# infergo-ml/gogp

Measured on AMD Instinct MI355X. Metric: GP.Observe+Gradient evals/sec (fp64) at N=16384 D=8, higher is better.
Workload: dtype f64

## Files before the change

### gogp_amd/_lib.py

```python
from __future__ import annotations

import ctypes
import os
import subprocess

from .kernel import CDesc

_HERE = os.path.dirname(os.path.abspath(__file__))
LIB_PATH = os.path.join(_HERE, "libgogp_hip.so")
HOOKS_PATH = os.path.join(_HERE, "libgogp_testhooks.so")

GOGP_OK, GOGP_EARG, GOGP_ENOTPD, GOGP_EHIP, GOGP_ESTATE, GOGP_ENOMEM, GOGP_ECOND = 0, 1, 2, 3, 4, 5, 6
GOGP_MAX_CANDIDATES = 16
GOGP_BATCH_MAX_N = 128
GOGP_COV_MAX_M = 4096
GOGP_MULTI_MAX_T = 128

_dp = ctypes.POINTER(ctypes.c_double)
_i64 = ctypes.c_int64
_h = ctypes.c_void_p
_descp = ctypes.POINTER(CDesc)
GOGP_UNIQUE_ID_BYTES = 128


class CXfer(ctypes.Structure):
    _fields_ = [("peer", ctypes.c_int32), ("is_send", ctypes.c_int32), ("buf", ctypes.c_void_p),
                ("bytes", ctypes.c_int64)]


EXCHANGE_FN = ctypes.CFUNCTYPE(ctypes.c_int, ctypes.c_void_p, ctypes.POINTER(CXfer), ctypes.c_int32)
ALLREDUCE_FN = ctypes.CFUNCTYPE(ctypes.c_int, ctypes.c_void_p, ctypes.POINTER(ctypes.c_double),
                                ctypes.c_int64)
class CGemmOpts(ctypes.Structure):
    _fields_ = [(n, ctypes.c_int32) for n in ("ktri", "krag0", "new_row0", "kbeg0", "small_below", "prio", "rule",
                                              "tpb_shift", "rblk0", "cblk0", "pr", "Pr", "pc", "Pc", "beta0", "k")]
    _fields_ += [("bstride", ctypes.c_int64)]
    DEFAULTS = dict(ktri=0, krag0=-1, new_row0=-1, kbeg0=0, small_below=384, prio=0, rule=0, tpb_shift=0, rblk0=0,
                    cblk0=0, pr=0, Pr=1, pc=0, Pc=1, beta0=-1, k=1, bstride=0)


class CKParams(ctypes.Structure):
    _T, _D, _E = 4, 64, 32
    _fields_ = [("ndim", ctypes.c_int32), ("nterms", ctypes.c_int32), ("kind", ctypes.c_int32 * _T),
                ("ard", ctypes.c_int32 * _T), ("c", ctypes.c_double * _T), ("w", ctypes.c_double * _T),
                ("inv_len", (ctypes.c_double * _D) * _T), ("noise_var", ctypes.c_double), ("dnoise", ctypes.c_double),
                ("nevents", ctypes.c_int32), ("ev_axis", ctypes.c_int32), ("ev_from", ctypes.c_double * _E),
                ("ev_to", ctypes.c_double * _E), ("ev_disc", ctypes.c_double * _E)]


GOGP_TEST_NACC = 16 + 64


class CGemmPlan(ctypes.Structure):
    _fields_ = [("tile", ctypes.c_int32), ("waves", ctypes.c_int32), ("grid_x", ctypes.c_int64),
                ("grid_z", ctypes.c_int64), ("flops", ctypes.c_double), ("tag", ctypes.c_int64)]


SYMBOLS = [
    ("gogp_desc_check", ctypes.c_int, [_descp]),
    ("gogp_desc_ntheta_noise", ctypes.c_int, [_descp]),
    ("gogp_create", ctypes.c_int, [_descp, ctypes.c_int, ctypes.POINTER(_h)]),
    ("gogp_destroy", None, [_h]),
    ("gogp_last_error", ctypes.c_char_p, [_h]),
    ("gogp_notpd_index", _i64, [_h]),
    ("gogp_graph_info", ctypes.c_int, [_h, ctypes.POINTER(ctypes.c_int64), ctypes.POINTER(ctypes.c_int)]),
    ("gogp_events_check", ctypes.c_int, [_dp, ctypes.c_int, ctypes.c_int, ctypes.c_int]),
    ("gogp_set_events", ctypes.c_int, [_h, _dp, ctypes.c_int, ctypes.c_int]),
    ("gogp_set_data", ctypes.c_int, [_h, _dp, _dp, _i64]),
    ("gogp_set_data_device", ctypes.c_int, [_h, ctypes.c_void_p, ctypes.c_void_p, _i64]),
    ("gogp_absorb", ctypes.c_int, [_h, _dp, _dp]),
    ("gogp_observe", ctypes.c_int, [_h, _dp, _i64, _dp]),
    ("gogp_observe_full", ctypes.c_int, [_h, _dp, _i64, _dp]),
    ("gogp_lml", ctypes.c_int, [_h, _dp]),
    ("gogp_gradient", ctypes.c_int, [_h, _dp, _i64]),
    ("gogp_loo", ctypes.c_int, [_h, _dp, _dp, _dp, _dp]),
    ("gogp_loo_gradient", ctypes.c_int, [_h, _dp, _i64]),
    ("gogp_multi_set_outputs", ctypes.c_int, [_h, _dp, _i64, ctypes.c_int32]),
    ("gogp_multi_lml", ctypes.c_int, [_h, _dp, _dp]),
    ("gogp_multi_gradient", ctypes.c_int, [_h, _dp, _i64]),
    ("gogp_multi_get_alpha", ctypes.c_int, [_h, _dp]),
    ("gogp_multi_produce", ctypes.c_int, [_h, _dp, _i64, _dp, _dp]),
    ("gogp_observe_gradient_batch", ctypes.c_int,
     [ctypes.POINTER(_h), ctypes.c_int, _dp, _i64, _dp, _dp, ctypes.POINTER(ctypes.c_int)]),
    ("gogp_observe_gradient_candidates", ctypes.c_int,
     [_h, ctypes.c_int, _dp, _i64, _dp, _dp, ctypes.POINTER(ctypes.c_int)]),
    ("gogp_batch_set_data", ctypes.c_int,
     [_h, _dp, _dp, _i64, ctypes.c_int32, ctypes.POINTER(_i64), ctypes.POINTER(_i64)]),
    ("gogp_batch_observe_gradient", ctypes.c_int,
     [_h, ctypes.c_int32, ctypes.POINTER(ctypes.c_int32), _dp, _i64, _dp, _dp, ctypes.POINTER(ctypes.c_int)]),
    ("gogp_batch_produce", ctypes.c_int,
     [_h, ctypes.c_int32, ctypes.POINTER(ctypes.c_int32), _dp, _i64, ctypes.POINTER(_i64), _dp, _dp, _dp, _dp,
      ctypes.POINTER(ctypes.c_int)]),
    ("gogp_batch_observe_full_gradient", ctypes.c_int,
     [_h, ctypes.c_int32, _dp, ctypes.POINTER(_i64), _dp, _dp, ctypes.POINTER(ctypes.c_int)]),
    ("gogp_batch_produce_full", ctypes.c_int,
     [_h, ctypes.c_int32, _dp, ctypes.POINTER(_i64), ctypes.POINTER(_i64), _dp, _dp, _dp, _dp,
      ctypes.POINTER(ctypes.c_int)]),
    ("gogp_produce", ctypes.c_int, [_h, _dp, _i64, _dp, _dp]),
    ("gogp_produce_gradient", ctypes.c_int, [_h, _dp, _i64, _dp, _dp, _dp, _dp]),
    ("gogp_produce_covariance", ctypes.c_int, [_h, _dp, _i64, _dp, _dp]),
    ("gogp_produce_samples", ctypes.c_int, [_h, _dp, _i64, _dp, _i64, ctypes.c_double, _dp, _dp]),
    ("gogp_n", _i64, [_h]),
    ("gogp_get_alpha", ctypes.c_int, [_h, _dp]),
    ("gogp_get_factor", ctypes.c_int, [_h, _dp]),
    ("gogp_get_factor_rows", ctypes.c_int, [_h, ctypes.POINTER(_i64), _i64, _dp]),
    ("gogp_get_factor_diag", ctypes.c_int, [_h, _dp]),
    ("gogp_set_factor", ctypes.c_int, [_h, _dp, _dp, _dp, _dp]),
    ("gogp_append", ctypes.c_int, [_h, _dp, _dp, ctypes.c_int64]),
    ("gogp_remove", ctypes.c_int, [_h, ctypes.POINTER(_i64), ctypes.c_int64]),
    ("gogp_dist_grid", ctypes.c_int, [ctypes.c_int, ctypes.POINTER(ctypes.c_int), ctypes.POINTER(ctypes.c_int)]),
    ("gogp_dist_unique_id", ctypes.c_int, [ctypes.c_void_p]),
    ("gogp_dist_init_rccl", ctypes.c_int,
     [_h, ctypes.c_int, ctypes.c_int, ctypes.c_int, ctypes.c_int, ctypes.c_char_p]),
    ("gogp_dist_init_callbacks", ctypes.c_int,
     [_h, ctypes.c_int, ctypes.c_int, ctypes.c_int, ctypes.c_int, ctypes.c_void_p, ctypes.c_void_p,
      ctypes.c_void_p]),
    ("gogp_dist_local_bytes", _i64, [_h]),
    ("gogp_dist_comm_ranks", ctypes.c_int, [_h, ctypes.POINTER(ctypes.c_int)]),
    ("gogp_dist_selftest", ctypes.c_int, [_h, ctypes.c_int, _i64]),
    ("gogp_profile_enable", ctypes.c_int, [_h, ctypes.c_int]),
    ("gogp_profile_read", ctypes.c_int, [_h, _dp, ctypes.POINTER(_i64), _dp, _dp]),
    ("gogp_profile_read_launches", ctypes.c_int,
     [_h, _i64, _dp, _dp, _dp, ctypes.POINTER(_i64), ctypes.POINTER(_i64)]),
    ("gogp_profile_read_aux", ctypes.c_int, [_h, ctypes.c_int, _dp, ctypes.POINTER(_i64)]),
    ("gogp_set_option", ctypes.c_int, [_h, ctypes.c_char_p, _i64]),
    ("gogp_version", ctypes.c_char_p, []),
]

HOOK_SYMBOLS = [
    ("gogp_mfma_f64_peak", ctypes.c_int, [ctypes.c_int, ctypes.c_int, _dp, _dp, _dp]),
    ("gogp_mfma_f32_peak", ctypes.c_int, [ctypes.c_int, ctypes.c_int, _dp, _dp, _dp]),
    ("gogp_bench_gemm", ctypes.c_int,
     [ctypes.c_int, ctypes.c_int, ctypes.c_int, ctypes.c_int, _i64, ctypes.c_int, _dp, _dp]),
    ("gogp_test_diag256", ctypes.c_int,
     [ctypes.c_int, _dp, _dp, _dp, ctypes.POINTER(ctypes.c_uint64), _dp]),
    ("gogp_test_dgemm_nt", ctypes.c_int,
     [ctypes.c_int, _i64, _i64, _i64, ctypes.c_double, _dp, _dp, ctypes.c_double, _dp]),
    ("gogp_test_valu_cost", ctypes.c_int, [ctypes.c_int, _dp]),
    ("gogp_test_panel128", ctypes.c_int,
     [ctypes.c_int, _dp, _dp, _i64, ctypes.c_int, ctypes.POINTER(ctypes.c_uint64), _dp]),
    ("gogp_test_panel128_slabs", ctypes.c_int, [ctypes.c_int, _dp, _dp, _i64, ctypes.c_int, ctypes.c_int, _dp]),
    ("gogp_test_gemm_nt", ctypes.c_int,
     [ctypes.c_int, ctypes.c_int, ctypes.c_int, ctypes.c_int, ctypes.c_int, _i64, ctypes.c_double, ctypes.c_double]
     + [ctypes.c_void_p, _i64, _i64, _i64] * 3 + [ctypes.POINTER(CGemmOpts)]),
    ("gogp_test_gemm_plan", ctypes.c_int,
     [ctypes.c_int, ctypes.c_int, ctypes.c_int, ctypes.c_int, _i64, ctypes.POINTER(CGemmOpts),
      ctypes.POINTER(CGemmPlan)]),
    ("gogp_test_diag_syrk", ctypes.c_int,
     [ctypes.c_int, ctypes.c_int, ctypes.c_void_p, _i64, _i64, _i64, _i64, _i64, _dp, _i64, ctypes.c_int]),
    ("gogp_test_diag256_product", ctypes.c_int,
     [ctypes.c_int, ctypes.c_int, _dp, _i64, _dp, _i64, _dp, _i64, _i64, ctypes.POINTER(ctypes.c_longlong)]),
    ("gogp_test_trsm_small_workspace", _i64, [_i64]),
    ("gogp_test_trsm_small", ctypes.c_int,
     [ctypes.c_int, ctypes.c_int, _i64, ctypes.c_void_p, _i64, _i64, ctypes.c_void_p, ctypes.c_void_p, _i64, _i64,
      ctypes.c_int, ctypes.c_int, _dp, _i64, ctypes.c_void_p, _i64, ctypes.POINTER(ctypes.c_int),
      ctypes.POINTER(ctypes.c_int), ctypes.POINTER(_i64), ctypes.POINTER(ctypes.c_uint)]),
    ("gogp_test_trsv_steps", ctypes.c_int,
     [ctypes.c_int, ctypes.c_int, ctypes.c_int, _i64, ctypes.c_void_p, _i64, _i64, ctypes.c_void_p, ctypes.c_int,
      ctypes.c_int, ctypes.c_int, _i64, _dp, _i64, _dp, _i64]),
    ("gogp_test_alpha_from_y", ctypes.c_int,
     [ctypes.c_int, ctypes.c_int, _i64, ctypes.c_void_p, _i64, _i64, _dp, _i64, _dp, _i64]),
    ("gogp_test_rownorm_dot", ctypes.c_int,
     [ctypes.c_int, ctypes.c_int, ctypes.c_void_p, _i64, _i64, _i64, _i64, _dp, _i64, _dp, _i64, _dp, _i64]),
    ("gogp_test_tinv", ctypes.c_int,
     [ctypes.c_int, ctypes.c_int, ctypes.c_int, ctypes.c_void_p, ctypes.c_void_p, _i64, _i64, ctypes.c_int,
      ctypes.c_void_p]),
    ("gogp_test_blockmm", ctypes.c_int,
     [ctypes.c_int, ctypes.c_int, ctypes.c_int, ctypes.c_void_p, _i64] + [ctypes.POINTER(_i64)] * 6
     + [ctypes.POINTER(ctypes.c_int), ctypes.c_double, ctypes.c_int, _i64]),
    ("gogp_test_grad_blocks", ctypes.c_int, [_i64, _i64, _i64, ctypes.c_int]),
    ("gogp_test_grad_reduce", ctypes.c_int,
     [ctypes.c_int, ctypes.c_int, ctypes.POINTER(CKParams)] + [ctypes.c_int] * 4
     + [_dp, _i64, _dp, _i64, ctypes.c_void_p, _i64, _i64, _i64, _i64, ctypes.c_int, ctypes.c_int, _i64, _dp, _i64, _dp]),
    ("gogp_test_grad_reduce_local", ctypes.c_int,
     [ctypes.c_int, ctypes.c_int, ctypes.POINTER(CKParams)] + [ctypes.c_int] * 4
     + [_dp, _i64, _dp, _i64, ctypes.c_void_p, _i64, _i64, _i64, _i64, _i64, _i64] + [ctypes.c_int] * 7
     + [_i64, _dp, _i64, _dp]),
    ("gogp_test_xgrad", ctypes.c_int,
     [ctypes.c_int, ctypes.POINTER(CKParams), ctypes.c_int, _dp, _i64, _dp, _i64, _dp, _i64, _i64, _i64, _i64, _dp,
      _i64]),
    ("gogp_test_append_gram", ctypes.c_int,
     [ctypes.c_int] + [ctypes.c_void_p, _i64, ctypes.c_int, ctypes.c_int, _i64] * 2
     + [ctypes.c_int, ctypes.c_int, _i64, _i64, _dp, _i64, _dp, _i64, _dp, _i64, _i64]),
    ("gogp_test_append_commit", ctypes.c_int,
     [ctypes.c_int, ctypes.POINTER(CKParams), ctypes.c_int, _dp, _i64, _dp, _i64, ctypes.c_int, _i64, _dp, _i64,
      ctypes.c_int, _dp, _i64, _i64, _dp, _i64, ctypes.POINTER(ctypes.c_longlong)]),
    ("gogp_test_remove_gather", ctypes.c_int,
     [ctypes.c_int, _dp, _i64, _i64, ctypes.POINTER(ctypes.c_int), _i64, _i64, _dp, _i64, _i64]),
    ("gogp_test_remove_w", ctypes.c_int,
     [ctypes.c_int, _dp, _i64, _i64, ctypes.POINTER(ctypes.c_int), _i64, ctypes.POINTER(ctypes.c_int), _i64, ctypes.c_int,
      ctypes.c_int, _i64, _i64, _i64, _dp, _i64]),
    ("gogp_test_remove_block", ctypes.c_int,
     [ctypes.c_int, _dp, _i64, _i64, ctypes.c_int, ctypes.c_int, _dp, _i64, _dp, _i64, ctypes.c_int, _i64, _i64, _i64]),
    ("gogp_test_bwd_panel", ctypes.c_int,
     [ctypes.c_int, _i64] + [_dp, _i64, _i64, _i64] * 3 + [_i64, _i64, ctypes.c_int, ctypes.c_int]),
    ("gogp_test_pcov_slabs", ctypes.c_int, [_i64, _i64, ctypes.c_int, ctypes.POINTER(ctypes.c_int)]),
    ("gogp_test_pcov", ctypes.c_int,
     [ctypes.c_int, ctypes.POINTER(CKParams), ctypes.c_int, _dp, _i64, _i64, _dp, _i64, _i64, _i64, ctypes.c_int, _dp, _i64,
      ctypes.c_double, _dp, _i64, _i64, _i64]),
    ("gogp_test_multi_weight", ctypes.c_int,
     [ctypes.c_int, _dp, _i64, _i64, ctypes.c_int, _dp, _i64, _i64, _i64, _i64, _dp, _i64]),
    ("gogp_test_dist_init_replay", ctypes.c_int, [ctypes.c_void_p] + [ctypes.c_int] * 4),
]


def build(force: bool = False) -> str:
    csrc = os.path.join(_HERE, "csrc")
    cmd = ["make", "-C", csrc, "-j8", "-s"]
    if force:
        cmd.append("-B")
    subprocess.check_call(cmd)
    if not os.path.exists(LIB_PATH):
        raise RuntimeError("build did not produce %s" % LIB_PATH)
    return LIB_PATH


_lib = None
_hooks = None


def hooks() -> ctypes.CDLL:
    global _hooks
    if _hooks is None:
        lib()
        if not os.path.exists(HOOKS_PATH):
            raise ImportError("%s is missing: run __graft_entry__.build()" % HOOKS_PATH)
        L = ctypes.CDLL(HOOKS_PATH)
        for name, restype, argtypes in HOOK_SYMBOLS:
            f = getattr(L, name)
            f.restype = restype
            f.argtypes = argtypes
        _hooks = L
    return _hooks


def lib() -> ctypes.CDLL:
    global _lib
    if _lib is None:
        if not os.path.exists(LIB_PATH):
            raise ImportError(
                "%s is missing: build it with `python -c 'import __graft_entry__ as g; g.build()'` "
                "(gogp_amd has no CPU fallback)" % LIB_PATH)
        try:
            import torch
        except ImportError:
            pass
        L = ctypes.CDLL(LIB_PATH, mode=ctypes.RTLD_GLOBAL)
        for name, restype, argtypes in SYMBOLS:
            f = getattr(L, name)
            f.restype = restype
            f.argtypes = argtypes
        _lib = L
    return _lib
```

### gogp_amd/csrc/api.hip

```cpp
#include <math.h>
#include <stdio.h>
#include <stdlib.h>
#include <string.h>

#include <algorithm>
#include <initializer_list>
#include <mutex>
#include <new>
#include <thread>
#include <type_traits>
#include <utility>

#include "handle.h"

using namespace gogp;

static thread_local std::string g_create_error;

extern "C" int gogp_desc_ntheta_noise(const gogp_desc *d) {
  return (d && (d->noise_kind == GOGP_NOISE_UNIFORM || d->noise_kind == GOGP_NOISE_CONSTANT_PARAM)) ? 1 : 0;
}

extern "C" int gogp_desc_check(const gogp_desc *d) {
  if (!d) return GOGP_EARG;
// ... 352 lines not shown
}

static void fill_params_theta(const gogp_handle *h, const double *ts, const double *tn, DevParams &p) {
  const gogp_desc &d = h->desc;
  memset(&p, 0, sizeof p);
  p.ndim = d.ndim;
  p.nterms = d.nterms;
  p.ns = h->ns;
  p.nn = h->nn;
  for (int t = 0; t < d.nterms; ++t) {
    const gogp_term &T = d.terms[t];
    p.kind[t] = T.kind;
    p.ard[t] = T.ard;
    p.c[t] = T.scale_idx >= 0 ? ts[T.scale_idx] : 1.0;
    p.w[t] = 0.0;
    if (T.kind == GOGP_K_PERIODIC)
      p.w[t] = M_PI / (T.period_mult * ts[T.period_idx]);
    for (int j = 0; j < d.ndim; ++j)
      p.inv_len[t][j] = 1.0 / ts[T.len_idx + (T.ard ? j : 0)];
  }
  if (d.noise_kind == GOGP_NOISE_CONSTANT || d.noise_kind == GOGP_NOISE_CONSTANT_PARAM) {
    p.noise_var = d.noise_std * d.noise_std;
    p.dnoise = 0.0;
  } else {
    const double sd = tn[0];
    p.noise_var = d.noise_scale * sd * sd;
    p.dnoise = 2.0 * p.noise_var;
  }
  p.nevents = h->nevents;
  p.ev_axis = h->ev_axis;
  for (int e = 0; e < h->nevents; ++e) {
    p.ev_from[e] = h->events[e][0];
    p.ev_to[e] = h->events[e][1];
    p.ev_disc[e] = h->events[e][2];
  }
}

static void fill_params(const gogp_handle *h, DevParams &p) {
  fill_params_theta(h, h->theta_s.data(), h->theta_n.data(), p);
}

int gogp_upload_params(gogp_handle *h) {
  if (h->batch_mode) return GOGP_OK;
  fill_params(h, *h->hostP);
  HIPCHK(h, hipMemcpyAsync(h->devP, h->hostP, sizeof(DevParams), hipMemcpyHostToDevice, h->s));
  return GOGP_OK;
}

static hipError_t cand_memset(gogp_handle *h, void *dst, size_t bytes, hipStream_t s) {
  hipError_t e = hipSuccess;
  for (int c = 0; c < h->batch_k && e == hipSuccess; ++c)
    e = gogp::rec_memset_async((char *)dst + (size_t)c * h->cand_stride, 0, bytes, s);
  return e;
}
static hipError_t cand_copy_in(gogp_handle *h, void *dst, const void *src, size_t bytes, hipStream_t s) {
  hipError_t e = hipSuccess;
  for (int c = 0; c < h->batch_k && e == hipSuccess; ++c)
    e = gogp::rec_memcpy_async((char *)dst + (size_t)c * h->cand_stride, src, bytes, hipMemcpyDeviceToDevice, s);
  return e;
}
static hipError_t cand_d2h(gogp_handle *h, double *hdst, const void *dsrc, size_t bytes, hipStream_t s) {
  hipError_t e = hipSuccess;
  for (int c = 0; c < h->batch_k && e == hipSuccess; ++c)
    e = gogp::rec_memcpy_async(hdst + (size_t)c * BATCH_ROW, (const char *)dsrc + (size_t)c * h->cand_stride, bytes,
                               hipMemcpyDeviceToHost, s);
  return e;
}

static int ensure_y(gogp_handle *h) {
  if (h->bufY && h->cap_y >= h->npad) return GOGP_OK;
  (void)hipFree(h->bufY);
  h->bufY = nullptr;
  h->cap_y = 0;
  const int64_t cap = std::max(h->npad, h->cap_npad);
  HIPCHK(h, hipMalloc(&h->bufY, (size_t)cap * (size_t)cap * h->esz()));
  h->cap_y = cap;
  return GOGP_OK;
}

static int ensure_d64(gogp_handle *h) {
  if (h->D64 && h->cap_d64 >= h->npad) return GOGP_OK;
  (void)hipFree(h->D64);
  h->D64 = nullptr;
  h->cap_d64 = 0;
  const int64_t cap = std::max(h->npad, h->cap_npad);
  HIPCHK(h, hipMalloc(&h->D64, (size_t)cap * PANEL * sizeof(double)));
  h->cap_d64 = cap;
  return GOGP_OK;
}

struct FactorResult {
  int rc = GOGP_OK;
  double lml = 0.0, cond_lb = 1.0, yta = 0.0;
  int64_t notpd = -1;
  std::string msg;
};
static FactorResult judge_scalars(const gogp_handle *h, const double *hs, bool fp32, bool refine, int64_t n = -1) {
  FactorResult r;
  long long info = 0;
  memcpy(&info, hs + HS_INFO, sizeof info);
  char buf[160];
  if (info != 0) {
    r.rc = GOGP_ENOTPD;
    r.notpd = (int64_t)info - 1;
    snprintf(buf, sizeof buf, "Factorize: matrix is not positive definite (pivot %lld)", (long long)r.notpd);
    r.msg = buf;
    return r;
  }
  const double logdet = fp32 ? hs[5] : hs[0];
  const double ztz = refine ? hs[6] : hs[1];
  r.yta = ztz;
  r.lml = -0.5 * (double)(n < 0 ? h->n : n) * log(2 * M_PI) - 0.5 * logdet - 0.5 * ztz;
  const double dmin = hs[3], dmax = hs[4];
  r.cond_lb = (dmin > 0.0) ? (dmax / dmin) * (dmax / dmin) : INFINITY;
  if (!(r.cond_lb <= h->cond_limit)) {
    snprintf(buf, sizeof buf, "Condition: matrix singular or near-singular with condition number >= %.4e",
             r.cond_lb);
    r.msg = buf;
    r.rc = GOGP_ECOND;
  }
  return r;
}

static int finish_factorize(gogp_handle *h, bool fp32, bool refine, bool kinv) {
  h->alpha_pending = true;
  if (h->batch_mode) {
    h->factored = h->have_alpha = true;
    if (kinv) h->have_kinv = true;
    return GOGP_OK;
  }
  HIPCHK(h, hipStreamSynchronize(h->s));
  HIPCHK(h, hipGetLastError());
  const FactorResult fr = judge_scalars(h, h->hscal, fp32, refine);
  if (fr.rc == GOGP_ENOTPD) {
    h->alpha_pending = h->kinv_pending = false;
    h->tinv_valid = h->tinv_pending = false;
    h->trtri_done = h->trtri_pending = false;
    h->notpd = fr.notpd;
    h->err = fr.msg;
    return GOGP_ENOTPD;
  }
  h->lml = fr.lml;
  h->logdet2 = h->hscal[0];
  h->yta = fr.yta;
  h->factored = h->have_alpha = true;
  h->z_valid = true;
  if (kinv) h->have_kinv = true;
  h->cond_lb = fr.cond_lb;
  if (fr.rc == GOGP_ECOND) h->err = fr.msg;
  return fr.rc;
}

static void diag_block(gogp_handle *h, hipStream_t sp, const double *A, int64_t ld, double *L, int64_t ldl,
                       double *Dp, int64_t c0) {
  launch_diag256(sp, A, ld, L, ldl, Dp, c0, h->n, h->info);
}
static void diag_block(gogp_handle *h, hipStream_t sp, const float *A, int64_t ld, float *L, int64_t ldl,
                       float *Dp, int64_t c0) {
  double *A64 = h->dscr, *L64 = h->dscr + PANEL * PANEL, *D64 = h->dscr + 2 * PANEL * PANEL;
  if (h->d64_active)
    A64 = h->D64 + (size_t)(c0 / PANEL) * PANEL * PANEL;
  else
    launch_convert_block(sp, A, ld, A64, PANEL, PANEL, PANEL);
  launch_diag256(sp, A64, PANEL, L64, PANEL, D64, c0, h->n, h->info);
  launch_convert_block(sp, L64, PANEL, L, ldl, PANEL, PANEL);
  launch_convert_block(sp, D64, PANEL, Dp, PANEL, PANEL, PANEL);
  launch_logdet_block(sp, L64, PANEL, c0, h->n, PANEL, h->scalars + 5);
}
static void diag_inv_only(gogp_handle *h, hipStream_t s, const double *L, int64_t ld, double *Dp) {
  (void)h;
  launch_diag256_inv_only(s, L, ld, Dp);
}
static void diag_inv_only(gogp_handle *h, hipStream_t s, const float *L, int64_t ld, float *Dp) {
  double *L64 = h->dscr + PANEL * PANEL, *D64 = h->dscr + 2 * PANEL * PANEL;
  launch_convert_block(s, L, ld, L64, PANEL, PANEL, PANEL);
  launch_diag256_inv_only(s, L64, PANEL, D64);
  launch_convert_block(s, D64, PANEL, Dp, PANEL, PANEL, PANEL);
}

static inline int chain_prio_of(const gogp_handle *h) {
  return h->chain_prio < 0 ? (h->npad <= 6144 ? 1 : 0) : h->chain_prio;
}
static inline GemmGrid chain_grid(const gogp_handle *h) {
  GemmGrid g;
  g.prio = chain_prio_of(h);
  return g;
}

static inline int superpanel_width(const gogp_handle *h, int npanel, int P0) {
  const int head = h->superpanel_head < 0 ? (h->prec == 32 ? 4 : 3) : h->superpanel_head;
  const int sw = (head > 0 && npanel - P0 > h->head_remaining) ? head : h->superpanel;
  return (npanel - P0 < sw) ? npanel - P0 : sw;
}
struct SuperPanel {
  int P0, nsub, prevP0, next_nsub;
  int64_t C0() const { return (int64_t)P0 * PANEL; }
  int64_t CE() const { return C0() + (int64_t)nsub * PANEL; }
};
static std::vector<SuperPanel> superpanels(const gogp_handle *h) {
  const int npanel = (int)(h->npad / PANEL);
  std::vector<SuperPanel> v;
  for (int P0 = 0; P0 < npanel; P0 += v.back().nsub) {
    const int nsub = superpanel_width(h, npanel, P0);
    if (!v.empty()) v.back().next_nsub = nsub;
    v.push_back({P0, nsub, v.empty() ? -1 : v.back().P0, 0});
  }
  return v;
}
struct InnerGroup {
  int grp;
  int64_t k0, ce;
};
static inline InnerGroup inner_group(int q, int64_t c2, int64_t CE) {
  const int done = q + 1, grp = done & -done;
  return {grp, c2 - (int64_t)grp * PANEL, std::min(c2 + (int64_t)grp * PANEL, CE)};
}

constexpr int TMT_BLOCKS = 8;
static inline int tinv_panels(const gogp_handle *h) { return h->produce_panels; }
static inline int64_t tinv_signature(const gogp_handle *h) {
  return (int64_t)h->produce_panels + (h->npad << 8) + ((int64_t)h->prec << 56);
}
static int ensure_tinv(gogp_handle *h) {
  const int64_t tld = (int64_t)tinv_panels(h) * PANEL;
  const size_t need = (size_t)std::max(h->npad, h->cap_npad) * (size_t)tld;
  if (!h->TX || h->cap_tinv < need) {
    (void)hipFree(h->TX);
    (void)hipFree(h->Tmt);
    h->TX = h->Tmt = nullptr;
    h->cap_tinv = 0;
    HIPCHK(h, hipMalloc(&h->TX, need * h->esz()));
    HIPCHK(h, hipMalloc(&h->Tmt, (size_t)TMT_BLOCKS * PANEL * PANEL * h->esz()));
    h->cap_tinv = need;
  }
  h->tinv_ld = tld;
  return GOGP_OK;
}

template <class T>
static void assemble_tinv(gogp_handle *h, hipStream_t sp, int P0, int nsub) {
  const int64_t ld = h->npad, tld = h->tinv_ld, C0 = (int64_t)P0 * PANEL;
  T *X = reinterpret_cast<T *>(h->TX) + C0 * tld;
  T *MT = reinterpret_cast<T *>(h->Tmt);
  const T *L = reinterpret_cast<const T *>(h->bufL);
  const T *Dinv = reinterpret_cast<const T *>(h->Dinv) + (size_t)P0 * PANEL * PANEL;
  launch_tinv_init(sp, Dinv, X, (T *)nullptr, nsub, tld);
  for (int d = 1; d < nsub; ++d) {
    const int cnt = nsub - d;
    for (int b0 = 0; b0 < cnt; b0 += 6) {
      const int nb = std::min(6, cnt - b0);
      const T *A1[6], *B1[6], *A2[6], *B2[6];
      T *C1[6], *C2[6];
      int64_t lda1[6], ldb1[6], ldc1[6], lda2[6], ldb2[6], ldc2[6];
      int K1[6], K2[6];
      for (int b = 0; b < nb; ++b) {
        const int i = d + b0 + b, j = i - d;
        A1[b] = L + (C0 + (int64_t)i * PANEL) * ld + C0 + (int64_t)j * PANEL;
        lda1[b] = ld;
        B1[b] = X + (int64_t)j * PANEL * tld + (int64_t)j * PANEL;
        ldb1[b] = tld;
        C1[b] = MT + (size_t)(b0 + b) * PANEL * PANEL;
        ldc1[b] = PANEL;
        K1[b] = d * PANEL;
        A2[b] = Dinv + (size_t)i * PANEL * PANEL;
        lda2[b] = PANEL;
        B2[b] = C1[b];
        ldb2[b] = PANEL;
        C2[b] = X + (int64_t)i * PANEL * tld + (int64_t)j * PANEL;
        ldc2[b] = tld;
        K2[b] = PANEL;
      }
      launch_blockmm(sp, nb, A1, lda1, B1, ldb1, C1, ldc1, K1, 1.0);
      launch_blockmm(sp, nb, A2, lda2, B2, ldb2, C2, ldc2, K2, -1.0);
    }
  }
}

template <class T>
struct InvBufs {
  T *A, *Y;
  const T *L, *Dinv;
};
template <class T>
static void trtri_superstep(gogp_handle *h, const InvBufs<T> &B, const SuperPanel &P, hipStream_t st, hipStream_t s2) {
  const int64_t npad = h->npad, ld = npad;
  T *R = B.A, *Y = B.Y;
  const T *L = B.L;
  GemmProfile *pf = &h->prof;
  const int P0 = P.P0;
  const int64_t C0 = P.C0(), CE = P.CE();
  for (int q = 0; q < P.nsub; ++q) {
    const int p = P0 + q;
    const int64_t c0 = (int64_t)p * PANEL, c2 = c0 + PANEL;
    const T *Dp = B.Dinv + (size_t)p * PANEL * PANEL;
    launch_ydiag(st, Dp, Y + c0 * ld + c0, ld);
    if (c2 < CE)
      launch_zero_block(st, Y + c2 * ld + c0, ld, CE - c2, PANEL);
    if (c0 > 0) {
      GemmGrid gtri = chain_grid(h);
      gtri.ktri = h->ktri;
      launch_gemm_nt(st, GEMM_RECT, (int)(c0 / TILE), 2, PANEL, 1.0, R + c0, ld, Dp, PANEL, 0.0,
                      Y + c0, ld, pf, &gtri);
    }
    if (c2 < CE) {
      const InnerGroup g = inner_group(q, c2, CE);
      GemmGrid gch = chain_grid(h);
      if (h->krag) gch.krag0 = (int)(g.k0 / TILE);
      launch_gemm_nt(st, GEMM_RECT, (int)(c2 / TILE), (int)((g.ce - c2) / TILE), (int64_t)g.grp * PANEL,
                      -1.0, Y + g.k0, ld, L + c2 * ld + g.k0, ld, 1.0, R + c2, ld, pf, &gch);
    }
  }
  order(h, EV_BASE + 4 * P0 + 2, st, s2);
  const int nt = (int)((npad - CE) / TILE);
  if (nt > 0) {
    const int64_t Kw = CE - C0;
    const int mr = (int)(CE / TILE);
    const int ntn = nt < 2 * P.next_nsub ? nt : 2 * P.next_nsub;
    if (P0 > 0 && st != s2)
      (void)gogp::rec_stream_wait(st, ev(h, EV_BASE + 4 * P.prevP0 + 3));
    GemmGrid gch = chain_grid(h), gbulk;
    if (h->krag) gch.krag0 = gbulk.krag0 = (int)(C0 / TILE);
    launch_gemm_nt(st, GEMM_RECT, mr, ntn, Kw, -1.0, Y + C0, ld, L + CE * ld + C0, ld, 1.0,
                    R + CE, ld, pf, &gch);
    if (nt > ntn) {
      const int64_t C3 = CE + (int64_t)ntn * TILE;
      launch_gemm_nt(s2, GEMM_RECT, mr, nt - ntn, Kw, -1.0, Y + C0, ld, L + C3 * ld + C0, ld, 1.0,
                      R + C3, ld, pf, &gbulk);
    }
    (void)gogp::rec_event_record(ev(h, EV_BASE + 4 * P0 + 3), s2);
  }
}

static inline bool mixed_gradient(const gogp_handle *h) {
  return h->grad_prec == 32 && h->prec == 64 && !h->batch_mode && !h->dist;
}
static int ensure_g32(gogp_handle *h) {
  const int64_t cap = std::max(h->npad, h->cap_npad);
  if (h->g32A && h->g32_cap >= cap) return GOGP_OK;
  (void)hipFree(h->g32A);
  (void)hipFree(h->g32L);
  (void)hipFree(h->g32Y);
  (void)hipFree(h->g32D);
  h->g32A = h->g32L = h->g32Y = h->g32D = nullptr;
  h->g32_cap = 0;
  const size_t nn = (size_t)cap * (size_t)cap * sizeof(float);
  HIPCHK(h, hipMalloc(&h->g32A, nn));
  HIPCHK(h, hipMalloc(&h->g32L, nn));
  HIPCHK(h, hipMalloc(&h->g32Y, nn));
  HIPCHK(h, hipMalloc(&h->g32D, (size_t)(cap / PANEL) * PANEL * PANEL * sizeof(float)));
  h->g32_cap = cap;
  return GOGP_OK;
}
static void mixed_superstep(gogp_handle *h, const SuperPanel &P, hipStream_t st, hipStream_t s2) {
  const int64_t npad = h->npad, ld = npad, C0 = P.C0(), W = P.CE() - C0;
  launch_convert_block(st, h->bufL + C0 * ld + C0, ld, h->g32L + C0 * ld + C0, ld, (int)(npad - C0), (int)W);
  launch_convert_block(st, h->Dinv + (size_t)P.P0 * PANEL * PANEL, PANEL, h->g32D + (size_t)P.P0 * PANEL * PANEL, PANEL,
                       (int)W, PANEL);
  const InvBufs<float> B{h->g32A, h->g32Y, h->g32L, h->g32D};
  trtri_superstep<float>(h, B, P, st, s2);
}

template <class T>
static void kinv_accumulate(gogp_handle *h, const T *Y, T *A, int64_t C0, int64_t CE) {
  (void)gogp::rec_stream_wait(h->sk, ev(h, EV_BASE + 4 * (size_t)(C0 / PANEL) + 2));
  GemmGrid gk;
  gk.new_row0 = (int)(C0 / TILE);
  if (h->krag) gk.krag0 = (int)(C0 / TILE);
  launch_gemm_nt(h->sk, GEMM_LOWER, (int)(CE / TILE), (int)(CE / TILE), CE - C0, 1.0, Y + C0, h->npad, Y + C0, h->npad,
                 1.0, A, h->npad, &h->prof, &gk);
}

template <class T>
static void zero_inverse_rhs(gogp_handle *h, bool mixed, hipStream_t s) {
  if (mixed)
    launch_zero_upper_blocks(s, h->g32A, h->npad, h->npad);
  else
    launch_zero_upper_blocks(s, reinterpret_cast<T *>(h->bufA), h->npad, h->npad);
}
template <class T>
static void inverse_superstep(gogp_handle *h, bool mixed, const SuperPanel &P, hipStream_t st, hipStream_t s2,
                              bool fuse_kinv) {
  if (mixed) {
    mixed_superstep(h, P, st, s2);
    if (fuse_kinv) kinv_accumulate<float>(h, h->g32Y, h->g32A, P.C0(), P.CE());
  } else {
    const InvBufs<T> B{reinterpret_cast<T *>(h->bufA), reinterpret_cast<T *>(h->bufY), reinterpret_cast<const T *>(h->bufL),
                       reinterpret_cast<const T *>(h->Dinv)};
    trtri_superstep<T>(h, B, P, st, s2);
    if (fuse_kinv) kinv_accumulate<T>(h, B.Y, B.A, P.C0(), P.CE());
  }
}

static inline int chain_split_of(const gogp_handle *h, bool eager) {
  if (h->dist || h->prec != 64) return 0;
  if (h->chain_split >= 0) return h->chain_split;
  return (h->npad <= 8192 || !eager) ? 2 : 0;
}
static void fused_panel(gogp_handle *h, hipStream_t sp, double *A, double *L, int64_t ld, int64_t c0, int64_t npad,
                        GemmProfile *pf) {
  const int64_t c1 = c0 + TILE, c2 = c0 + PANEL;
  const int mt1 = (int)((npad - c1) / TILE);
  const GemmGrid gch = chain_grid(h);
  launch_panel128_slabs(sp, A + c0 * ld + c0, ld, L + c0 * ld + c0, ld, 0, npad - c1, c0, h->n, h->info, h->chain_slabs);
  launch_gemm_nt(sp, GEMM_RECT, mt1, 1, TILE, -1.0, L + c1 * ld + c0, ld, L + c1 * ld + c0, ld, 1.0, A + c1 * ld + c1, ld,
                 pf, &gch);
  launch_panel128_slabs(sp, A + c0 * ld + c0, ld, L + c0 * ld + c0, ld, 1, npad - c2, c0, h->n, h->info, h->chain_slabs);
}

static void begin_evaluation(gogp_handle *h, std::initializer_list<hipStream_t> streams) {
  auto wait = [&](int e) {
    for (hipStream_t q : streams) (void)gogp::rec_stream_wait(q, ev(h, e));
  };
  if (h->trtri_pending) wait(EV_TRTRI);
  if (h->kinv_pending) wait(EV_KINV);
  if (h->kinv_c1 > 0 && !h->have_kinv) wait(EV_KINV);
  h->trtri_pending = h->kinv_pending = false;
  h->factored = h->have_alpha = h->have_kinv = h->grad_valid = false;
  h->multi_solved = false;
  h->alpha_pending = h->trtri_done = h->ydone_valid = h->d64_active = false;
  h->notpd = -1;
  h->kinv_c1 = 0;
  if (!h->batch_mode) h->tinv_valid = false;
}
static hipError_t enqueue_result_scalars(gogp_handle *h, hipStream_t s) {
  const hipError_t e = cand_d2h(h, h->hscal, h->scalars, 7 * sizeof(double), s);
  return e != hipSuccess ? e : cand_d2h(h, h->hscal + HS_INFO, h->info, sizeof(long long), s);
}

template <class T>
static void substitute_fwd(gogp_handle *h, hipStream_t q, const T *L, const T *Dinv, double *w, double *dst) {
  const int npanel = (int)(h->npad / PANEL);
  for (int b = 0; b < npanel; ++b) launch_trsv_fwd_step(q, L, h->npad, Dinv, b, npanel, w, dst);
}
template <class T>
static hipError_t substitute_bwd(gogp_handle *h, hipStream_t q, const T *L, const T *Dinv, const double *src, double *w,
                                 double *dst) {
  const int npanel = (int)(h->npad / PANEL);
  const hipError_t e = hipMemcpyAsync(w, src, (size_t)h->npad * sizeof(double), hipMemcpyDeviceToDevice, q);
  for (int b = npanel - 1; b >= 0 && e == hipSuccess; --b) launch_trsv_bwd_step(q, L, h->npad, Dinv, b, npanel, w, dst);
  return e;
}

template <class T>
struct Sweep {
  static constexpr bool fp32 = sizeof(T) == 4;
  gogp_handle *h;
  bool eager;
  T *A = reinterpret_cast<T *>(h->bufA), *L = reinterpret_cast<T *>(h->bufL), *Dinv = reinterpret_cast<T *>(h->Dinv);
  int64_t npad = h->npad, ld = npad;
  int npanel = (int)(npad / PANEL);
  GemmProfile *pf = &h->prof;
  hipStream_t s = h->s, st = h->st, s2 = h->s2;
  hipStream_t sp = h->lookahead ? h->sp : h->s;
  hipStream_t sz = h->lookahead ? h->sl : sp;
  bool mixed = !fp32 && mixed_gradient(h);
  bool fuse_kinv = eager && (h->kinv_fused < 0 ? (npad <= 10240 || mixed) : h->kinv_fused != 0);
  int split = fp32 ? 0 : chain_split_of(h, eager);

  void d64_init(hipStream_t q, int first, int nblk) const {
    if constexpr (fp32)
      launch_widen_diag_blocks(q, A + (int64_t)first * PANEL * (ld + 1), ld, h->D64 + (size_t)first * PANEL * PANEL, nblk);
  }
  void d64_update(hipStream_t q, int64_t k0, int64_t K, int first, int nblk) const {
    if constexpr (fp32) {
      if (h->d64_active)
        launch_diag_syrk_f64(q, L + (int64_t)first * PANEL * ld + k0, ld, K, h->D64 + (size_t)first * PANEL * PANEL, nblk);
    }
  }

  int build_gram() const {
    if (sp != s) order(h, EV_ENTRY, s, sp);
    HIPCHK(h, cand_memset(h, h->info, sizeof(long long), sp));
    const int w0 = superpanel_width(h, npanel, 0);
    {
      AuxTimer tm(h, GOGP_PROF_GRAM, s);
      launch_gram_lower_split(sp, s, h->devP, h->D, h->dX, h->n, npad, A, ld, (int64_t)w0 * PANEL, h->ev());
    }
    h->d64_active = fp32 && h->diag_fp64 != 0;
    if (h->d64_active) {
      const int rc = ensure_d64(h);
      if (rc != GOGP_OK) return rc;
      d64_init(sp, 0, w0);
      if (npanel > w0) d64_init(s, w0, npanel - w0);
    }
    (void)gogp::rec_event_record(ev(h, EV_GRAM), s);
    if (eager) {
      (void)gogp::rec_stream_wait(s2, ev(h, EV_GRAM));
      (void)gogp::rec_stream_wait(st, ev(h, EV_GRAM));
      zero_inverse_rhs<T>(h, mixed, s2);
      order(h, EV_INIT, s2, st);
    }
    return GOGP_OK;
  }

  void chain_superpanel(const SuperPanel &P) const {
    const int64_t CE = P.CE();
    for (int q = 0; q < P.nsub; ++q) {
      const int p = P.P0 + q;
      const int64_t c0 = (int64_t)p * PANEL, c2 = c0 + PANEL;
      if constexpr (!fp32) {
        if (split) fused_panel(h, sp, A, L, ld, c0, npad, pf);
      }
      if (!split) {
        T *Dp = Dinv + (size_t)p * PANEL * PANEL;
        diag_block(h, sp, A + c0 * ld + c0, ld, L + c0 * ld + c0, ld, Dp, c0);
        const int mt2 = (int)((npad - c2) / TILE);
        if (mt2 > 0) {
          GemmGrid gtri = chain_grid(h);
          gtri.ktri = h->ktri;
          launch_gemm_nt(sp, GEMM_RECT, mt2, 2, PANEL, 1.0, A + c2 * ld + c0, ld, Dp, PANEL, 0.0,
                          L + c2 * ld + c0, ld, pf, &gtri);
        }
      }
      if (c2 < CE) {
        d64_update(sp, c0, PANEL, p + 1, (int)((CE - c2) / PANEL));
        const InnerGroup g = inner_group(q, c2, CE);
        const GemmGrid gch = chain_grid(h);
        launch_gemm_nt(sp, GEMM_TRAP, (int)((npad - c2) / TILE), (int)((g.ce - c2) / TILE),
                        (int64_t)g.grp * PANEL, -1.0, L + c2 * ld + g.k0, ld, L + c2 * ld + g.k0, ld, 1.0,
                        A + c2 * ld + c2, ld, pf, &gch);
      }
    }
  }

  void panels_final(const SuperPanel &P) const {
    order(h, EV_BASE + 4 * P.P0, sp, s);
    if (sz != sp) (void)gogp::rec_stream_wait(sz, ev(h, EV_BASE + 4 * P.P0));
    if constexpr (!fp32) {
      if (split) {
        launch_dinv256_blocks(sz, L + (int64_t)P.P0 * PANEL * (ld + 1), ld, Dinv + (size_t)P.P0 * PANEL * PANEL, P.nsub);
        if (eager) {
          (void)gogp::rec_event_record(ev(h, EV_BASE + 5 * (size_t)npanel + 32 + (size_t)P.P0), sz);
          (void)gogp::rec_stream_wait(st, ev(h, EV_BASE + 5 * (size_t)npanel + 32 + (size_t)P.P0));
        }
      }
    }
    for (int q = 0; q < P.nsub; ++q) launch_trsv_fwd_step(sz, L, ld, Dinv, P.P0 + q, npanel, h->w, h->z);
  }

  void trailing_update(const SuperPanel &P) const {
    const int64_t C0 = P.C0(), CE = P.CE();
    const int mtE = (int)((npad - CE) / TILE);
    if (mtE <= 0) return;
    const int64_t Kw = CE - C0;
    const int ntn = mtE < 2 * P.next_nsub ? mtE : 2 * P.next_nsub;
    (void)gogp::rec_stream_wait(sp, ev(h, P.P0 > 0 ? EV_BASE + 4 * P.prevP0 + 1 : EV_GRAM));
    const GemmGrid gch = chain_grid(h);
    launch_gemm_nt(sp, GEMM_TRAP, mtE, ntn, Kw, -1.0, L + CE * ld + C0, ld, L + CE * ld + C0, ld,
                    1.0, A + CE * ld + CE, ld, pf, &gch);
    d64_update(sp, C0, Kw, (int)(CE / PANEL), ntn / 2);
    if (mtE > ntn) {
      const int64_t C3 = CE + (int64_t)ntn * TILE;
      launch_gemm_nt(s, GEMM_LOWER, mtE - ntn, mtE - ntn, Kw, -1.0, L + C3 * ld + C0, ld,
                      L + C3 * ld + C0, ld, 1.0, A + C3 * ld + C3, ld, pf);
      d64_update(s, C0, Kw, (int)(C3 / PANEL), (mtE - ntn) / 2);
    }
    (void)gogp::rec_event_record(ev(h, EV_BASE + 4 * P.P0 + 1), s);
  }

  void inverse_behind(const SuperPanel &P) const {
    const int64_t CE = P.CE();
    (void)gogp::rec_stream_wait(st, ev(h, EV_BASE + 4 * P.P0));
    inverse_superstep<T>(h, mixed, P, st, s2, fuse_kinv);
    if (!fp32 && !fuse_kinv && !mixed && !h->batch_mode && h->kinv_split > 0 && h->kinv_c1 == 0 && CE < npad &&
        CE * 100 >= npad * (int64_t)h->kinv_split) {
      (void)gogp::rec_stream_wait(h->sk, ev(h, EV_BASE + 4 * P.P0 + 2));
      const T *Y0 = reinterpret_cast<const T *>(h->bufY);
      launch_gemm_nt(h->sk, GEMM_LAUUM, (int)(CE / TILE), (int)(CE / TILE), CE, 1.0, Y0, ld, Y0, ld, 0.0, A, ld, pf);
      (void)gogp::rec_event_record(ev(h, EV_KINV), h->sk);
      h->kinv_c1 = CE;
    }
  }

  int finish_alpha() const {
    if (fp32) {
      if (sz != sp) (void)gogp::rec_stream_wait(sp, ev(h, EV_FWD));
      HIPCHK(h, substitute_bwd(h, sp, L, Dinv, h->z, h->w, h->alpha));
      for (int it = 0; it < h->refine_steps; ++it) {
        launch_residual(sp, h->devP, h->D, h->dX, h->n, npad, h->alpha, h->dy, h->rpart, REFINE_SLABS, h->rw,
                        h->radial1, h->ev());
        substitute_fwd(h, sp, L, Dinv, h->rw, h->rz);
        HIPCHK(h, substitute_bwd(h, sp, L, Dinv, h->rz, h->rw, h->rd));
        launch_axpy(sp, h->alpha, h->rd, npad);
      }
      launch_dot(sp, h->dy, h->alpha, h->n, h->scalars + 6);
      order(h, EV_ALPHA, sp, s);
    }
    HIPCHK(h, enqueue_result_scalars(h, s));
    if (fp32) {
      if (eager) (void)gogp::rec_event_record(ev(h, EV_TRTRI), st);
    } else if (eager && !mixed) {
      (void)gogp::rec_stream_wait(st, ev(h, EV_FWD));
      launch_alpha_from_y(st, reinterpret_cast<const T *>(h->bufY), ld, h->z, npad, h->alpha);
      (void)gogp::rec_event_record(ev(h, EV_ALPHA), st);
      (void)gogp::rec_event_record(ev(h, EV_TRTRI), st);
    } else {
      if (sz != sp) (void)gogp::rec_stream_wait(sp, ev(h, EV_FWD));
      HIPCHK(h, substitute_bwd(h, sp, L, Dinv, h->z, h->w, h->alpha));
      (void)gogp::rec_event_record(ev(h, EV_ALPHA), sp);
    }
    return GOGP_OK;
  }
};

template <class T>
static int factorize_t(gogp_handle *h, bool eager) {
  const Sweep<T> c{h, eager && h->lookahead != 0};
  begin_evaluation(h, {c.s, c.sp});
  int rc = gogp_upload_params(h);
  if (rc == GOGP_OK && (c.mixed || c.eager)) rc = c.mixed ? ensure_g32(h) : ensure_y(h);
  if (rc == GOGP_OK) rc = c.build_gram();
  if (rc != GOGP_OK) return rc;
  if (c.fp32) HIPCHK(h, hipMemsetAsync(h->scalars + 5, 0, sizeof(double), c.sp));
  HIPCHK(h, cand_copy_in(h, h->w, h->dy, (size_t)c.npad * sizeof(double), c.sp));
  if (c.sz != c.sp) order(h, EV_W, c.sp, c.sz);
  for (const SuperPanel &P : superpanels(h)) {
    c.chain_superpanel(P);
    c.panels_final(P);
    c.trailing_update(P);
    if (c.eager) c.inverse_behind(P);
  }
  if (c.fuse_kinv) {
    (void)gogp::rec_event_record(ev(h, EV_KINV), h->sk);
    h->kinv_pending = true;
  }
  if (c.eager) {
    (void)gogp::rec_event_record(ev(h, EV_TRTRI), c.st);
    (void)gogp::rec_event_record(ev(h, EV_YDONE), c.st);
    h->ydone_valid = h->trtri_done = h->trtri_pending = true;
  }
  order(h, EV_FWD, c.sz, c.s);
  launch_lml_scalars(c.s, c.L, c.ld, h->z, nullptr, nullptr, h->n, h->scalars);
  rc = c.finish_alpha();
  if (rc != GOGP_OK) return rc;
  const int rcf = finish_factorize(h, c.fp32, c.fp32, false);
  if (rcf == GOGP_ENOTPD)
    for (hipStream_t q : {c.sp, c.st, c.s2, h->sl, h->sk}) (void)hipStreamSynchronize(q);
  return rcf;
}

static inline bool tiny_ok(const gogp_handle *h) {
  return h->tiny && !h->dist && h->prec == 64 && h->npad == PANEL && h->n <= TILE && !mixed_gradient(h);
}
static int tiny_factorize(gogp_handle *h, bool eager) {
  hipStream_t s = h->s;
  begin_evaluation(h, {s});
  int rc = gogp_upload_params(h);
  if (rc != GOGP_OK) return rc;
  if (h->lookahead && !h->batch_mode) {
    order(h, EV_ENTRY, h->sp, s);
    order(h, EV_W, h->sl, s);
  }
  HIPCHK(h, cand_memset(h, h->info, sizeof(long long), s));
  launch_tiny_eval(s, h->devP, h->dX, h->dy, h->n, h->bufA, h->bufL, h->Dinv, h->z, h->alpha, h->info, eager, h->ev());
  launch_lml_scalars(s, h->bufL, h->npad, h->z, nullptr, nullptr, h->n, h->scalars);
  (void)gogp::rec_event_record(ev(h, EV_ALPHA), s);
  HIPCHK(h, enqueue_result_scalars(h, s));
  return finish_factorize(h, false, false, eager);
// ... 1946 lines not shown
  return GOGP_OK;
}

extern "C" int gogp_profile_read(gogp_handle *h, double *gemm_ms, int64_t *gemm_launches,
                                 double *gemm_flops, double *gemm_busy_ms) {
  if (!h) return GOGP_EARG;
  HIPCHK(h, hipSetDevice(h->device));
  for (hipStream_t q : work_streams(h)) HIPCHK(h, hipStreamSynchronize(q));
  double ms = 0.0, busy = 0.0;
  std::vector<std::pair<double, double>> iv;
  iv.reserve(h->prof.used / 2);
  for (size_t i = 0; i + 1 < h->prof.used; i += 2) {
    float t = 0.f, t0 = 0.f;
    if (hipEventElapsedTime(&t, h->prof.pool[i], h->prof.pool[i + 1]) != hipSuccess) continue;
    ms += t;
    if (hipEventElapsedTime(&t0, h->prof.pool[0], h->prof.pool[i]) != hipSuccess) continue;
    iv.emplace_back((double)t0, (double)t0 + (double)t);
  }
  std::sort(iv.begin(), iv.end());
  double cur_b = 0, cur_e = -1;
  for (auto &p : iv) {
    if (cur_e < cur_b || p.first > cur_e) {
      if (cur_e >= cur_b) busy += cur_e - cur_b;
      cur_b = p.first;
      cur_e = p.second;
    } else if (p.second > cur_e) {
      cur_e = p.second;
    }
  }
  if (cur_e >= cur_b && !iv.empty()) busy += cur_e - cur_b;
  if (gemm_ms) *gemm_ms = ms;
  if (gemm_launches) *gemm_launches = h->prof.launches;
  if (gemm_flops) *gemm_flops = h->prof.flops;
  if (gemm_busy_ms) *gemm_busy_ms = busy;
  h->prof.used = 0;
  h->prof.flops = 0;
  h->prof.launches = 0;
  h->prof.lflops.clear();
  h->prof.ltag.clear();
  return GOGP_OK;
}

extern "C" int gogp_set_option(gogp_handle *h, const char *name, int64_t value) {
  if (!h || !name) return GOGP_EARG;
  drop_cand_graph(h);
  if (strcmp(name, "produce_tinv") == 0) {
    h->produce_tinv = value != 0;
    return GOGP_OK;
  }
  if (strcmp(name, "produce_panels") == 0) {
    if (value < 1 || value > 8) return fail(h, GOGP_EARG, "produce_panels must be 1..8");
    h->produce_panels = (int)value;
    return GOGP_OK;
  }
  if (strcmp(name, "produce_small_below") == 0) {
    if (value < 0) return fail(h, GOGP_EARG, "produce_small_below must be >= 0");
    h->produce_small_below = (int)value;
    return GOGP_OK;
  }
  if (strcmp(name, "produce_small_max") == 0) {
    if (value < 0 || value > 64) return fail(h, GOGP_EARG, "produce_small_max must be 0..64");
    h->produce_small_max = (int)value;
    return GOGP_OK;
  }
  if (strcmp(name, "produce_groups") == 0) {
    if (value < 1 || value > PRODUCE_GROUPS) return fail(h, GOGP_EARG, "produce_groups must be 1..4");
    h->produce_groups = (int)value;
    return GOGP_OK;
  }
  if (strcmp(name, "gradient_precision") == 0) {
    if (value != 32 && value != 64) return fail(h, GOGP_EARG, "gradient_precision must be 32 or 64");
    if (value == 32 && (h->desc.nterms != 1 || h->desc.terms[0].scale_idx < 0))
      return fail(h, GOGP_EARG, "gradient_precision = 32 is offered for one-term kernels with an output scale only");
    HIPCHK(h, hipSetDevice(h->device));
    for (hipStream_t q : work_streams(h)) HIPCHK(h, hipStreamSynchronize(q));
    h->grad_prec = (int)value;
    h->have_kinv = h->grad_valid = false;
    h->trtri_done = h->trtri_pending = h->kinv_pending = false;
    return GOGP_OK;
  }
  if (strcmp(name, "trace_fp64") == 0) {
    h->trace_fp64 = value != 0;
    return GOGP_OK;
  }
  if (strcmp(name, "krag") == 0) {
    h->krag = value != 0;
    return GOGP_OK;
  }
  if (strcmp(name, "lookahead") == 0) {
    h->lookahead = value != 0;
    return GOGP_OK;
  }
  if (strcmp(name, "eager") == 0) {
    h->eager = value != 0;
    return GOGP_OK;
  }
  if (strcmp(name, "precision") == 0) {
    if (value != 32 && value != 64) return fail(h, GOGP_EARG, "precision must be 32 or 64");
    if (h->dist && (int)value != h->prec)
      return fail(h, GOGP_EARG, "precision: set it before gogp_dist_init_* (the shard's buffers are typed)");
    if ((int)value != h->prec) {
      HIPCHK(h, hipSetDevice(h->device));
      for (hipStream_t q : work_streams(h)) HIPCHK(h, hipStreamSynchronize(q));
      free_n_buffers(h);
      free_m_buffers(h);
      free_cand_buffers(h);
      h->prec = (int)value;
      h->have_data = h->factored = h->have_alpha = h->have_kinv = h->observed = h->grad_valid = false;
      h->multi_T = 0;
      h->multi_solved = false;
      h->trtri_done = h->trtri_pending = h->alpha_pending = h->kinv_pending = false;
    }
    return GOGP_OK;
  }
  if (strcmp(name, "kinv_split") == 0) {
    if (value < 0 || value > 95) return fail(h, GOGP_EARG, "kinv_split must be 0..95");
    h->kinv_split = (int)value;
    return GOGP_OK;
  }
  if (strcmp(name, "kinv_fused") == 0) {
    h->kinv_fused = value < 0 ? -1 : (value != 0);
    return GOGP_OK;
  }
  if (strcmp(name, "superpanel_head") == 0) {
    if (value < -1 || value > 8) return fail(h, GOGP_EARG, "superpanel_head must be -1..8");
    h->superpanel_head = (int)value;
    return GOGP_OK;
  }
  if (strcmp(name, "head_remaining") == 0) {
    if (value < 0) return fail(h, GOGP_EARG, "head_remaining must be >= 0");
    h->head_remaining = (int)value;
    return GOGP_OK;
  }
  if (strcmp(name, "ard_mfma_min_dims") == 0) {
    if (value < 1 || value > 65) return fail(h, GOGP_EARG, "ard_mfma_min_dims must be 1..65");
    h->ard_mfma_min = (int)value;
    return GOGP_OK;
  }
  if (strcmp(name, "chain_prio") == 0) {
    if (value < -1 || value > 2) return fail(h, GOGP_EARG, "chain_prio must be -1..2");
    h->chain_prio = (int)value;
    return GOGP_OK;
  }
  if (strcmp(name, "tiny") == 0) {
    if (value < 0 || value > 1) return fail(h, GOGP_EARG, "tiny must be 0 or 1");
    h->tiny = (int)value;
    return GOGP_OK;
  }
  if (strcmp(name, "chain_slabs") == 0) {
    if (value < 0 || value > 8) return fail(h, GOGP_EARG, "chain_slabs must be 0..8");
    h->chain_slabs = (int)value;
    return GOGP_OK;
  }
  if (strcmp(name, "chain_split") == 0) {
    if (value < -1 || value > 2 || value == 1) return fail(h, GOGP_EARG, "chain_split must be -1, 0 or 2");
    h->chain_split = (int)value;
    return GOGP_OK;
  }
  if (strcmp(name, "ktri") == 0) {
    h->ktri = value != 0;
    return GOGP_OK;
  }
  if (strcmp(name, "graph") == 0) {
    if (value < 0 || value > 3) return fail(h, GOGP_EARG, "graph must be 0..3");
    h->use_graph = (int)value;
    h->graph_failed = false;
    drop_cand_graph(h);
    return GOGP_OK;
  }
  if (strcmp(name, "diag_fp64") == 0) {
    if (value < 0 || value > 1) return fail(h, GOGP_EARG, "diag_fp64 must be 0 or 1");
    h->diag_fp64 = (int)value;
    return GOGP_OK;
  }
  if (strcmp(name, "refine_steps") == 0) {
    if (value < 0 || value > 8) return fail(h, GOGP_EARG, "refine_steps must be 0..8");
    h->refine_steps = (int)value;
    return GOGP_OK;
  }
  if (strcmp(name, "cond_limit_log10") == 0) {
    if (value < 1 || value > 300) return fail(h, GOGP_EARG, "cond_limit_log10 must be 1..300");
    h->cond_limit = pow(10.0, (double)value);
    return GOGP_OK;
  }
  if (strcmp(name, "superpanel") == 0) {
    if (value < 1 || value > 8) return fail(h, GOGP_EARG, "superpanel must be 1..8");
    h->superpanel = (int)value;
    return GOGP_OK;
  }
  return fail(h, GOGP_EARG, "unknown option");
}
```

### gogp_amd/csrc/common.h

```cpp
#pragma once
#include <hip/hip_runtime.h>
#include <stdint.h>

#include <string>
#include <vector>

#include "../../include/gogp_hip.h"
#include "graphrec.h"

namespace gogp {

constexpr int TILE = 128;
constexpr int PANEL = 256;
constexpr int GEMM_BK = 16;

struct DevParams {
  int ndim, nterms, ns, nn;
  int kind[GOGP_MAX_TERMS];
  int ard[GOGP_MAX_TERMS];
  double c[GOGP_MAX_TERMS];
  double w[GOGP_MAX_TERMS];
  double inv_len[GOGP_MAX_TERMS][GOGP_MAX_NDIM];
  double noise_var;
  double dnoise;
  int nevents, ev_axis;
  double ev_from[GOGP_MAX_EVENTS], ev_to[GOGP_MAX_EVENTS], ev_disc[GOGP_MAX_EVENTS];
};

constexpr int ACC_TRACE = 3 * GOGP_MAX_TERMS;
constexpr int ACC_ARD0 = 16;
constexpr int NACC = ACC_ARD0 + GOGP_MAX_NDIM;

struct Batch {
  int k = 1;
  long stride = 0;
};
inline thread_local Batch tl_batch;
template <class P>
__device__ __forceinline__ P *cand(P *p, long bstride) {
  return (P *)((const char *)p + (long)blockIdx.z * bstride);
}

struct GemmProfile {
  bool on = false;
  std::vector<hipEvent_t> pool;
  size_t used = 0;
  double flops = 0;
  int64_t launches = 0;
  std::vector<double> lflops;
  std::vector<int64_t> ltag;
};

struct GemmGrid {
  int rule = 0, tpb_shift = 0, rblk0 = 0, cblk0 = 0, pr = 0, Pr = 1, pc = 0, Pc = 1, beta0 = -1;
  int new_row0 = -1;
  int ktri = 0;
  int prio = 0;
  int krag0 = -1;
  int small_below = 384;
  int kbeg0 = 0;
};

struct BlockMap {
  int nb_shift = 9, pr = 0, Pr = 1, pc = 0, Pc = 1;
  __host__ __device__ long grow(long lrow) const {
    const long nbm = (1L << nb_shift) - 1;
    return ((((lrow >> nb_shift) * Pr + pr)) << nb_shift) + (lrow & nbm);
  }
  __host__ __device__ long gcol(long lcol) const {
    const long nbm = (1L << nb_shift) - 1;
    return ((((lcol >> nb_shift) * Pc + pc)) << nb_shift) + (lcol & nbm);
  }
};

#ifdef GOGP_WGSTAMP
struct StampRec {
  long long base, nwg, tag, stream;
};
constexpr int STAMP_SLOTS = 8;
extern unsigned long long *g_stamp_buf;
extern long long g_stamp_cap, g_stamp_used, g_stamp_nrec;
extern StampRec g_stamp_rec[1 << 16];
unsigned long long *stamp_reserve(long long nwg, long long tag, hipStream_t s);
#endif

enum GemmMode { GEMM_RECT = 0, GEMM_LOWER = 1, GEMM_LAUUM = 2,
                GEMM_TRAP = 3 };

void launch_dgemm_nt(hipStream_t s, GemmMode mode, int mt, int nt, int64_t K,
                     double alpha, const double *A, int64_t lda, const double *B,
                     int64_t ldb, double beta, double *C, int64_t ldc,
                     GemmProfile *prof, const GemmGrid *grid = nullptr);

void launch_gemm_nt(hipStream_t s, GemmMode mode, int mt, int nt, int64_t K, double alpha, const double *A,
                    int64_t lda, const double *B, int64_t ldb, double beta, double *C, int64_t ldc,
                    GemmProfile *prof, const GemmGrid *grid = nullptr);
void launch_gemm_nt(hipStream_t s, GemmMode mode, int mt, int nt, int64_t K, double alpha, const float *A,
                    int64_t lda, const float *B, int64_t ldb, double beta, float *C, int64_t ldc,
                    GemmProfile *prof, const GemmGrid *grid = nullptr);
void launch_gram_lower_split(hipStream_t s_first, hipStream_t s_rest, const DevParams *p, int ndim,
                             const double *X, int64_t n, int64_t npad, float *K, int64_t ld,
                             int64_t wcols, bool ev = false);
void launch_cross(hipStream_t s, const DevParams *p, int ndim, const double *X, int64_t n,
                  int64_t npad, const double *Z, int64_t m, int64_t mpad, float *KsT, int64_t ld, bool ev = false);
void launch_trsv_fwd_step(hipStream_t s, const float *L, int64_t ld, const float *Dinv, int b, int nblk,
                          double *y, double *z);
void launch_trsv_bwd_step(hipStream_t s, const float *L, int64_t ld, const float *Dinv, int b, int nblk,
                          double *zwork, double *alpha);
void launch_lml_scalars(hipStream_t s, const float *L, int64_t ld, const double *z, const double *y,
                        const double *alpha, int64_t n, double *scalars);
void launch_alpha_from_y(hipStream_t s, const float *Y, int64_t ld, const double *z, int64_t npad,
                         double *alpha);
void launch_rownorm_dot(hipStream_t s, const float *V, int64_t ld, const double *vec, int64_t ncols,
                        int64_t m, double *dot, double *sq);
void launch_zero_upper_blocks(hipStream_t s, float *R, int64_t ld, int64_t npad);
void launch_zero_block(hipStream_t s, float *B, int64_t ld, int64_t rows, int64_t cols);
void launch_ydiag(hipStream_t s, const float *Dinv, float *Ydiag, int64_t ld);
void launch_extract_lower(hipStream_t s, const float *L, int64_t ld, int64_t n, double *out);
void launch_pack_lower(hipStream_t s, const double *in, int64_t n, int64_t npad, float *L, int64_t ld);
void launch_convert_block(hipStream_t s, const float *src, int64_t lds_, double *dst, int64_t ldd, int rows,
                          int cols);
void launch_convert_block(hipStream_t s, const double *src, int64_t lds_, float *dst, int64_t ldd, int rows,
                          int cols);
void launch_grad_reduce(hipStream_t s, const DevParams *p, int ndim, int ard_dims, const double *X,
                        const double *alpha, const float *Kinv, int64_t ld, int64_t n, int64_t npad,
                        double *partials, double *out, bool radial1 = false, int mfma_min_dims = 1, bool ev = false,
                        int max_blocks = 0);

void launch_gram_lower(hipStream_t s, const DevParams *p, int ndim, const double *X,
                       int64_t n, int64_t npad, double *K, int64_t ld, bool ev = false);
void launch_gram_local(hipStream_t s, const DevParams *p, int ndim, const double *X, int64_t n,
                       int64_t mrows, int64_t ncols, BlockMap map, double *K, int64_t ld, bool ev = false);
void launch_gram_local(hipStream_t s, const DevParams *p, int ndim, const double *X, int64_t n,
                       int64_t mrows, int64_t ncols, BlockMap map, float *K, int64_t ld, bool ev = false);
void launch_gram_lower_split(hipStream_t s_first, hipStream_t s_rest, const DevParams *p, int ndim,
                             const double *X, int64_t n, int64_t npad, double *K, int64_t ld,
                             int64_t wcols, bool ev = false);
void launch_cross(hipStream_t s, const DevParams *p, int ndim, const double *X, int64_t n,
                  int64_t npad, const double *Z, int64_t m, int64_t mpad, double *KsT,
                  int64_t ld, bool ev = false);
void launch_residual(hipStream_t s, const DevParams *p, int ndim, const double *X, int64_t n, int64_t npad,
                     const double *v, const double *y, double *part, int nslab, double *r, bool radial1 = false,
                     bool ev = false);
void launch_kmatvec_share(hipStream_t s, const DevParams *p, int ndim, const double *X, int64_t n, int64_t npad,
                          const double *v, int part_idx, int nparts, double *part, int nslab, double *out,
                          bool radial1 = false, bool ev = false);
void launch_prior(hipStream_t s, const DevParams *p, const double *Z, int64_t m,
                  double *prior);

void launch_trsv_fwd_step(hipStream_t s, const double *L, int64_t ld, const double *Dinv,
                          int b, int nblk, double *y, double *z);
void launch_trsv_bwd_step(hipStream_t s, const double *L, int64_t ld, const double *Dinv,
                          int b, int nblk, double *zwork, double *alpha);

void launch_lml_scalars(hipStream_t s, const double *L, int64_t ld, const double *z,
                        const double *y, const double *alpha, int64_t n, double *scalars);
void launch_diag256(hipStream_t s, const double *A, int64_t ld, double *Lout, int64_t ldl,
                    double *Dinv, int64_t row0, int64_t nvalid, long long *info);
void launch_diag256_ld512(hipStream_t s, const double *A, int64_t ld, double *Lout, int64_t ldl,
                          double *Dinv, int64_t row0, int64_t nvalid, long long *info);
void launch_diag256_inv_only(hipStream_t s, const double *L, int64_t ld, double *Dinv);
void launch_diag_syrk_f64(hipStream_t s, const float *Lrows, int64_t ld, int64_t K, double *D64, int nblocks);
void launch_widen_diag_blocks(hipStream_t s, const float *A, int64_t ld, double *D64, int nblocks);
void launch_diag_syrk_f64_tiles(hipStream_t s, const float *Lrows, int64_t ld, int64_t K, double *D64, int nblocks,
                                int64_t row_stride, int bs);
void launch_panel128(hipStream_t s, const double *A, int64_t ld, double *Lout, int64_t ldl, int half, int64_t rows_below,
                     int64_t row0, int64_t nvalid, long long *info);
void launch_panel128_slabs(hipStream_t s, const double *A, int64_t ld, double *Lout, int64_t ldl, int half,
                           int64_t rows_below, int64_t row0, int64_t nvalid, long long *info, int slabs);
void launch_tiny_eval(hipStream_t s, const DevParams *P, const double *X, const double *y, int64_t n, double *A, double *L,
                      double *Dinv, double *z, double *alpha, long long *info, bool want_kinv, bool ev = false);
struct BatchItem {
  DevParams P;
  long off, n;
  long zoff, m;
  long roff;
};
constexpr int BATCH_ROW = NACC + 16;
void launch_batch_eval(hipStream_t s, const BatchItem *items, int k, const double *X, const double *y, const double *Z,
                       double *rows, double *mu, double *sigma, int ard_dims, bool produce, bool ev);
void launch_batch_eval_full(hipStream_t s, const BatchItem *items, int k, const double *x, const double *Z, double *rows,
                            double *mu, double *sigma, int ard_dims, bool produce, bool ev);
void launch_dinv256_blocks(hipStream_t s, const double *L, int64_t ld, double *Dinv, int nblk);
void launch_diag256_inv_only_ld512(hipStream_t s, const double *L, int64_t ld, double *Dinv);
void launch_convert_block(hipStream_t s, const double *src, int64_t lds_, double *dst, int64_t ldd, int rows,
                          int cols);
void launch_pack_lower(hipStream_t s, const double *in, int64_t n, int64_t npad, double *L,
                       int64_t ld);
void launch_sigma(hipStream_t s, const double *prior, const double *q, int64_t m,
                  double *sigma);
void launch_bwd_panel(hipStream_t s, int64_t rows16, const double *A, int64_t lda, const double *B, int64_t ldb,
                      double *C, int64_t ldc, int64_t ncols, int K, bool tri, bool sub);
int pgrad_slabs(int64_t npad, int64_t m, int *tiles_per_slab);
void launch_pgrad(hipStream_t s, const DevParams *p, int ndim, const double *X, int64_t n, int64_t npad,
                  const double *Z, int64_t m, const double *alpha, const double *Wt, int64_t ld, const double *sigma,
                  double *part, double *dmu, double *dsigma, bool ev);
int pcov_slabs(int64_t npad, int64_t m, int ncu, int *cols_per_slab);
void launch_pcov(hipStream_t s, const DevParams *p, const double *Z, int64_t m, const double *Vt, int64_t ld,
                 int64_t npad, int ncu, double *part, double diag_add, double *out, int64_t mo, int64_t ldo, bool ev);
void launch_pcov_add_mu(hipStream_t s, const double *G, int64_t ldg, const double *mu, int64_t ns, int64_t m, double *out);
int grad_reduce_blocks(int64_t npad);

void launch_grad_reduce(hipStream_t s, const DevParams *p, int ndim, int ard_dims,
                        const double *X, const double *alpha, const double *Kinv, int64_t ld, int64_t n,
                        int64_t npad, double *partials, double *out, bool radial1 = false, int mfma_min_dims = 1,
                        bool ev = false, int max_blocks = 0);
int grad_reduce_blocks_local(int64_t mrows, int64_t ncols);
void launch_grad_reduce_local(hipStream_t s, const DevParams *p, int ndim, int ard_dims,
                              const double *X, const double *alpha, const double *Kinv, int64_t ld,
                              int64_t n, int64_t mrows, int64_t ncols, BlockMap map, double *partials,
                              double *out, bool radial1 = false, int mfma_min_dims = 1, bool ev = false,
                              int max_blocks = 0);
void launch_grad_reduce_local(hipStream_t s, const DevParams *p, int ndim, int ard_dims,
                              const double *X, const double *alpha, const float *Kinv, int64_t ld,
                              int64_t n, int64_t mrows, int64_t ncols, BlockMap map, double *partials,
                              double *out, bool radial1 = false, int mfma_min_dims = 1, bool ev = false,
                              int max_blocks = 0);

void launch_grad_ard_mfma(hipStream_t s, const DevParams *p, int ndim, const double *X, const double *alpha,
                          const double *Kinv, int64_t ld, int64_t n, int nt, int ntc, int ntiles, int blocks,
                          BlockMap map, double *partials);
void launch_grad_ard_mfma(hipStream_t s, const DevParams *p, int ndim, const double *X, const double *alpha,
                          const float *Kinv, int64_t ld, int64_t n, int nt, int ntc, int ntiles, int blocks,
                          BlockMap map, double *partials);

void launch_xgrad(hipStream_t s, const DevParams *p, int ndim, const double *X,
                  const double *alpha, double *Kinv, int64_t ld, int64_t n, int64_t npad,
                  double *gx, bool ev = false);

void launch_rownorm_dot(hipStream_t s, const double *V, int64_t ld, const double *vec,
                        int64_t ncols, int64_t m, double *dot, double *sq);

void launch_zero_upper_blocks(hipStream_t s, double *R, int64_t ld, int64_t npad);
void launch_alpha_from_y(hipStream_t s, const double *Y, int64_t ld, const double *z,
                         int64_t npad, double *alpha);
void launch_zero_block(hipStream_t s, double *B, int64_t ld, int64_t rows, int64_t cols);
void launch_ydiag(hipStream_t s, const double *Dinv, double *Ydiag, int64_t ld);
void launch_tinv_init(hipStream_t s, const double *Dinv, double *X, double *XT, int nsub, int64_t tld);
void launch_tinv_init(hipStream_t s, const float *Dinv, float *X, float *XT, int nsub, int64_t tld);
void launch_blockmm(hipStream_t s, int nprod, const double *const *A, const int64_t *lda, const double *const *B,
                    const int64_t *ldb, double *const *C, const int64_t *ldc, const int *K, double alpha);
void launch_blockmm(hipStream_t s, int nprod, const float *const *A, const int64_t *lda, const float *const *B,
                    const int64_t *ldb, float *const *C, const int64_t *ldc, const int *K, double alpha);
void launch_trace_from_y(hipStream_t s, const float *Y, int64_t ld, int64_t n, int64_t npad, const double *alpha,
                         double *part, double *out);
size_t trsm_small_workspace_bytes(int64_t npad);
void launch_trsm_small(hipStream_t s, const double *L, int64_t ld, const double *Dinv, const double *KsT, int64_t ldk,
                       int64_t npad, int j0, int cnt, void *ws, double *dq, unsigned **tmo_dev);
void launch_trsm_small(hipStream_t s, const float *L, int64_t ld, const float *Dinv, const float *KsT, int64_t ldk,
                       int64_t npad, int j0, int cnt, void *ws, double *dq, unsigned **tmo_dev);
enum { TS_SOL_PAIRED = 0, TS_SOL_COMPACT = 1, TS_SOL_GRANULE = 2, TS_SOL_ROWS = 3 };
struct TsSolution {
  const void *p = nullptr;
  int kind = TS_SOL_PAIRED, width = 32;
};
TsSolution trsm_small_solution(int64_t npad, int j0, int cnt, void *ws, bool f32 = false);
constexpr int APPEND_PART = 64 * 64 + 64;
void launch_append_gram(hipStream_t s, TsSolution v0, TsSolution v1, int m0, int m, int64_t npc, int64_t n,
                        const double *z, double *part, double *Lnew, int64_t ld);
void launch_append_commit(hipStream_t s, const DevParams *p, const double *X2, const double *y2, int m, int64_t n,
                          const double *part, int nslab, double *Lnew, int64_t ld, double *z2out, long long *info,
                          bool ev);
void launch_append_identity_rows(hipStream_t s, double *L, int64_t ld, int64_t r0, int64_t r1, int64_t ncols);
void launch_append_restride(hipStream_t s, const double *src, int64_t ld0, int64_t npad0, double *dst, int64_t ld1,
                            int64_t npad1);
constexpr int REMOVE_W = 32, REMOVE_W_SMALL = 4;
void launch_remove_gather(hipStream_t s, const double *src, int64_t ld0, const int *map, int64_t n1, double *dst,
                          int64_t npad1);
void launch_remove_rows(hipStream_t s, const double *src, const int *map, int64_t n1, int width, double *dst);
void launch_remove_w(hipStream_t s, const double *src, int64_t ld0, const int *map, const int *rem, int mc, int mw, int64_t r0,
                     int64_t n1, int64_t npad1, double *W);
void launch_remove_snap(hipStream_t s, const double *L, int64_t ld, int b0, int nb, double *snap);
void launch_remove_block(hipStream_t s, double *L, int64_t ld, const double *snap, double *W, int mw, int64_t kb, int64_t n1);
void launch_loo_stats(hipStream_t s, const double *Kinv, int64_t ld, const double *alpha, const double *y, int64_t n,
                      int64_t npad, double *mu, double *sigma, double *logp, double *v, double *sc, double *part);
void launch_loo_scale_symv(hipStream_t s, const double *Kinv, int64_t ld, int64_t n, int64_t npad, const double *sc,
                           const double *v, double *B, int64_t ldb, double *upart, double *u);
void launch_loo_rank2(hipStream_t s, double *G, int64_t ld, int64_t n, int64_t npad, const double *u, const double *alpha);
void launch_multi_weight(hipStream_t s, const double *At, int64_t ld, int T, const double *Kinv, int64_t ldk, int64_t n,
                         int64_t npad, double *G);
void launch_multi_dots(hipStream_t s, const double *Yt, const double *At, int64_t ld, int64_t n, int T, double *dots);
void launch_fill(hipStream_t s, double *p, int64_t count, double v);
void launch_axpy(hipStream_t s, double *a, const double *b, int64_t count);
void launch_dot(hipStream_t s, const double *a, const double *b, int64_t n, double *out);
void launch_transpose_sq(hipStream_t s, const double *src, int64_t lds_, double *dst, int64_t ldd,
                         int n);
void launch_transpose_sq(hipStream_t s, const float *src, int64_t lds_, float *dst, int64_t ldd, int n);
void launch_pack_blocks(hipStream_t s, double *dst, const double *src, int nblk, int64_t blk,
                        int first, int stride);
int64_t chunk_tdot_scratch(int64_t max_rows, int nb);
void launch_chunk_tdot(hipStream_t s, const double *chunk, int64_t rows, int nb, const double *v,
                       double *part, double *out);
void launch_chunk_tdot(hipStream_t s, const float *chunk, int64_t rows, int nb, const double *v,
                       double *part, double *out);
void launch_chunk_alpha(hipStream_t s, const double *Ych, int mloc, int nloc, int nb, BlockMap map,
                        const double *z, double *out);
void launch_chunk_alpha(hipStream_t s, const float *Ych, int mloc, int nloc, int nb, BlockMap map,
                        const double *z, double *out);
void launch_chunk_sumsq(hipStream_t s, const double *Ych, int mloc, int nloc, int nb, BlockMap map, int64_t n, double *part,
                        double *out);
void launch_chunk_sumsq(hipStream_t s, const float *Ych, int mloc, int nloc, int nb, BlockMap map, int64_t n, double *part,
                        double *out);
void launch_logdet_block(hipStream_t s, const double *L, int64_t ld, int64_t row0, int64_t n, int nb,
                         double *acc);
void launch_sumsq_info(hipStream_t s, const double *z, int64_t n, const long long *info, double *out);
void launch_info_to_double(hipStream_t s, const long long *info, double *out);
void launch_extract_lower(hipStream_t s, const double *L, int64_t ld, int64_t n,
                          double *out);

}
```

### gogp_amd/csrc/diag256.hip

```cpp
#ifndef GOGP_EV
#include "common.h"
#include "kern_eval.h"
#include "pivot16.h"

#ifndef GOGP_NS
#define GOGP_NS gogp
#endif
namespace GOGP_NS {
using namespace gogp;


typedef double f64x4 __attribute__((ext_vector_type(4)));
typedef double f64x2 __attribute__((ext_vector_type(2)));

namespace {

constexpr int SLD = 130;
constexpr int XLD = 18;
constexpr int GSIZE = 2304;
constexpr int NT = 512;
constexpr int NW = NT / 64;

__device__ __forceinline__ double readlane_d(double x, int l) {
  int lo = __double2loint(x), hi = __double2hiint(x);
  lo = __builtin_amdgcn_readlane(lo, l);
  hi = __builtin_amdgcn_readlane(hi, l);
  return __hiloint2double(hi, lo);
}

__device__ __forceinline__ f64x4 mfma(double a, double b, f64x4 c) {
  return __builtin_amdgcn_mfma_f64_16x16x4f64(a, b, c, 0, 0, 0);
}

__device__ __forceinline__ void panel16(double *S, int kb, int lane, int row0, bool report,
                                        long grow0, long nvalid, long long *info,
                                        double (&keep)[16], double &keep_rinv) {
  const int r = lane & 15;
  const int prow = row0 + lane;
  const double *srcd = S + (kb * 16 + r) * SLD + kb * 16;
  double *srcp = S + (prow < 128 ? prow : 127) * SLD + kb * 16;
  double ap[16];
#pragma unroll
  for (int c = 0; c < 16; c += 2) {
    const f64x2 v = *reinterpret_cast<const f64x2 *>(srcd + c);
    const f64x2 u = *reinterpret_cast<const f64x2 *>(srcp + c);
    keep[c] = v.x;
    keep[c + 1] = v.y;
    ap[c] = u.x;
    ap[c + 1] = u.y;
  }
  int bad = 16;
  double mine = 0.0;
  PivotColumn<0, true>::run(keep, ap, bcast16<0>(keep[0]), 0.0, 0.0, bad, mine, r);
#pragma unroll
  for (int c = 0; c < 16; ++c) asm volatile("" : "+v"(ap[c]));
  asm volatile("" : "+v"(mine));
  if (row0 < 128) {
#pragma unroll
    for (int c = 0; c < 16; c += 2) *reinterpret_cast<f64x2 *>(srcp + c) = (f64x2){ap[c], ap[c + 1]};
  }
  keep_rinv = mine;
  if (report && bad < 16 && lane == 0 && grow0 + bad < nvalid && *info == 0)
    *info = (long long)(grow0 + bad + 1);
}

__device__ __forceinline__ void panel16_store_diag(double *S, int kb, double *rinv, int lane,
                                                   const double (&keep)[16], double keep_rinv) {
  if (lane < 16) {
    double *dst = S + (kb * 16 + lane) * SLD + kb * 16;
#pragma unroll
    for (int c = 0; c < 16; ++c) dst[c] = (c <= lane) ? keep[c] : 0.0;
    rinv[lane] = keep_rinv;
  }
}

template <bool HAVE_RINV>
__device__ __forceinline__ void inv16(const double *S, int kb, double *Xb, const double *rinv,
                                      int lane) {
  const int r = lane & 15;
  const double *Lb = S + (kb * 16) * SLD + kb * 16;
  double x[16];
#pragma unroll
  for (int rr = 0; rr < 16; ++rr) {
    double s = (rr == r) ? 1.0 : 0.0;
#pragma unroll
    for (int q = 0; q < rr; ++q) s -= Lb[rr * SLD + q] * x[q];
    double ri;
    if (HAVE_RINV) {
      ri = rinv[rr];
    } else {
      const double d = Lb[rr * SLD + rr];
      ri = __builtin_amdgcn_rcp(d);
      ri = fma(ri, fma(-d, ri, 1.0), ri);
      ri = fma(ri, fma(-d, ri, 1.0), ri);
    }
    x[rr] = (rr >= r) ? s * ri : 0.0;
  }
  if (lane < 16) {
#pragma unroll
    for (int rr = 0; rr < 16; ++rr) Xb[rr * XLD + r] = x[rr];
  }
}

__device__ __forceinline__ void tile_update16(double *S, int i, int c, int kb, int fr, int fk) {
  f64x4 acc = {0.0, 0.0, 0.0, 0.0};
#pragma unroll
  for (int k4 = 0; k4 < 4; ++k4) {
    const double av = S[(i * 16 + fr) * SLD + kb * 16 + k4 * 4 + fk];
    const double bv = S[(c * 16 + fr) * SLD + kb * 16 + k4 * 4 + fk];
    acc = mfma(av, bv, acc);
  }
#pragma unroll
  for (int v = 0; v < 4; ++v) S[(i * 16 + fk + 4 * v) * SLD + c * 16 + fr] -= acc[v];
}

#ifdef GOGP_POTRF_NOINLINE
__device__ __noinline__ void potrf128_lds(
#else
__device__ __forceinline__ void potrf128_lds(
#endif
    double *S, double *XD, double *rinv, int tid, long grow0,
                             long nvalid, long long *info, unsigned long long *st = nullptr) {
  const int lane = tid & 63, w = tid >> 6;
  const int fr = lane & 15, fk = lane >> 4;
  double keep[16], keep_rinv = 0.0;
  if (w < 2) panel16(S, 0, lane, 16 + 64 * w, w == 0, grow0, nvalid, info, keep, keep_rinv);
  if (st && tid == 0) st[1] = __builtin_amdgcn_s_memtime();
  __syncthreads();
  for (int kb = 0; kb < 7; ++kb) {
    if (w == 0) panel16_store_diag(S, kb, rinv + kb * 16, lane, keep, keep_rinv);
    if (kb + 1 + w < 8) tile_update16(S, kb + 1 + w, kb + 1, kb, fr, fk);
    __syncthreads();
    if (w < 2) {
      if ((kb + 2) * 16 + 64 * w < 128 || w == 0)
        panel16(S, kb + 1, lane, (kb + 2) * 16 + 64 * w, w == 0, grow0 + (kb + 1) * 16, nvalid,
                info, keep, keep_rinv);
      if (st && tid == 0 && kb < 2) st[kb * 3 + 2] = __builtin_amdgcn_s_memtime();
    } else {
      const int m = 6 - kb;
      const int nt3 = m * (m + 1) / 2;
      for (int t = w - 2; t < nt3; t += 6) {
        int ii = 0;
        while ((ii + 1) * (ii + 2) / 2 <= t) ++ii;
        const int cc = t - ii * (ii + 1) / 2;
        tile_update16(S, kb + 2 + ii, kb + 2 + cc, kb, fr, fk);
      }
    }
    __syncthreads();
  }
  if (w == 0) panel16_store_diag(S, 7, rinv + 7 * 16, lane, keep, keep_rinv);
  __syncthreads();
  inv16<true>(S, w, XD + w * 16 * XLD, rinv + w * 16, lane);
  __syncthreads();
}

template <int BS>
__device__ __forceinline__ void inv_phase(const double *S, f64x4 (&acc)[2], int w, int fr, int fk,
                                          int aoff, int boff) {
  constexpr int TB = BS / 16, NTPP = TB * TB, NTL = 4 * TB, KS = BS / 4;
  double av[2][KS], bv[2][KS];
#pragma unroll
  for (int u = 0; u < 2; ++u) {
    const int tile = w + u * NW;
    acc[u] = (f64x4){0.0, 0.0, 0.0, 0.0};
    if (tile < NTL) {
      const int p = tile / NTPP, tl = tile - p * NTPP;
      const int ti = tl / TB, tj = tl - ti * TB, o = p * 2 * BS;
#pragma unroll
      for (int ks = 0; ks < KS; ++ks) {
        av[u][ks] = S[(o + BS + ti * 16 + fr) * SLD + o + aoff + ks * 4 + fk];
        bv[u][ks] = S[(o + boff + ks * 4 + fk) * SLD + o + tj * 16 + fr];
      }
    }
  }
#pragma unroll
  for (int ks = 0; ks < KS; ++ks)
#pragma unroll
    for (int u = 0; u < 2; ++u)
      if (w + u * NW < NTL) acc[u] = mfma(av[u][ks], bv[u][ks], acc[u]);
}

template <int BS>
__device__ __forceinline__ void inv_store(double *S, const f64x4 (&acc)[2], int w, int fr, int fk,
                                          double sign) {
  constexpr int TB = BS / 16, NTPP = TB * TB, NTL = 4 * TB;
#pragma unroll
  for (int u = 0; u < 2; ++u) {
    const int tile = w + u * NW;
    if (tile < NTL) {
      const int p = tile / NTPP, tl = tile - p * NTPP;
      const int ti = tl / TB, tj = tl - ti * TB, o = p * 2 * BS;
#pragma unroll
      for (int v = 0; v < 4; ++v)
        S[(o + BS + ti * 16 + fk + 4 * v) * SLD + o + tj * 16 + fr] = sign * acc[u][v];
    }
  }
}

template <int BS>
__device__ __forceinline__ void inv_level(double *S, int w, int fr, int fk) {
  f64x4 acc[2];
  inv_phase<BS>(S, acc, w, fr, fk, 0, 0);
  __syncthreads();
  inv_store<BS>(S, acc, w, fr, fk, 1.0);
  __syncthreads();
  inv_phase<BS>(S, acc, w, fr, fk, BS, BS);
  __syncthreads();
  inv_store<BS>(S, acc, w, fr, fk, -1.0);
  __syncthreads();
}

__device__ void invert128_lds(double *S, const double *XD, int tid) {
  const int lane = tid & 63, w = tid >> 6;
  const int fr = lane & 15, fk = lane >> 4;
  for (int idx = tid; idx < 8 * 256; idx += NT) {
    const int kb = idx >> 8, e = idx & 255, rr = e >> 4, c = e & 15;
    S[(kb * 16 + rr) * SLD + kb * 16 + c] = XD[kb * 16 * XLD + rr * XLD + c];
  }
  __syncthreads();
  inv_level<16>(S, w, fr, fk);
  inv_level<32>(S, w, fr, fk);
  inv_level<64>(S, w, fr, fk);
}

#define GOGP_RT(m) ((m) ? 7 - wr : wr)
#define GOGP_CT(n) (2 * (n) + wc)
enum { TRI_A = 0, TRI_B = 1, TRI_SYM = 2 };
constexpr int BCH = 8;
constexpr int BBUF = 1152;
static_assert(2 * BBUF <= GSIZE, "chunk buffers must fit G");
template <bool B_NT, int TRI>
__device__ void wg_gemm128(f64x4 (&c)[2][4], const double *S, double *G, const double *Bg, long ldb,
                           int tid) {
  const int lane = tid & 63, w = tid >> 6;
  const int fr = lane & 15, fk = lane >> 4;
  const int wr = w >> 1, wc = w & 1;
#pragma unroll
  for (int m = 0; m < 2; ++m)
#pragma unroll
    for (int n = 0; n < 4; ++n) c[m][n] = (f64x4){0.0, 0.0, 0.0, 0.0};
  const double *gp;
  long gstep;
  int so;
  if (B_NT) {
    const int jj = tid >> 2, kq = (tid & 3) * 2;
    gp = Bg + (long)jj * ldb + kq;
    gstep = BCH;
    so = jj * 9 + kq;
  } else {
    const int kk = tid >> 6, j2 = (tid & 63) * 2;
    gp = Bg + (long)kk * ldb + j2;
    gstep = BCH * ldb;
    so = kk * 144 + j2;
  }
  const double *ap0 = S + (GOGP_RT(0) * 16 + fr) * SLD + fk;
  const double *ap1 = S + (GOGP_RT(1) * 16 + fr) * SLD + fk;
  const int bo = B_NT ? (wc * 16 + fr) * 9 + fk : fk * 144 + wc * 16 + fr;
  constexpr int BN = B_NT ? 32 * 9 : 32;
  constexpr int BS = B_NT ? 4 : 4 * 144;
  const int e0 = (TRI == TRI_A) ? 2 * (GOGP_RT(0) + 1) : 128 / BCH;
  const int e1 = (TRI == TRI_A) ? 2 * (GOGP_RT(1) + 1) : 128 / BCH;
  const int n0 = (TRI == TRI_SYM) ? (wr >= wc ? (wr - wc) / 2 + 1 : 0) : 4;
  const int n1 = (TRI == TRI_SYM) ? (7 - wr - wc) / 2 + 1 : 4;
  if (TRI == TRI_SYM) {
    const double *bp = S + (wc * 16 + fr) * SLD + fk;
#pragma unroll 2
    for (int k4 = 0; k4 < 32; ++k4) {
      const double a0 = ap0[k4 * 4];
      const double a1 = ap1[k4 * 4];
      double b[4];
#pragma unroll
      for (int n = 0; n < 4; ++n) b[n] = bp[n * 32 * SLD + k4 * 4];
#pragma unroll
      for (int n = 0; n < 4; ++n) {
        if (n < n0) c[0][n] = mfma(a0, b[n], c[0][n]);
        if (n < n1) c[1][n] = mfma(a1, b[n], c[1][n]);
      }
    }
    __syncthreads();
    return;
  }
  constexpr int NCH = 128 / BCH, PD = 4;
  static_assert(NCH % PD == 0, "the chunk loop is unrolled by the prefetch depth");
  double2 pre[PD];
  pre[0] = *reinterpret_cast<const double2 *>(gp);
#pragma unroll
  for (int u = 1; u < PD; ++u) pre[u] = *reinterpret_cast<const double2 *>(gp + (long)u * gstep);
  G[so] = pre[0].x;
  G[so + 1] = pre[0].y;
  __syncthreads();
#pragma unroll 1
  for (int kc0 = 0; kc0 < NCH; kc0 += PD) {
#pragma unroll
    for (int u = 0; u < PD; ++u) {
      const int kc = kc0 + u;
      const bool more = kc + 1 < NCH;
      if (kc + PD < NCH) pre[u] = *reinterpret_cast<const double2 *>(gp + (long)(kc + PD) * gstep);
      const double *bs = G + (kc & 1) * BBUF + bo;
      int nb = 0;
      if (TRI == TRI_B) {
        const int h = kc / 2 - wc;
        nb = h < 0 ? 0 : min(4, h / 2 + 1);
      }
      const bool act0 = kc < e0, act1 = kc < e1;
      if (act0 || act1) {
#pragma unroll
        for (int k4 = 0; k4 < BCH / 4; ++k4) {
          const double a0 = ap0[kc * BCH + k4 * 4];
          const double a1 = ap1[kc * BCH + k4 * 4];
          double b[4];
#pragma unroll
          for (int n = 0; n < 4; ++n) b[n] = bs[n * BN + k4 * BS];
#pragma unroll
          for (int n = 0; n < 4; ++n) {
            const bool on = (TRI == TRI_B) ? n < nb : true;
            if (on && act0 && n < n0) c[0][n] = mfma(a0, b[n], c[0][n]);
            if (on && act1 && n < n1) c[1][n] = mfma(a1, b[n], c[1][n]);
          }
        }
      }
      if (more) {
        double *d = G + ((kc + 1) & 1) * BBUF + so;
        d[0] = pre[(u + 1) % PD].x;
        d[1] = pre[(u + 1) % PD].y;
      }
      __syncthreads();
    }
  }
}

}

#define GOGP_STAMP(k)                                                   \
  do {                                                                  \
    if (STAMP && tid == 0) stamps[k] = __builtin_amdgcn_s_memtime();    \
  } while (0)

template <bool DO_POTRF, bool STAMP, int LDD>
__device__ __forceinline__ void diag256_body(double *S, double *G, double *rinv_s,
                                             const double *__restrict__ A, long ld,
                                             double *__restrict__ Lout, long ldl,
                                             double *__restrict__ Dinv, long row0, long nvalid,
                                             long long *info, unsigned long long *stamps) {
  const int tid = threadIdx.x;
  const int lane = tid & 63, w = tid >> 6;
  const int fr = lane & 15, fk = lane >> 4;
  const int wr = w >> 1, wc = w & 1;
  f64x4 c[2][4];
  const double *L10g = DO_POTRF ? (Lout + 128 * ldl) : (A + 128 * ld);
  const long ld10 = DO_POTRF ? ldl : ld;

#pragma unroll 1
  for (int half = 0; half < 2; ++half) {
    const long off = half * 128;
    GOGP_STAMP(half * 8 + 0);
    if (half == 0 || !DO_POTRF) {
#pragma unroll 2
      for (int idx = tid; idx < 128 * 64; idx += NT) {
        const int i = idx >> 6, cc = (idx & 63) * 2;
        const f64x2 v = *reinterpret_cast<const f64x2 *>(A + (off + i) * ld + off + cc);
        *reinterpret_cast<f64x2 *>(S + i * SLD + cc) =
            (f64x2){(cc <= i) ? v.x : 0.0, (cc + 1 <= i) ? v.y : 0.0};
      }
      __syncthreads();
    } else {
      wg_gemm128<true, TRI_SYM>(c, S, G, L10g, ld10, tid);
      GOGP_STAMP(26);
      double a11[2][4][4];
#pragma unroll
      for (int m = 0; m < 2; ++m)
#pragma unroll
        for (int n = 0; n < 4; ++n)
#pragma unroll
          for (int v = 0; v < 4; ++v)
            a11[m][n][v] = A[(128 + GOGP_RT(m) * 16 + fk + 4 * v) * ld + 128 + GOGP_CT(n) * 16 + fr];
      asm volatile("" ::: "memory");
#pragma unroll
      for (int m = 0; m < 2; ++m)
#pragma unroll
        for (int n = 0; n < 4; ++n)
#pragma unroll
          for (int v = 0; v < 4; ++v) {
            const int i = GOGP_RT(m) * 16 + fk + 4 * v, cc = GOGP_CT(n) * 16 + fr;
            S[i * SLD + cc] = (cc <= i) ? a11[m][n][v] - c[m][n][v] : 0.0;
          }
      __syncthreads();
    }
    GOGP_STAMP(half * 8 + 1);
    if (DO_POTRF) {
      potrf128_lds(S, G, rinv_s, tid, row0 + off, nvalid, info,
                   (STAMP && half == 0) ? stamps + 19 : nullptr);
      GOGP_STAMP(half * 8 + 2);
#pragma unroll 2
      for (int idx = tid; idx < 128 * 64; idx += NT) {
        const int i = idx >> 6, cc = (idx & 63) * 2;
        *reinterpret_cast<f64x2 *>(Lout + (off + i) * ldl + off + cc) =
            *reinterpret_cast<const f64x2 *>(S + i * SLD + cc);
        if (half == 0)
          *reinterpret_cast<f64x2 *>(Lout + i * ldl + 128 + cc) = (f64x2){0.0, 0.0};
      }
    } else {
      inv16<false>(S, w, G + w * 16 * XLD, rinv_s + w * 16, lane);
    }
    __syncthreads();
    GOGP_STAMP(half * 8 + 3);
    invert128_lds(S, G, tid);
    GOGP_STAMP(half * 8 + 4);
#pragma unroll 2
    for (int idx = tid; idx < 128 * 64; idx += NT) {
      const int i = idx >> 6, cc = (idx & 63) * 2;
      *reinterpret_cast<f64x2 *>(Dinv + (off + i) * LDD + off + cc) =
          *reinterpret_cast<const f64x2 *>(S + i * SLD + cc);
      if (half == 0) *reinterpret_cast<f64x2 *>(Dinv + i * LDD + 128 + cc) = (f64x2){0.0, 0.0};
    }
    __syncthreads();
    GOGP_STAMP(half * 8 + 5);
    if (half == 0) {
      if (DO_POTRF) {
        wg_gemm128<true, TRI_A>(c, S, G, A + 128 * ld, ld, tid);
        GOGP_STAMP(27);
#pragma unroll
        for (int m = 0; m < 2; ++m)
#pragma unroll
          for (int n = 0; n < 4; ++n)
#pragma unroll
            for (int v = 0; v < 4; ++v) {
              const int i = GOGP_RT(m) * 16 + fk + 4 * v, j = GOGP_CT(n) * 16 + fr;
              S[j * SLD + i] = c[m][n][v];
            }
        __syncthreads();
#pragma unroll 2
        for (int idx = tid; idx < 128 * 64; idx += NT) {
          const int i = idx >> 6, cc = (idx & 63) * 2;
          *reinterpret_cast<f64x2 *>(Lout + (128 + i) * ldl + cc) =
              *reinterpret_cast<const f64x2 *>(S + i * SLD + cc);
        }
      }
    }
  }
  GOGP_STAMP(16);
  wg_gemm128<false, TRI_A>(c, S, G, L10g, ld10, tid);
  GOGP_STAMP(17);
#pragma unroll
  for (int m = 0; m < 2; ++m)
#pragma unroll
    for (int n = 0; n < 4; ++n)
#pragma unroll
      for (int v = 0; v < 4; ++v)
        S[(GOGP_RT(m) * 16 + fk + 4 * v) * SLD + GOGP_CT(n) * 16 + fr] = c[m][n][v];
  __syncthreads();
  wg_gemm128<false, TRI_B>(c, S, G, Dinv, LDD, tid);
#pragma unroll
  for (int m = 0; m < 2; ++m)
#pragma unroll
    for (int n = 0; n < 4; ++n)
#pragma unroll
      for (int v = 0; v < 4; ++v)
        Dinv[(128 + GOGP_RT(m) * 16 + fk + 4 * v) * LDD + GOGP_CT(n) * 16 + fr] = -c[m][n][v];
  GOGP_STAMP(18);
}

template <bool DO_POTRF, bool STAMP, int LDD>
__global__ __launch_bounds__(NT) void diag256_kernel(const double *__restrict__ A, long ld,
                                                       double *__restrict__ Lout, long ldl,
                                                       double *__restrict__ Dinv, long row0,
                                                       long nvalid, long long *info,
                                                       unsigned long long *stamps, long bstride) {
  A = gogp::cand(A, bstride);
  if (Lout) Lout = gogp::cand(Lout, bstride);
  Dinv = gogp::cand(Dinv, bstride);
  if (info) info = gogp::cand(info, bstride);
  __shared__ __attribute__((aligned(16))) double S[128 * SLD];
  __shared__ __attribute__((aligned(16))) double G[GSIZE];
  __shared__ double rinv_s[8 * 16];
#ifdef GOGP_WGSTAMP
  unsigned long long *wgst = STAMP ? nullptr : stamps;
  if (wgst && threadIdx.x == 0) {
    wgst[blockIdx.z * 8 + 0] = __builtin_amdgcn_s_memrealtime();
    wgst[blockIdx.z * 8 + 4] = __builtin_amdgcn_s_getreg((4 << 0) | (0 << 6) | (31 << 11));
    wgst[blockIdx.z * 8 + 5] = __builtin_amdgcn_s_getreg((20 << 0) | (0 << 6) | (31 << 11));
  }
#endif
  diag256_body<DO_POTRF, STAMP, LDD>(S, G, rinv_s, A, ld, Lout, ldl, Dinv, row0, nvalid, info, stamps);
#ifdef GOGP_WGSTAMP
  if (wgst) {
    __builtin_amdgcn_s_waitcnt(0x0F70);
    __syncthreads();
    if (threadIdx.x == 0) wgst[blockIdx.z * 8 + 3] = __builtin_amdgcn_s_memrealtime();
  }
#endif
}

__global__ __launch_bounds__(NT) void dinv256_blocks_kernel(const double *__restrict__ L, long ld, double *__restrict__ Dinv,
                                                             long bstride) {
  L = gogp::cand(L, bstride);
  Dinv = gogp::cand(Dinv, bstride);
  __shared__ __attribute__((aligned(16))) double S[128 * SLD];
  __shared__ __attribute__((aligned(16))) double G[GSIZE];
  __shared__ double rinv_s[8 * 16];
  const long b = blockIdx.x;
  diag256_body<false, false, 256>(S, G, rinv_s, L + b * 256 * (ld + 1), ld, nullptr, 0L, Dinv + b * 65536L, 0L, 0L, nullptr,
                                  nullptr);
}

#define GOGP_EV 0
#define GOGP_EVN(name) name
#endif

__global__ __launch_bounds__(NT) void GOGP_EVN(tiny_eval_kernel)(const DevParams *__restrict__ Pp, const double *__restrict__ X,
                                                        const double *__restrict__ y, long n, double *__restrict__ A,
                                                        double *__restrict__ Lout, double *__restrict__ Dinv,
                                                        double *__restrict__ z, double *__restrict__ alpha,
                                                        long long *info, int want_kinv, long bstride) {
  const DevParams &P = *gogp::cand(Pp, bstride);
  A = gogp::cand(A, bstride);
  Lout = gogp::cand(Lout, bstride);
  Dinv = gogp::cand(Dinv, bstride);
  z = gogp::cand(z, bstride);
  alpha = gogp::cand(alpha, bstride);
  info = gogp::cand(info, bstride);
  const int tid = threadIdx.x;
  if (blockIdx.x != 0) {
    const int q = blockIdx.x, r0 = (q >= 2) ? 128 : 0, c0 = (q & 1) ? 128 : 0;
    for (int idx = tid; idx < 128 * 64; idx += NT) {
      const int i = idx >> 6, cc = (idx & 63) * 2;
      const f64x2 v = {(q == 3 && cc == i) ? 1.0 : 0.0, (q == 3 && cc + 1 == i) ? 1.0 : 0.0};
      *reinterpret_cast<f64x2 *>(Lout + (long)(r0 + i) * 256 + c0 + cc) = v;
      *reinterpret_cast<f64x2 *>(Dinv + (long)(r0 + i) * 256 + c0 + cc) = v;
      if (want_kinv) *reinterpret_cast<f64x2 *>(A + (long)(r0 + i) * 256 + c0 + cc) = v;
    }
    if (q == 3)
      for (int i = tid; i < 128; i += NT) z[128 + i] = alpha[128 + i] = 0.0;
    return;
  }
  __shared__ __attribute__((aligned(16))) double S[128 * SLD];
  __shared__ __attribute__((aligned(16))) double G[GSIZE];
  __shared__ double rinv_s[8 * 16];
  __shared__ double ys[128], zs[128];
  __shared__ unsigned long long em[GOGP_EV ? 128 : 1];
  const int D = P.ndim;
  if (GOGP_EV) {
    if (tid < 128) em[tid] = event_mask(P, tid < n ? X[(long)tid * D + P.ev_axis] : 0.0);
    __syncthreads();
  }
  for (int idx = tid; idx < 128 * 128; idx += NT) {
    const int i = idx >> 7, j = idx & 127;
    double k = 0.0;
    if (j <= i) {
      if (i < n) {
        const double *xi = X + (long)i * D, *xj = X + (long)j * D;
        k = simil_value(P, [&](int d) { return xi[d]; }, [&](int d) { return xj[d]; });
        if (GOGP_EV) k *= event_discount(P, em[i], em[j]);
        if (i == j) k += P.noise_var;
      } else {
        k = (i == j) ? 1.0 : 0.0;
      }
    }
    S[i * SLD + j] = k;
  }
  if (tid < 128) ys[tid] = tid < n ? y[tid] : 0.0;
  __syncthreads();
  potrf128_lds(S, G, rinv_s, tid, 0, n, info);
  for (int idx = tid; idx < 128 * 64; idx += NT) {
    const int i = idx >> 6, cc = (idx & 63) * 2;
    *reinterpret_cast<f64x2 *>(Lout + (long)i * 256 + cc) = *reinterpret_cast<const f64x2 *>(S + i * SLD + cc);
  }
  __syncthreads();
  invert128_lds(S, G, tid);
  for (int idx = tid; idx < 128 * 64; idx += NT) {
    const int i = idx >> 6, cc = (idx & 63) * 2;
    *reinterpret_cast<f64x2 *>(Dinv + (long)i * 256 + cc) = *reinterpret_cast<const f64x2 *>(S + i * SLD + cc);
  }
  {
    const int i = tid >> 2, p = tid & 3;
    double a = 0.0;
    for (int k = p; k <= i; k += 4) a += S[i * SLD + k] * ys[k];
    a += __shfl_xor(a, 1);
    a += __shfl_xor(a, 2);
    if (p == 0) {
      zs[i] = a;
      z[i] = a;
    }
  }
  __syncthreads();
  {
    const int j = tid >> 2, p = tid & 3;
    double a = 0.0;
    for (int k = j + p; k < 128; k += 4) a += S[k * SLD + j] * zs[k];
    a += __shfl_xor(a, 1);
    a += __shfl_xor(a, 2);
    if (p == 0) alpha[j] = a;
  }
  if (!want_kinv) return;
  __syncthreads();
  for (int idx = tid; idx < 128 * 128; idx += NT) {
    const int i = idx >> 7, j = idx & 127;
    if (j < i) {
      const double v = S[i * SLD + j];
      S[j * SLD + i] = v;
      S[i * SLD + j] = 0.0;
    }
  }
  __syncthreads();
  f64x4 c[2][4];
  wg_gemm128<true, TRI_SYM>(c, S, G, nullptr, 0, tid);
  const int lane = tid & 63, w = tid >> 6;
  const int fr = lane & 15, fk = lane >> 4;
  const int wr = w >> 1, wc = w & 1;
#pragma unroll
  for (int m = 0; m < 2; ++m)
#pragma unroll
    for (int nn = 0; nn < 4; ++nn)
      if (GOGP_CT(nn) <= GOGP_RT(m)) {
#pragma unroll
        for (int v = 0; v < 4; ++v) {
          const long i = GOGP_RT(m) * 16 + fk + 4 * v, j = GOGP_CT(nn) * 16 + fr;
          A[i * 256 + j] = c[m][nn][v];
          A[j * 256 + i] = c[m][nn][v];
        }
      }
}

template <int ARD_D, bool PRODUCE, bool FULL = false>
__global__ __launch_bounds__(NT) void GOGP_EVN(batch_eval_kernel)(const BatchItem *__restrict__ items,
                                                          const double *__restrict__ X, const double *__restrict__ y,
                                                          const double *__restrict__ Z, double *__restrict__ rows,
                                                          double *__restrict__ mu, double *__restrict__ sigma,
                                                          int ard_dims) {
  const BatchItem &it = items[blockIdx.x];
  const DevParams &P = it.P;
  const int D = P.ndim;
  const long n = it.n;
  if (FULL) {
    X += it.off;
    y = X + n * D;
  } else {
    X += it.off * D;
    y += it.off;
  }
  double *row = FULL ? rows + it.roff : rows + (long)blockIdx.x * BATCH_ROW;
  __shared__ __attribute__((aligned(16))) double S[128 * SLD];
  __shared__ __attribute__((aligned(16))) double G[GSIZE];
  __shared__ double rinv_s[8 * 16];
  __shared__ double ys[128], zs[128];
  __shared__ double sc[2][3];
  __shared__ long long info_s;
  __shared__ unsigned long long em[GOGP_EV ? 128 : 1];
  const int tid = threadIdx.x;
  const int lane = tid & 63, w = tid >> 6;
  if (tid == 0) info_s = 0;
  if (GOGP_EV) {
    if (tid < 128) em[tid] = event_mask(P, tid < n ? X[(long)tid * D + P.ev_axis] : 0.0);
    __syncthreads();
  }
  for (int idx = tid; idx < 128 * 128; idx += NT) {
    const int i = idx >> 7, j = idx & 127;
// ... 343 lines not shown
```

### gogp_amd/csrc/handle.h

```cpp
#pragma once
#include <algorithm>
#include <array>
#include <string>
#include <vector>

#include "common.h"

namespace gogp {
struct Dist2D;
}
using gogp::DevParams;
using gogp::GemmProfile;

constexpr int REFINE_SLABS = 8;

constexpr int HS_INFO = 8;
constexpr int HS_TRACE = 9;
constexpr int HS_TMO = 10;
constexpr int HS_PIVOT = 12;
constexpr int HS_GRAD = 16;
static_assert(HS_INFO < HS_TMO && HS_TMO < HS_PIVOT && HS_PIVOT < HS_GRAD, "the staging words lie below the gradient's sums");
static_assert(HS_GRAD + gogp::NACC == gogp::BATCH_ROW, "the pinned row is a batch row");

struct EvalBufs {
  DevParams *devP = nullptr;
  long long *info = nullptr;
  double *scalars = nullptr;
  double *gout = nullptr;
  double *bufA = nullptr, *bufL = nullptr, *bufY = nullptr, *Dinv = nullptr;
  double *z = nullptr, *w = nullptr, *alpha = nullptr;
  double *gpart = nullptr;
};

struct NBufs {
  double *dX = nullptr, *dy = nullptr, *bufA = nullptr, *bufL = nullptr, *Dinv = nullptr;
  double *z = nullptr, *w = nullptr, *alpha = nullptr, *gpart = nullptr;
};

struct gogp_handle;
struct Workspace {
  void *p = nullptr;
  size_t bytes = 0;
  inline int reserve(gogp_handle *h, size_t need);
  void release() {
    (void)hipFree(p);
    p = nullptr;
    bytes = 0;
  }
  template <class T>
  T *as() const { return static_cast<T *>(p); }
};

struct EvalState {
  bool factored = false, have_alpha = false, have_kinv = false;
  bool observed = false, with_obs = false;
  bool grad_valid = false;
  bool trtri_done = false;
  double lml = 0.0;
  double logdet2 = 0.0;
  double cond_lb = 1.0;
  int64_t notpd = -1;
};

struct CandGraphKey {
  int k = 0;
  int64_t n = 0, cap_npad = 0;
  size_t stride = 0;
  const void *arena = nullptr, *dX = nullptr, *dy = nullptr, *hostP = nullptr, *hscal = nullptr;
  bool operator==(const CandGraphKey &o) const {
    return k == o.k && n == o.n && cap_npad == o.cap_npad && stride == o.stride && arena == o.arena && dX == o.dX &&
           dy == o.dy && hostP == o.hostP && hscal == o.hscal;
  }
};

struct gogp_handle : EvalBufs, EvalState {
  gogp_desc desc;
  int device = 0;
  int ns = 0, nn = 0, P = 0, D = 0;
  int ard_dims = 0;
  bool radial1 = false;
  int nevents = 0, ev_axis = 0;
  double events[GOGP_MAX_EVENTS][3] = {};
  bool ev() const { return nevents > 0; }
  int64_t n = 0, npad = 0;
  int nblk = 0;
  double *dX = nullptr, *dy = nullptr;
  double *dscr = nullptr;
  double *D64 = nullptr;
  int64_t cap_d64 = 0;
  int diag_fp64 = 1;
  bool d64_active = false;
  int prec = 64;
  size_t esz() const { return prec == 32 ? sizeof(float) : sizeof(double); }
  int refine_steps = 1;
  double *rw = nullptr, *rz = nullptr, *rd = nullptr, *rpart = nullptr;
  DevParams *hostP = nullptr;
  double *hscal = nullptr;
  int64_t cap_npad = 0;
  int64_t cap_y = 0;
  double *dZ = nullptr, *KsT = nullptr, *Vt = nullptr, *pvec = nullptr;
  int64_t cap_m = 0, cap_mp_npad = 0;
  Workspace pg_ws;
  Workspace pc_ws;
  int ncu = 0;
  hipStream_t s = nullptr;
  hipStream_t sp = nullptr;
  char *cand_arena = nullptr;
  size_t cand_stride = 0;
  int cand_cap_k = 0;
  int64_t cand_cap_npad = 0;
  DevParams *cand_hostP = nullptr;
  double *cand_hscal = nullptr;
  int cand_host_k = 0;
  int batch_k = 1;
  bool batch_mode = false;
  int use_graph = 1;
  bool graph_failed = false;
  int graph_nodes = 0;
  std::string graph_note;
  hipGraphExec_t cand_graph = nullptr;
  hipStream_t sg = nullptr;
  CandGraphKey cand_graph_key, cand_seen_key;
  double *bt_X = nullptr, *bt_y = nullptr;
  int64_t bt_rows = 0, bt_cap_rows = 0;
  std::vector<int64_t> bt_off, bt_n;
  bool bt_have = false;
  char *bt_din = nullptr, *bt_hin = nullptr;
  size_t bt_in_cap = 0;
  double *bt_dout = nullptr, *bt_hout = nullptr;
  size_t bt_out_cap = 0;
  gogp::Dist2D *dist = nullptr;
  hipStream_t sl = nullptr;
  hipStream_t s2 = nullptr;
  hipStream_t st = nullptr;
  hipStream_t sk = nullptr;
  void *stream_set = nullptr;
  std::vector<hipEvent_t> evs;
  int lookahead = 1;
  int superpanel = 2;
  int eager = 1;
  int superpanel_head = -1;
  int head_remaining = 16;
  int chain_prio = -1;
  int tiny = 1;
  int chain_slabs = 0;
  int chain_split = -1;
  int ktri = 1;
  double *TX = nullptr, *Tmt = nullptr;
  int64_t tinv_ld = 0;
  size_t cap_tinv = 0;
  int grad_prec = 64;
  float *g32A = nullptr, *g32L = nullptr, *g32Y = nullptr, *g32D = nullptr;
  int64_t g32_cap = 0;
  int produce_panels = 4;
  int produce_small_below = 1024;
  int produce_tinv = 1;
  bool tinv_valid = false, tinv_pending = false;
  int64_t tinv_sig = 0;
  int produce_small_max = 64;
  Workspace small_ws;
  int produce_groups = 2;
  int krag = 1;
  int ard_mfma_min = 1;
  int kinv_split = 60;
  int64_t kinv_c1 = 0;
  int kinv_fused = -1;
  bool kinv_pending = false;
  bool trtri_pending = false;
  bool ydone_valid = false;
  bool alpha_pending = false;
  std::vector<double> theta_s, theta_n;
  bool have_data = false;
  bool have_theta = false;
  bool z_valid = false;
  Workspace app_ws;
  Workspace rm_ws;
  Workspace loo_vec;
  Workspace loo_mat;
  int multi_T = 0;
  bool multi_solved = false;
  Workspace multi_vec;
  Workspace multi_mean;
  Workspace multi_mat;
  double yta = 0.0;
  int trace_fp64 = 1;
  double cond_limit = 1e16;
  std::vector<double> grad_cache;
  std::string err;
  GemmProfile prof;
  std::vector<hipEvent_t> aux_ev[GOGP_PROF_NCLASS];
  size_t aux_used[GOGP_PROF_NCLASS] = {0, 0, 0, 0};
};

struct AuxTimer {
  gogp_handle *h;
  int cls;
  hipStream_t s;
  hipEvent_t e1 = nullptr;
  AuxTimer(gogp_handle *h_, int cls_, hipStream_t s_) : h(h_), cls(cls_), s(s_) {
    if (!h->prof.on || cls < 0 || cls >= GOGP_PROF_NCLASS) return;
    auto &pool = h->aux_ev[cls];
    size_t &used = h->aux_used[cls];
    while (pool.size() < used + 2) {
      hipEvent_t e = nullptr;
      (void)hipEventCreate(&e);
      pool.push_back(e);
    }
    (void)hipEventRecord(pool[used], s);
    e1 = pool[used + 1];
    used += 2;
  }
  ~AuxTimer() {
    if (e1) (void)hipEventRecord(e1, s);
  }
};

#define HIPCHK(h, call)                                                                \
  do {                                                                                 \
    hipError_t e_ = (call);                                                            \
    if (e_ != hipSuccess) {                                                            \
      char buf_[512];                                                                  \
      snprintf(buf_, sizeof buf_, "%s failed: %s (%s:%d)", #call, hipGetErrorString(e_), \
               __FILE__, __LINE__);                                                    \
      (h)->err = buf_;                                                                 \
      (void)hipGetLastError();  \
      return (e_ == hipErrorOutOfMemory) ? GOGP_ENOMEM : GOGP_EHIP;                     \
    }                                                                                  \
  } while (0)

inline int Workspace::reserve(gogp_handle *h, size_t need) {
  if (p && bytes >= need) return GOGP_OK;
  release();
  HIPCHK(h, hipMalloc(&p, need));
  bytes = need;
  return GOGP_OK;
}

static inline unsigned *hs_tmo(const gogp_handle *h) { return reinterpret_cast<unsigned *>(h->hscal + HS_TMO); }

static inline void nbufs_free(const NBufs &b) {
  for (double *q : {b.dX, b.dy, b.bufA, b.bufL, b.Dinv, b.z, b.w, b.alpha, b.gpart}) (void)hipFree(q);
}
static inline hipError_t nbufs_alloc(const gogp_handle *h, int64_t cap, NBufs *b) {
  const size_t nn = (size_t)cap * (size_t)cap * h->esz(), vec = (size_t)cap * sizeof(double);
  hipError_t e = hipMalloc(&b->dX, ((size_t)cap * h->D + GOGP_MAX_NDIM) * sizeof(double));
  if (e == hipSuccess) e = hipMalloc(&b->dy, vec);
  if (e == hipSuccess) e = hipMalloc(&b->bufA, nn);
  if (e == hipSuccess) e = hipMalloc(&b->bufL, nn);
  if (e == hipSuccess) e = hipMalloc(&b->Dinv, (size_t)(cap / gogp::PANEL) * gogp::PANEL * gogp::PANEL * h->esz());
  if (e == hipSuccess) e = hipMalloc(&b->z, vec);
  if (e == hipSuccess) e = hipMalloc(&b->w, vec);
  if (e == hipSuccess) e = hipMalloc(&b->alpha, vec);
  if (e == hipSuccess) e = hipMalloc(&b->gpart, (size_t)gogp::grad_reduce_blocks(cap) * gogp::NACC * sizeof(double));
  if (e != hipSuccess) {
    nbufs_free(*b);
    *b = NBufs();
  }
  return e;
}
static inline NBufs nbufs_of(const gogp_handle *h) {
  NBufs b;
  b.dX = h->dX, b.dy = h->dy, b.bufA = h->bufA, b.bufL = h->bufL, b.Dinv = h->Dinv;
  b.z = h->z, b.w = h->w, b.alpha = h->alpha, b.gpart = h->gpart;
  return b;
}
static inline void nbufs_put(gogp_handle *h, const NBufs &b) {
  h->dX = b.dX, h->dy = b.dy, h->bufA = b.bufA, h->bufL = b.bufL, h->Dinv = b.Dinv;
  h->z = b.z, h->w = b.w, h->alpha = b.alpha, h->gpart = b.gpart;
}

static inline std::array<hipStream_t, 6> work_streams(const gogp_handle *h) {
  return {h->s, h->sp, h->s2, h->st, h->sl, h->sk};
}

static inline int fail(gogp_handle *h, int code, const char *msg) {
  if (h) h->err = msg;
  return code;
}

enum { EV_GRAM = 0, EV_FWD = 1, EV_ALPHA = 2, EV_INIT = 3, EV_TRTRI = 4, EV_W = 5, EV_ENTRY = 6, EV_KINV = 7,
       EV_YDONE = 8,
       EV_TINV = 9,
       EV_BASE = 10 };
static inline hipEvent_t ev(gogp_handle *h, size_t i) {
  while (h->evs.size() <= i) {
    hipEvent_t e = nullptr;
    (void)hipEventCreateWithFlags(&e, hipEventDisableTiming);
    h->evs.push_back(e);
  }
  return h->evs[i];
}
static inline void order(gogp_handle *h, size_t i, hipStream_t from, hipStream_t to) {
  hipEvent_t e = ev(h, i);
  (void)gogp::rec_event_record(e, from);
  (void)gogp::rec_stream_wait(to, e);
}


// ... 11 lines not shown
```

### gogp_amd/csrc/testhooks.hip

```cpp
#include <cstdlib>
#include <cstring>
#include <stdio.h>

#include "common.h"
#include "gemm_plan.h"
#include "../../include/gogp_testhooks.h"

struct gogp_handle;
namespace gogp {
int dist_init_replay(gogp_handle *h, int rank, int nranks, int prow, int pcol);
}
extern "C" int gogp_test_dist_init_replay(void *h, int rank, int nranks, int prow, int pcol) {
  return gogp::dist_init_replay(static_cast<gogp_handle *>(h), rank, nranks, prow, pcol);
}

namespace gogp_th {
void launch_diag256(hipStream_t s, const double *A, int64_t ld, double *Lout, int64_t ldl,
                    double *Dinv, int64_t row0, int64_t nvalid, long long *info);
void launch_diag256_stamped(hipStream_t s, const double *A, double *Lout, double *Dinv,
                            long long *info, unsigned long long *stamps);
void launch_panel128_stamped(hipStream_t s, const double *A, double *Lout, int64_t rows_below, long long *info,
                             unsigned long long *stamps);
}

// ... 174 lines not shown
  if (e == hipSuccess) e = hipMemcpy(dC, C, (size_t)M * N * sizeof(double), hipMemcpyHostToDevice);
  if (e == hipSuccess) {
    launch_dgemm_nt(0, GEMM_RECT, (int)(M / TILE), (int)(N / TILE), K, alpha, dA, K, dB, K, beta,
                    dC, N, nullptr);
    e = hipDeviceSynchronize();
  }
  if (e == hipSuccess) e = hipMemcpy(C, dC, (size_t)M * N * sizeof(double), hipMemcpyDeviceToHost);
  (void)hipFree(dA);
  (void)hipFree(dB);
  (void)hipFree(dC);
  return e == hipSuccess ? GOGP_OK : GOGP_EHIP;
}

namespace {
bool covers(int64_t len, int64_t off, int64_t ld, int64_t rows, int64_t cols, int64_t k, int64_t stride) {
  if (len <= 0 || off < 0 || ld < cols || rows <= 0 || cols <= 0 || k <= 0 || stride < 0) return false;
  const int64_t hi = off + (k - 1) * stride + (rows - 1) * ld + cols;
  return hi <= len;
}
bool device_ok(int device) {
  int ndev = 0;
  if (hipGetDeviceCount(&ndev) != hipSuccess || ndev <= 0) return false;
  return device < 0 || hipSetDevice(device) == hipSuccess;
}
bool gemm_launch_args_ok(int precision, int mode, int mt, int nt, int64_t K, const gogp_test_gemm_opts &o) {
  if (precision != 64 && precision != 32) return false;
  if (mode < GEMM_RECT || mode > GEMM_TRAP || mt <= 0 || nt <= 0 || K <= 0) return false;
  const int64_t kstep = precision == 64 ? GEMM_BK : SGEMM_BK, al = 16 / (precision / 8);
  if (K % kstep || K > (1 << 30)) return false;
  if ((mode == GEMM_LOWER || mode == GEMM_LAUUM) && mt != nt) return false;
  if (o.k < 1 || o.k > 64 || o.bstride < 0 || o.bstride % al || (o.k > 1 && o.bstride == 0)) return false;
  if (precision == 32 && (o.k > 1 || o.kbeg0 != 0)) return false;
  if (o.kbeg0 < 0 || o.kbeg0 % kstep || o.kbeg0 > K || (o.kbeg0 && mode != GEMM_LAUUM)) return false;
  if (o.new_row0 < -1 || (o.new_row0 >= 0 && mode != GEMM_LOWER)) return false;
  if (o.ktri && mode != GEMM_RECT) return false;
  if (o.krag0 < -1 || (o.krag0 >= 0 && (o.ktri || (mode != GEMM_RECT && mode != GEMM_LOWER)))) return false;
  if (o.krag0 >= 0 && o.krag0 < mt && K < (int64_t)(mt - o.krag0) * TILE) return false;
  if (o.rule < 0 || o.rule > 2 || (o.rule && mode != GEMM_RECT)) return false;
  if (o.rule && (o.tpb_shift < 0 || o.tpb_shift > 8 || o.rblk0 < 0 || o.cblk0 < 0 || o.Pr < 1 || o.Pc < 1 ||
                 o.pr < 0 || o.pr >= o.Pr || o.pc < 0 || o.pc >= o.Pc))
    return false;
  return true;
}
const gogp_test_gemm_opts GEMM_OPTS_DEFAULT = {0, -1, -1, 0, 384, 0, 0, 0, 0, 0, 0, 1, 0, 1, -1, 1, 0};
GemmGrid gemm_grid_of(const gogp_test_gemm_opts &o) {
  GemmGrid g;
  g.ktri = o.ktri;
  g.krag0 = o.krag0;
  g.new_row0 = o.new_row0;
  g.kbeg0 = o.kbeg0;
  g.small_below = o.small_below;
  g.prio = o.prio;
  g.rule = o.rule;
  g.tpb_shift = o.tpb_shift;
  g.rblk0 = o.rblk0;
  g.cblk0 = o.cblk0;
  g.pr = o.pr;
  g.Pr = o.Pr;
  g.pc = o.pc;
  g.Pc = o.Pc;
  g.beta0 = o.beta0;
  return g;
}
}

extern "C" int gogp_test_gemm_plan(int precision, int mode, int mt, int nt, int64_t K, const gogp_test_gemm_opts *opt,
                                   gogp_test_gemm_plan_out *out) {
  const gogp_test_gemm_opts o = opt ? *opt : GEMM_OPTS_DEFAULT;
  if (!out || !gemm_launch_args_ok(precision, mode, mt, nt, K, o)) return GOGP_EARG;
  const GemmGrid g = gemm_grid_of(o);
  const GemmPlan p = gemm_plan((GemmMode)mode, mt, nt, K, &g, o.k, precision == 64 ? GEMM_F64 : GEMM_F32);
  out->tile = p.tile;
  out->waves = p.waves;
  out->grid_x = p.gridx;
  out->grid_z = p.gridz;
  out->flops = p.flops;
  out->tag = p.tag;
  return GOGP_OK;
}

extern "C" int gogp_test_gemm_nt(int device, int precision, int mode, int mt, int nt, int64_t K, double alpha,
                                 double beta, const void *A, int64_t a_len, int64_t a_off, int64_t lda, const void *B,
                                 int64_t b_len, int64_t b_off, int64_t ldb, void *C, int64_t c_len, int64_t c_off,
                                 int64_t ldc, const gogp_test_gemm_opts *opt) {
  const gogp_test_gemm_opts o = opt ? *opt : GEMM_OPTS_DEFAULT;
  if (!A || !B || !C || !gemm_launch_args_ok(precision, mode, mt, nt, K, o)) return GOGP_EARG;
  const int64_t es = precision / 8, al = 16 / es;
  if (alpha == 0.0 || (precision == 32 && (float)alpha == 0.0f)) return GOGP_EARG;
  if (lda % al || ldb % al || ldc % al || a_off % al || b_off % al || c_off % al) return GOGP_EARG;
  const int64_t M = (int64_t)mt * TILE, N = (int64_t)nt * TILE;
  if (!covers(a_len, a_off, lda, M, K, o.k, o.bstride) || !covers(b_len, b_off, ldb, N, K, o.k, o.bstride) ||
      !covers(c_len, c_off, ldc, M, N, o.k, o.bstride))
    return GOGP_EARG;
  if (!device_ok(device)) return GOGP_EHIP;

  char *dA = nullptr, *dB = nullptr, *dC = nullptr;
  hipError_t e = hipMalloc(&dA, (size_t)(a_len * es));
  if (e == hipSuccess) e = hipMalloc(&dB, (size_t)(b_len * es));
  if (e == hipSuccess) e = hipMalloc(&dC, (size_t)(c_len * es));
  if (e == hipSuccess) e = hipMemcpy(dA, A, (size_t)(a_len * es), hipMemcpyHostToDevice);
  if (e == hipSuccess) e = hipMemcpy(dB, B, (size_t)(b_len * es), hipMemcpyHostToDevice);
  if (e == hipSuccess) e = hipMemcpy(dC, C, (size_t)(c_len * es), hipMemcpyHostToDevice);
  if (e == hipSuccess) {
    const GemmGrid g = gemm_grid_of(o);
    tl_batch.k = o.k;
    tl_batch.stride = (long)(o.bstride * es);
    if (precision == 64)
      launch_gemm_nt(0, (GemmMode)mode, mt, nt, K, alpha, (const double *)dA + a_off, lda, (const double *)dB + b_off, ldb,
                     beta, (double *)dC + c_off, ldc, nullptr, &g);
    else
      launch_gemm_nt(0, (GemmMode)mode, mt, nt, K, alpha, (const float *)dA + a_off, lda, (const float *)dB + b_off, ldb,
                     beta, (float *)dC + c_off, ldc, nullptr, &g);
    tl_batch.k = 1;
    tl_batch.stride = 0;
    e = hipGetLastError();
    if (e == hipSuccess) e = hipDeviceSynchronize();
  }
  if (e == hipSuccess) e = hipMemcpy(C, dC, (size_t)(c_len * es), hipMemcpyDeviceToHost);
  (void)hipFree(dA);
  (void)hipFree(dB);
  (void)hipFree(dC);
  return e == hipSuccess ? GOGP_OK : GOGP_EHIP;
}

extern "C" int gogp_test_diag_syrk(int device, int bs, const float *L, int64_t l_len, int64_t l_off, int64_t ld,
                                   int64_t K, int64_t row_stride, double *D64, int64_t d_len, int nblocks) {
  if (!L || !D64 || (bs != PANEL && bs != 2 * PANEL) || nblocks < 1 || nblocks > 4096) return GOGP_EARG;
  if (K < 16 || K % 16 || ld % 4 || l_off % 4 || row_stride % 4) return GOGP_EARG;
  if (bs == PANEL && row_stride != PANEL * ld) return GOGP_EARG;
  if (!covers(l_len, l_off, ld, bs, K, nblocks, row_stride) || d_len < (int64_t)nblocks * bs * bs) return GOGP_EARG;
  if (!device_ok(device)) return GOGP_EHIP;
  float *dL = nullptr;
  double *dD = nullptr;
  hipError_t e = hipMalloc(&dL, (size_t)l_len * sizeof(float));
  if (e == hipSuccess) e = hipMalloc(&dD, (size_t)d_len * sizeof(double));
  if (e == hipSuccess) e = hipMemcpy(dL, L, (size_t)l_len * sizeof(float), hipMemcpyHostToDevice);
  if (e == hipSuccess) e = hipMemcpy(dD, D64, (size_t)d_len * sizeof(double), hipMemcpyHostToDevice);
  if (e == hipSuccess) {
    if (bs == PANEL)
      launch_diag_syrk_f64(0, dL + l_off, ld, K, dD, nblocks);
    else
      launch_diag_syrk_f64_tiles(0, dL + l_off, ld, K, dD, nblocks, row_stride, bs);
    e = hipGetLastError();
    if (e == hipSuccess) e = hipDeviceSynchronize();
  }
  if (e == hipSuccess) e = hipMemcpy(D64, dD, (size_t)d_len * sizeof(double), hipMemcpyDeviceToHost);
  (void)hipFree(dL);
  (void)hipFree(dD);
  return e == hipSuccess ? GOGP_OK : GOGP_EHIP;
}

extern "C" int gogp_test_diag256_product(int device, int variant, const double *A, int64_t ld, double *L, int64_t ldl,
                                         double *Dinv, int64_t row0, int64_t nvalid, long long *info) {
  if (!A || !L || !Dinv || !info || variant < 0 || variant > 3) return GOGP_EARG;
  if (ld < PANEL || ldl < PANEL || ld % 2 || ldl % 2 || row0 < 0 || nvalid < 0) return GOGP_EARG;
  const int64_t ldd = (variant & 1) ? 2 * PANEL : PANEL;
  if (!device_ok(device)) return GOGP_EHIP;
  double *dA = nullptr, *dL = nullptr, *dD = nullptr;
  long long *dinfo = nullptr;
  const size_t na = (size_t)PANEL * ld * 8, nl = (size_t)PANEL * ldl * 8, nd = (size_t)PANEL * ldd * 8;
  hipError_t e = hipMalloc(&dA, na);
  if (e == hipSuccess) e = hipMalloc(&dL, nl);
  if (e == hipSuccess) e = hipMalloc(&dD, nd);
  if (e == hipSuccess) e = hipMalloc(&dinfo, 8);
  if (e == hipSuccess) e = hipMemcpy(dA, A, na, hipMemcpyHostToDevice);
  if (e == hipSuccess) e = hipMemcpy(dL, L, nl, hipMemcpyHostToDevice);
  if (e == hipSuccess) e = hipMemcpy(dD, Dinv, nd, hipMemcpyHostToDevice);
  if (e == hipSuccess) e = hipMemcpy(dinfo, info, 8, hipMemcpyHostToDevice);
  if (e == hipSuccess) {
    switch (variant) {
      case 0: launch_diag256(0, dA, ld, dL, ldl, dD, row0, nvalid, dinfo); break;
      case 1: launch_diag256_ld512(0, dA, ld, dL, ldl, dD, row0, nvalid, dinfo); break;
      case 2: launch_diag256_inv_only(0, dA, ld, dD); break;
      default: launch_diag256_inv_only_ld512(0, dA, ld, dD); break;
    }
    e = hipGetLastError();
    if (e == hipSuccess) e = hipDeviceSynchronize();
  }
  if (e == hipSuccess) e = hipMemcpy(L, dL, nl, hipMemcpyDeviceToHost);
  if (e == hipSuccess) e = hipMemcpy(Dinv, dD, nd, hipMemcpyDeviceToHost);
  if (e == hipSuccess) e = hipMemcpy(info, dinfo, 8, hipMemcpyDeviceToHost);
  (void)hipFree(dA); (void)hipFree(dL); (void)hipFree(dD); (void)hipFree(dinfo);
  return e == hipSuccess ? GOGP_OK : GOGP_EHIP;
}

extern "C" int gogp_test_diag256(int device, const double *A, double *Lout, double *Dinv,
                                 unsigned long long *stamps, double *elapsed_us) {
  if (!A || !Lout || !Dinv || !stamps) return GOGP_EARG;
  int ndev = 0;
  if (hipGetDeviceCount(&ndev) != hipSuccess || ndev <= 0) return GOGP_EHIP;
  if (device >= 0 && hipSetDevice(device) != hipSuccess) return GOGP_EHIP;
  double *dA = nullptr, *dL = nullptr, *dD = nullptr;
  long long *dinfo = nullptr;
  unsigned long long *dst = nullptr;
  const size_t nb = 256 * 256 * sizeof(double);
  hipError_t e = hipMalloc(&dA, nb);
  if (e == hipSuccess) e = hipMalloc(&dL, nb);
  if (e == hipSuccess) e = hipMalloc(&dD, nb);
  if (e == hipSuccess) e = hipMalloc(&dinfo, 8);
  if (e == hipSuccess) e = hipMalloc(&dst, 32 * 8);
  if (e == hipSuccess) e = hipMemcpy(dA, A, nb, hipMemcpyHostToDevice);
  if (e == hipSuccess) e = hipMemset(dinfo, 0, 8);
  if (e == hipSuccess) e = hipMemset(dst, 0, 32 * 8);
  hipEvent_t e0, e1;
  (void)hipEventCreate(&e0);
  (void)hipEventCreate(&e1);
  float ms = 0.f;
  if (e == hipSuccess) {
    gogp_th::launch_diag256_stamped(0, dA, dL, dD, dinfo, dst);
    (void)hipDeviceSynchronize();
    (void)hipEventRecord(e0, 0);
    gogp::launch_diag256(0, dA, 256, dL, 256, dD, 0, 256, dinfo);
    (void)hipEventRecord(e1, 0);
    (void)hipEventSynchronize(e1);
    (void)hipEventElapsedTime(&ms, e0, e1);
    gogp_th::launch_diag256_stamped(0, dA, dL, dD, dinfo, dst);
    e = hipDeviceSynchronize();
  }
  if (e == hipSuccess) e = hipMemcpy(Lout, dL, nb, hipMemcpyDeviceToHost);
  if (e == hipSuccess) e = hipMemcpy(Dinv, dD, nb, hipMemcpyDeviceToHost);
  if (e == hipSuccess) e = hipMemcpy(stamps, dst, 32 * 8, hipMemcpyDeviceToHost);
  if (elapsed_us) *elapsed_us = ms * 1e3;
  (void)hipFree(dA); (void)hipFree(dL); (void)hipFree(dD); (void)hipFree(dinfo); (void)hipFree(dst);
  (void)hipEventDestroy(e0); (void)hipEventDestroy(e1);
  return e == hipSuccess ? GOGP_OK : GOGP_EHIP;
}

__global__ __launch_bounds__(64) void valu_cost_kernel(double *out, double seed) {
  double x = seed + 1e-9 * threadIdx.x, y = 1.0000001, z = 0.9999999;
  double a0 = x, a1 = x + 1, a2 = x + 2, a3 = x + 3, a4 = x + 4, a5 = x + 5, a6 = x + 6, a7 = x + 7;
  unsigned long long t[9];
#define GOGP_T(k) t[k] = __builtin_amdgcn_s_memtime(); asm volatile("s_waitcnt lgkmcnt(0)" ::: "memory")
#define REP8(X) X X X X X X X X
#define REP64(X) REP8(REP8(X))
  GOGP_T(0);
  asm volatile(REP64("v_fma_f64 %0, %0, %1, %2\n\t") : "+v"(a0) : "v"(y), "v"(z));
  GOGP_T(1);
  asm volatile(REP8("v_fma_f64 %0, %0, %8, %9\n\tv_fma_f64 %1, %1, %8, %9\n\tv_fma_f64 %2, %2, %8, %9\n\tv_fma_f64 %3, %3, %8, %9\n\t"
                    "v_fma_f64 %4, %4, %8, %9\n\tv_fma_f64 %5, %5, %8, %9\n\tv_fma_f64 %6, %6, %8, %9\n\tv_fma_f64 %7, %7, %8, %9\n\t")
               : "+v"(a0), "+v"(a1), "+v"(a2), "+v"(a3), "+v"(a4), "+v"(a5), "+v"(a6), "+v"(a7) : "v"(y), "v"(z));
  GOGP_T(2);
  asm volatile(REP64("s_nop 1\n\tv_mov_b64_dpp %0, %0 row_newbcast:3 row_mask:0xf bank_mask:0xf bound_ctrl:1\n\t") : "+v"(a0));
  GOGP_T(3);
  asm volatile(REP8("v_mov_b64_dpp %0, %8 row_newbcast:1 row_mask:0xf bank_mask:0xf bound_ctrl:1\n\t"
                    "v_mov_b64_dpp %1, %8 row_newbcast:2 row_mask:0xf bank_mask:0xf bound_ctrl:1\n\t"
                    "v_mov_b64_dpp %2, %8 row_newbcast:3 row_mask:0xf bank_mask:0xf bound_ctrl:1\n\t"
                    "v_mov_b64_dpp %3, %8 row_newbcast:4 row_mask:0xf bank_mask:0xf bound_ctrl:1\n\t"
                    "v_mov_b64_dpp %4, %8 row_newbcast:5 row_mask:0xf bank_mask:0xf bound_ctrl:1\n\t"
                    "v_mov_b64_dpp %5, %8 row_newbcast:6 row_mask:0xf bank_mask:0xf bound_ctrl:1\n\t"
                    "v_mov_b64_dpp %6, %8 row_newbcast:7 row_mask:0xf bank_mask:0xf bound_ctrl:1\n\t"
                    "v_mov_b64_dpp %7, %8 row_newbcast:8 row_mask:0xf bank_mask:0xf bound_ctrl:1\n\t")
               : "+v"(a0), "+v"(a1), "+v"(a2), "+v"(a3), "+v"(a4), "+v"(a5), "+v"(a6), "+v"(a7) : "v"(y));
  GOGP_T(4);
  asm volatile(REP64("v_rsq_f64 %0, %0\n\t") : "+v"(a0));
  GOGP_T(5);
  asm volatile(REP8("v_rsq_f64 %0, %8\n\tv_rsq_f64 %1, %8\n\tv_rsq_f64 %2, %8\n\tv_rsq_f64 %3, %8\n\t"
                    "v_rsq_f64 %4, %8\n\tv_rsq_f64 %5, %8\n\tv_rsq_f64 %6, %8\n\tv_rsq_f64 %7, %8\n\t")
               : "+v"(a0), "+v"(a1), "+v"(a2), "+v"(a3), "+v"(a4), "+v"(a5), "+v"(a6), "+v"(a7) : "v"(y));
  GOGP_T(6);
  asm volatile(REP64("v_mul_f64 %0, %0, %1\n\t") : "+v"(a1) : "v"(y));
  GOGP_T(7);
  asm volatile(REP64("s_nop 1\n\tv_mov_b64_dpp %1, %0 row_newbcast:3 row_mask:0xf bank_mask:0xf bound_ctrl:1\n\tv_fma_f64 %0, %1, %2, %0\n\t")
               : "+v"(a2), "+v"(a3) : "v"(y));
  GOGP_T(8);
#undef GOGP_T
#undef REP8
#undef REP64
  if (threadIdx.x == 0)
    for (int k = 0; k < 8; ++k) out[k] = (double)(t[k + 1] - t[k]) / 64.0;
  out[8 + threadIdx.x] = a0 + a1 + a2 + a3 + a4 + a5 + a6 + a7;
}
extern "C" int gogp_test_valu_cost(int device, double *out8) {
  if (!out8) return GOGP_EARG;
  int ndev = 0;
  if (hipGetDeviceCount(&ndev) != hipSuccess || ndev <= 0) return GOGP_EHIP;
  if (device >= 0 && hipSetDevice(device) != hipSuccess) return GOGP_EHIP;
  double *d = nullptr;
  if (hipMalloc(&d, (8 + 64) * sizeof(double)) != hipSuccess) return GOGP_ENOMEM;
  for (int rep = 0; rep < 3; ++rep) hipLaunchKernelGGL(valu_cost_kernel, dim3(1), dim3(64), 0, 0, d, 1.5);
  hipError_t e = hipDeviceSynchronize();
  if (e == hipSuccess) e = hipMemcpy(out8, d, 8 * sizeof(double), hipMemcpyDeviceToHost);
  (void)hipFree(d);
  return e == hipSuccess ? GOGP_OK : GOGP_EHIP;
}

extern "C" int gogp_test_panel128(int device, const double *A, double *Lout, int64_t rows_below, int reps,
                                  unsigned long long *stamps, double *elapsed_us) {
  if (!A || !Lout || !stamps || rows_below < 0 || rows_below % 64 || reps <= 0) return GOGP_EARG;
  int ndev = 0;
  if (hipGetDeviceCount(&ndev) != hipSuccess || ndev <= 0) return GOGP_EHIP;
  if (device >= 0 && hipSetDevice(device) != hipSuccess) return GOGP_EHIP;
  double *dA = nullptr, *dL = nullptr;
  long long *dinfo = nullptr;
  unsigned long long *dst = nullptr;
  const size_t rows = 128 + (size_t)rows_below, nb = rows * 128 * sizeof(double), nb2 = rows * 256 * sizeof(double);
  hipError_t e = hipMalloc(&dA, nb + nb2);
  if (e == hipSuccess) e = hipMalloc(&dL, nb + nb2);
  if (e == hipSuccess) e = hipMalloc(&dinfo, 8);
  if (e == hipSuccess) e = hipMalloc(&dst, 72 * 8);
  if (e == hipSuccess) e = hipMemcpy(dA, A, nb, hipMemcpyHostToDevice);
  if (e == hipSuccess) e = hipMemcpy2D(dA + rows * 128, 256 * sizeof(double), A, 128 * sizeof(double), 128 * sizeof(double), rows,
                                       hipMemcpyHostToDevice);
  if (e == hipSuccess) e = hipMemset(dinfo, 0, 8);
  if (e == hipSuccess) e = hipMemset(dst, 0, 72 * 8);
  hipEvent_t e0, e1;
  (void)hipEventCreate(&e0);
  (void)hipEventCreate(&e1);
  float ms = 0.f;
  if (e == hipSuccess) {
    double *A2 = dA + rows * 128, *L2 = dL + rows * 128;
    gogp::launch_panel128(0, A2, 256, L2, 256, 0, rows_below, 0, (int64_t)rows, dinfo);
    (void)hipDeviceSynchronize();
    (void)hipEventRecord(e0, 0);
    for (int r = 0; r < reps; ++r) gogp::launch_panel128(0, A2, 256, L2, 256, 0, rows_below, 0, (int64_t)rows, dinfo);
    (void)hipEventRecord(e1, 0);
    (void)hipEventSynchronize(e1);
    (void)hipEventElapsedTime(&ms, e0, e1);
    gogp_th::launch_panel128_stamped(0, dA, dL, rows_below, dinfo, dst);
    (void)hipDeviceSynchronize();
    gogp_th::launch_panel128_stamped(0, dA, dL, rows_below, dinfo, dst);
    e = hipDeviceSynchronize();
  }
  if (e == hipSuccess) e = hipMemcpy(Lout, dL, nb, hipMemcpyDeviceToHost);
  if (e == hipSuccess) e = hipMemcpy(stamps, dst, 72 * 8, hipMemcpyDeviceToHost);
  if (elapsed_us) *elapsed_us = ms * 1e3 / reps;
  (void)hipFree(dA); (void)hipFree(dL); (void)hipFree(dinfo); (void)hipFree(dst);
  (void)hipEventDestroy(e0); (void)hipEventDestroy(e1);
  return e == hipSuccess ? GOGP_OK : GOGP_EHIP;
}

extern "C" int gogp_test_panel128_slabs(int device, const double *A, double *Lout, int64_t rows_below, int slabs, int reps,
                                        double *elapsed_us) {
  if (!A || !Lout || rows_below < 0 || rows_below % 64 || slabs < 0 || slabs > 8 || reps <= 0) return GOGP_EARG;
  int ndev = 0;
  if (hipGetDeviceCount(&ndev) != hipSuccess || ndev <= 0) return GOGP_EHIP;
// ... 786 lines not shown
```

### gogp_amd/gp.py

```python
from __future__ import annotations

import ctypes
import operator
from typing import List, Optional, Sequence

import numpy as np

from . import _lib
from .kernel import NoiseKernel, SimilKernel, build_desc


class GogpError(RuntimeError):
    def __init__(self, code: int, msg: str):
        super().__init__("gogp_hip error %d: %s" % (code, msg))
        self.code = code


class FactorizeError(GogpError):

    def __init__(self, msg: str, pivot: int):
        super().__init__(_lib.GOGP_ENOTPD, msg)
        self.pivot = pivot


# ... 556 lines not shown
        self.Priors = Priors
        self._x = None

    def Observe(self, x) -> float:
        self._x = _arr(x).reshape(-1).copy()
        if self._x.size != self.gp._ns + self.gp._nn:
            raise ValueError("len(x): the LOO objective takes the hyperparameters only")
        self.gp.Observe(self._x)
        v = self.gp.LOOScore()
        return v + self.Priors.Observe(self._x) if self.Priors is not None else v

    def Gradient(self) -> np.ndarray:
        g = self.gp.LOOGradient()
        if self.Priors is not None:
            self.Priors.Observe(self._x)
            pg = np.asarray(self.Priors.Gradient(), dtype=float)
            g[:len(pg)] += pg
        return g


class MultiModel:

    def __init__(self, gp: GP, Priors=None):
        self.gp = gp
        self.Priors = Priors
        self._x = None

    def Observe(self, x) -> float:
        self._x = _arr(x).reshape(-1).copy()
        if self._x.size != self.gp._ns + self.gp._nn:
            raise ValueError("len(x): the multi-output objective takes the hyperparameters only")
        self.gp.Observe(self._x)
        v = self.gp.MultiLML()[0]
        return v + self.Priors.Observe(self._x) if self.Priors is not None else v

    def Gradient(self) -> np.ndarray:
        g = self.gp.MultiGradient()
        if self.Priors is not None:
            self.Priors.Observe(self._x)
            pg = np.asarray(self.Priors.Gradient(), dtype=float)
            g[:len(pg)] += pg
        return g


def mfma_f64_peak(iters: int = 20000, device: int = -1, details: bool = False):
    v, c, m = ctypes.c_double(0.0), ctypes.c_double(0.0), ctypes.c_double(0.0)
    rc = _lib.hooks().gogp_mfma_f64_peak(device, iters, ctypes.byref(v), ctypes.byref(c),
                                       ctypes.byref(m))
    if rc != _lib.GOGP_OK:
        raise GogpError(rc, "mfma_f64_peak")
    return (v.value, c.value, m.value) if details else v.value


def mfma_f32_peak(iters: int = 20000, device: int = -1, details: bool = False):
    v, c, m = ctypes.c_double(0.0), ctypes.c_double(0.0), ctypes.c_double(0.0)
    rc = _lib.hooks().gogp_mfma_f32_peak(device, iters, ctypes.byref(v), ctypes.byref(c), ctypes.byref(m))
    if rc != _lib.GOGP_OK:
        raise GogpError(rc, "mfma_f32_peak")
    return (v.value, c.value, m.value) if details else v.value


def dgemm_nt_check(A: np.ndarray, B: np.ndarray, C: np.ndarray, alpha=1.0, beta=0.0,
                  device: int = -1) -> np.ndarray:
    A, B = _arr(A), _arr(B)
    out = _arr(C).copy()
    M, K = A.shape
    N = B.shape[0]
    rc = _lib.hooks().gogp_test_dgemm_nt(device, M, N, K, alpha, _dp(A), _dp(B), beta, _dp(out))
    if rc != _lib.GOGP_OK:
        raise GogpError(rc, "test_dgemm_nt")
    return out


def diag256_check(A: np.ndarray, device: int = -1):
    A = _arr(A)
    assert A.shape == (256, 256)
    L, X = np.zeros((256, 256)), np.zeros((256, 256))
    st = (ctypes.c_uint64 * 32)()
    us = ctypes.c_double(0.0)
    rc = _lib.hooks().gogp_test_diag256(device, _dp(A), _dp(L), _dp(X), st, ctypes.byref(us))
    if rc != _lib.GOGP_OK:
        raise GogpError(rc, "test_diag256")
    return L, X, np.array(list(st), dtype=np.uint64), us.value


def bench_gemm(mode: int, mt: int, nt: int, K: int, reps: int = 5, device: int = -1):
    ms, tf = ctypes.c_double(0.0), ctypes.c_double(0.0)
    rc = _lib.hooks().gogp_bench_gemm(device, mode, mt, nt, K, reps, ctypes.byref(ms), ctypes.byref(tf))
    if rc != _lib.GOGP_OK:
        raise GogpError(rc, "bench_gemm")
    return ms.value, tf.value


GEMM_MODES = {"RECT": 0, "LOWER": 1, "LAUUM": 2, "TRAP": 3}


def _covers(n, off, ld, rows, cols, k, stride, what):
    if off < 0 or ld < cols or stride < 0 or off + (k - 1) * stride + (rows - 1) * ld + cols > n:
        raise ValueError("%s: %d elements do not cover off %d, ld %d, %d x %d, %d slots %d apart"
                         % (what, n, off, ld, rows, cols, k, stride))


def gemm_nt_check(mode, mt: int, nt: int, K: int, A: np.ndarray, B: np.ndarray, C: np.ndarray, alpha=1.0, beta=0.0,
                  lda=None, ldb=None, ldc=None, a_off=0, b_off=0, c_off=0, device: int = -1, **opts) -> np.ndarray:
    mode = GEMM_MODES.get(mode, mode)
    arrs = []
    for a in (A, B, C):
        if not isinstance(a, np.ndarray) or a.dtype not in (np.float64, np.float32) or not a.flags.c_contiguous:
            raise TypeError("operands: C-contiguous float64 / float32 arrays")
        arrs.append(a)
    if len({a.dtype for a in arrs}) != 1:
        raise TypeError("A, B and C must share one dtype")
    prec = 64 if A.dtype == np.float64 else 32
    lda = A.shape[-1] if lda is None else lda
    ldb = B.shape[-1] if ldb is None else ldb
    ldc = C.shape[-1] if ldc is None else ldc
    o = dict(_lib.CGemmOpts.DEFAULTS)
    unknown = set(opts) - set(o)
    if unknown:
        raise TypeError("unknown options %s" % sorted(unknown))
    o.update(opts)
    k, bstride = o["k"], o["bstride"]
    rows_b = mt if mode in (1, 2) else nt
    _covers(A.size, a_off, lda, mt * 128, K, k, bstride, "A")
    _covers(B.size, b_off, ldb, rows_b * 128, K, k, bstride, "B")
    _covers(C.size, c_off, ldc, mt * 128, nt * 128, k, bstride, "C")
    out = C.copy()
    copt = _lib.CGemmOpts(**o)
    rc = _lib.hooks().gogp_test_gemm_nt(device, prec, mode, mt, nt, K, alpha, beta,
                                        A.ctypes.data, A.size, a_off, lda, B.ctypes.data, B.size, b_off, ldb,
                                        out.ctypes.data, out.size, c_off, ldc, ctypes.byref(copt))
    if rc != _lib.GOGP_OK:
        raise GogpError(rc, "test_gemm_nt")
    return out


def diag_syrk_check(L: np.ndarray, D64: np.ndarray, K: int, nblocks: int, bs: int = 256, ld=None, l_off: int = 0,
                    row_stride=None, device: int = -1) -> np.ndarray:
    if L.dtype != np.float32 or D64.dtype != np.float64 or not (L.flags.c_contiguous and D64.flags.c_contiguous):
        raise TypeError("L: float32, D64: float64, both C-contiguous")
    ld = L.shape[-1] if ld is None else ld
    row_stride = bs * ld if row_stride is None else row_stride
    _covers(L.size, l_off, ld, bs, K, nblocks, row_stride, "L")
    if D64.size < nblocks * bs * bs:
        raise ValueError("D64 holds fewer than %d blocks" % nblocks)
    out = D64.copy()
    rc = _lib.hooks().gogp_test_diag_syrk(device, bs, L.ctypes.data, L.size, l_off, ld, K, row_stride, _dp(out),
                                          out.size, nblocks)
    if rc != _lib.GOGP_OK:
        raise GogpError(rc, "test_diag_syrk")
    return out


def diag256_product(A: np.ndarray, variant: int = 0, row0: int = 0, nvalid: int = 256, L=None, Dinv=None,
                    device: int = -1):
    A = _arr(A)
    if A.ndim != 2 or A.shape[0] != 256 or A.shape[1] < 256:
        raise ValueError("A: 256 rows of at least 256")
    L = np.zeros((256, 256)) if L is None else _arr(L).copy()
    ldd = 512 if variant in (1, 3) else 256
    Dinv = np.zeros((256, ldd)) if Dinv is None else _arr(Dinv).copy()
    if L.ndim != 2 or L.shape[0] != 256 or L.shape[1] < 256 or Dinv.shape != (256, ldd):
        raise ValueError("L: 256 rows of at least 256, Dinv: 256 x %d" % ldd)
    info = ctypes.c_longlong(0)
    rc = _lib.hooks().gogp_test_diag256_product(device, variant, _dp(A), A.shape[1], _dp(L), L.shape[1], _dp(Dinv),
                                                row0, nvalid, ctypes.byref(info))
    if rc != _lib.GOGP_OK:
        raise GogpError(rc, "test_diag256_product")
    return L, Dinv, info.value


def _mat(a, what):
    if not isinstance(a, np.ndarray) or a.dtype not in (np.float64, np.float32) or not a.flags.c_contiguous:
        raise TypeError("%s: a C-contiguous float64 / float32 array" % what)
    return a


def _prec(*arrs):
    if len({a.dtype for a in arrs}) != 1:
        raise TypeError("the matrices must share one dtype")
    return 64 if arrs[0].dtype == np.float64 else 32


def _vec(a, what):
    if not isinstance(a, np.ndarray) or a.dtype != np.float64 or not a.flags.c_contiguous:
        raise TypeError("%s: a C-contiguous float64 array" % what)
    return a


def trsm_small_workspace(npad: int) -> int:
    n = _lib.hooks().gogp_test_trsm_small_workspace(npad)
    if n < 0:
        raise GogpError(_lib.GOGP_EARG, "test_trsm_small_workspace")
    return int(n)


def trsm_small_check(npad: int, L: np.ndarray, ld: int, Dinv: np.ndarray, KsT: np.ndarray, ldk: int, j0: int, cnt: int,
                     dq: np.ndarray, ws=None, device: int = -1):
    L, Dinv, KsT = _mat(L, "L"), _mat(Dinv, "Dinv"), _mat(KsT, "KsT")
    prec = _prec(L, Dinv, KsT)
    if Dinv.size != npad * 256:
        raise ValueError("Dinv: npad / 256 blocks of 256 x 256")
    dq = _vec(dq, "dq").copy()
    nbytes = trsm_small_workspace(npad)
    ws = np.zeros(nbytes, np.uint8) if ws is None else np.ascontiguousarray(ws, dtype=np.uint8).copy()
    kind, width, tmo, off = ctypes.c_int(-1), ctypes.c_int(-1), ctypes.c_uint(0), ctypes.c_int64(-1)
    rc = _lib.hooks().gogp_test_trsm_small(device, prec, npad, L.ctypes.data, L.size, ld, Dinv.ctypes.data,
                                           KsT.ctypes.data, KsT.size, ldk, j0, cnt, _dp(dq), dq.size, ws.ctypes.data,
                                           ws.size, ctypes.byref(kind), ctypes.byref(width), ctypes.byref(off),
                                           ctypes.byref(tmo))
    if rc != _lib.GOGP_OK:
        raise GogpError(rc, "test_trsm_small")
    return dq, ws, kind.value, width.value, off.value, tmo.value


def trsv_steps_check(direction: str, npad: int, L: np.ndarray, ld: int, Dinv: np.ndarray, b0: int, b1: int,
                     w: np.ndarray, out: np.ndarray, k: int = 1, bstride: int = 0, device: int = -1):
    L, Dinv = _mat(L, "L"), _mat(Dinv, "Dinv")
    prec = _prec(L, Dinv)
    if Dinv.size != (k - 1) * bstride + npad * 256:
        raise ValueError("Dinv: (k - 1) * bstride + npad * 256 elements")
    w, out = _vec(w, "w").copy(), _vec(out, "out").copy()
    rc = _lib.hooks().gogp_test_trsv_steps(device, prec, {"fwd": 0, "bwd": 1}[direction], npad, L.ctypes.data, L.size,
                                           ld, Dinv.ctypes.data, b0, b1, k, bstride, _dp(w), w.size, _dp(out), out.size)
    if rc != _lib.GOGP_OK:
        raise GogpError(rc, "test_trsv_steps")
    return w, out


def alpha_from_y_check(npad: int, Y: np.ndarray, ld: int, z: np.ndarray, alpha: np.ndarray, device: int = -1):
    Y, z, alpha = _mat(Y, "Y"), _vec(z, "z"), _vec(alpha, "alpha").copy()
    rc = _lib.hooks().gogp_test_alpha_from_y(device, _prec(Y), npad, Y.ctypes.data, Y.size, ld, _dp(z), z.size,
                                             _dp(alpha), alpha.size)
    if rc != _lib.GOGP_OK:
        raise GogpError(rc, "test_alpha_from_y")
    return alpha


def rownorm_dot_check(V: np.ndarray, ld: int, ncols: int, m: int, vec=None, dot=None, sq=None, device: int = -1):
    V = _mat(V, "V")
    vec = None if vec is None else _vec(vec, "vec")
    dot = None if dot is None else _vec(dot, "dot").copy()
    sq = None if sq is None else _vec(sq, "sq").copy()
    size = lambda a: 0 if a is None else a.size
    rc = _lib.hooks().gogp_test_rownorm_dot(device, _prec(V), V.ctypes.data, V.size, ld, ncols, m, _dp(vec), size(vec),
                                            _dp(dot), size(dot), _dp(sq), size(sq))
    if rc != _lib.GOGP_OK:
        raise GogpError(rc, "test_rownorm_dot")
    return dot, sq


def tinv_check(nsub: int, Dinv: np.ndarray, X: np.ndarray, tld: int, XT=None, device: int = -1):
    Dinv, X = _mat(Dinv, "Dinv"), _mat(X, "X").copy()
    arrs = [Dinv, X]
    if XT is not None:
        XT = _mat(XT, "XT").copy()
        arrs.append(XT)
        if XT.size != X.size:
            raise ValueError("XT: as many elements as X")
    if Dinv.size != nsub * 65536:
        raise ValueError("Dinv: nsub blocks of 256 x 256")
    rc = _lib.hooks().gogp_test_tinv(device, _prec(*arrs), nsub, Dinv.ctypes.data, X.ctypes.data, X.size, tld,
                                     int(XT is not None), None if XT is None else XT.ctypes.data)
    if rc != _lib.GOGP_OK:
        raise GogpError(rc, "test_tinv")
    return X, XT


def blockmm_check(arena: np.ndarray, prods, alpha: float = 1.0, k: int = 1, bstride: int = 0, device: int = -1):
    arena = _mat(arena, "arena").copy()
    n = len(prods)
    cols = [(ctypes.c_int64 * max(n, 1))(*[int(p[i]) for p in prods]) for i in range(6)]
    K = (ctypes.c_int * max(n, 1))(*[int(p[6]) for p in prods])
    rc = _lib.hooks().gogp_test_blockmm(device, _prec(arena), n, arena.ctypes.data, arena.size, *cols, K, alpha, k,
                                        bstride)
    if rc != _lib.GOGP_OK:
        raise GogpError(rc, "test_blockmm")
    return arena


NACC = _lib.GOGP_TEST_NACC
ACC_TRACE, ACC_ARD0 = 12, 16


def kparams(ndim: int, terms, noise_var: float = 0.0, dnoise: float = 0.0, events=(), ev_axis: int = 0):
    if not 1 <= ndim <= 64 or not 1 <= len(terms) <= 4 or len(events) > 32:
        raise ValueError("kparams: 1..64 dimensions, 1..4 terms, at most 32 events")
    p = _lib.CKParams()
    p.ndim, p.nterms, p.noise_var, p.dnoise, p.nevents, p.ev_axis = ndim, len(terms), noise_var, dnoise, len(events), ev_axis
    for t, T in enumerate(terms):
        p.kind[t], p.ard[t], p.c[t], p.w[t] = int(T["kind"]), int(bool(T.get("ard"))), T.get("c", 1.0), T.get("w", 0.0)
        il = np.broadcast_to(np.asarray(T.get("inv_len", 1.0), float), (ndim,))
        for d in range(ndim):
            p.inv_len[t][d] = il[d]
    for e, (frm, to, disc) in enumerate(events):
        p.ev_from[e], p.ev_to[e], p.ev_disc[e] = frm, to, disc
    return p


def grad_blocks(npad: int, max_blocks: int = 0, mrows: int = 0, ncols: int = 0) -> int:
    b = _lib.hooks().gogp_test_grad_blocks(npad, mrows, ncols, max_blocks)
    if b < 0:
        raise GogpError(_lib.GOGP_EARG, "test_grad_blocks")
    return int(b)


# ... 164 lines not shown
```

### include/gogp_testhooks.h

```cpp
#ifndef GOGP_TESTHOOKS_H
#define GOGP_TESTHOOKS_H

#include <stdint.h>

#include "gogp_hip.h"

#ifdef __cplusplus
extern "C" {
#endif

int gogp_mfma_f64_peak(int device, int iters, double *tflops, double *cyc_per_mfma,
                       double *clock_mhz);
int gogp_mfma_f32_peak(int device, int iters, double *tflops, double *cyc_per_mfma,
                       double *clock_mhz);

int gogp_test_dgemm_nt(int device, int64_t M, int64_t N, int64_t K, double alpha,
                       const double *A, const double *B, double beta, double *C);

typedef struct gogp_test_gemm_opts {
  int32_t ktri, krag0, new_row0, kbeg0, small_below, prio;
  int32_t rule, tpb_shift, rblk0, cblk0, pr, Pr, pc, Pc, beta0;
  int32_t k;
  int64_t bstride;
} gogp_test_gemm_opts;

int gogp_test_gemm_nt(int device, int precision, int mode, int mt, int nt, int64_t K, double alpha, double beta,
                      const void *A, int64_t a_len, int64_t a_off, int64_t lda, const void *B, int64_t b_len,
                      int64_t b_off, int64_t ldb, void *C, int64_t c_len, int64_t c_off, int64_t ldc,
                      const gogp_test_gemm_opts *opt);

typedef struct gogp_test_gemm_plan_out {
  int32_t tile, waves;
  int64_t grid_x, grid_z;
  double flops;
  int64_t tag;
} gogp_test_gemm_plan_out;
int gogp_test_gemm_plan(int precision, int mode, int mt, int nt, int64_t K, const gogp_test_gemm_opts *opt,
                        gogp_test_gemm_plan_out *out);

int gogp_test_diag_syrk(int device, int bs, const float *L, int64_t l_len, int64_t l_off, int64_t ld, int64_t K,
                        int64_t row_stride, double *D64, int64_t d_len, int nblocks);

int gogp_test_diag256_product(int device, int variant, const double *A, int64_t ld, double *L, int64_t ldl,
                              double *Dinv, int64_t row0, int64_t nvalid, long long *info);


int64_t gogp_test_trsm_small_workspace(int64_t npad);

int gogp_test_trsm_small(int device, int precision, int64_t npad, const void *L, int64_t l_len, int64_t ld,
                         const void *Dinv, const void *KsT, int64_t k_len, int64_t ldk, int j0, int cnt, double *dq,
                         int64_t dq_len, void *sol, int64_t sol_len, int *kind, int *width, int64_t *sol_off,
                         unsigned *tmo);

int gogp_test_trsv_steps(int device, int precision, int dir, int64_t npad, const void *L, int64_t l_len, int64_t ld,
                         const void *Dinv, int b0, int b1, int k, int64_t bstride, double *w, int64_t w_len, double *out,
                         int64_t out_len);

int gogp_test_alpha_from_y(int device, int precision, int64_t npad, const void *Y, int64_t y_len, int64_t ld,
                           const double *z, int64_t z_len, double *alpha, int64_t alpha_len);

int gogp_test_rownorm_dot(int device, int precision, const void *V, int64_t v_len, int64_t ld, int64_t ncols, int64_t m,
                          const double *vec, int64_t vec_len, double *dot, int64_t dot_len, double *sq, int64_t sq_len);

int gogp_test_tinv(int device, int precision, int nsub, const void *Dinv, void *X, int64_t x_len, int64_t tld, int with_xt,
                   void *XT);

int gogp_test_blockmm(int device, int precision, int nprod, void *arena, int64_t arena_len, const int64_t *a_off,
                      const int64_t *lda, const int64_t *b_off, const int64_t *ldb, const int64_t *c_off,
                      const int64_t *ldc, const int *K, double alpha, int k, int64_t bstride);


typedef struct gogp_test_kparams {
  int32_t ndim, nterms;
  int32_t kind[GOGP_MAX_TERMS], ard[GOGP_MAX_TERMS];
  double c[GOGP_MAX_TERMS], w[GOGP_MAX_TERMS], inv_len[GOGP_MAX_TERMS][GOGP_MAX_NDIM];
  double noise_var, dnoise;
  int32_t nevents, ev_axis;
  double ev_from[GOGP_MAX_EVENTS], ev_to[GOGP_MAX_EVENTS], ev_disc[GOGP_MAX_EVENTS];
} gogp_test_kparams;

#define GOGP_TEST_NACC (16 + GOGP_MAX_NDIM)

int gogp_test_grad_blocks(int64_t npad, int64_t mrows, int64_t ncols, int max_blocks);

int gogp_test_grad_reduce(int device, int precision, const gogp_test_kparams *kparams, int ard_dims, int radial1,
                          int mfma_min, int ev, const double *X, int64_t x_len, const double *alpha, int64_t alpha_len,
                          const void *Kinv, int64_t kinv_len, int64_t ld, int64_t n, int64_t npad, int max_blocks, int k,
                          int64_t bstride, double *partials, int64_t partials_len, double *out);

int gogp_test_grad_reduce_local(int device, int precision, const gogp_test_kparams *kparams, int ard_dims, int radial1,
                                int mfma_min, int ev, const double *X, int64_t x_len, const double *alpha,
                                int64_t alpha_len, const void *Kinv, int64_t kinv_len, int64_t ld, int64_t n, int64_t npad,
                                int64_t mrows, int64_t ncols, int nb_shift, int pr, int Pr, int pc, int Pc, int max_blocks,
                                int k, int64_t bstride, double *partials, int64_t partials_len, double *out);

int gogp_test_xgrad(int device, const gogp_test_kparams *kparams, int ev, const double *X, int64_t x_len,
                    const double *alpha, int64_t alpha_len, double *Kinv, int64_t kinv_len, int64_t ld, int64_t n,
                    int64_t npad, double *gx, int64_t gx_len);


int gogp_test_append_gram(int device, const void *sol0, int64_t sol0_len, int kind0, int width0, int64_t off0,
                          const void *sol1, int64_t sol1_len, int kind1, int width1, int64_t off1, int m0, int m,
                          int64_t npc, int64_t n, const double *z, int64_t z_len, double *part, int64_t part_len,
                          double *Lnew, int64_t lnew_len, int64_t ld);

int gogp_test_append_commit(int device, const gogp_test_kparams *kparams, int ev, const double *X2, int64_t x2_len,
                            const double *y2, int64_t y2_len, int m, int64_t n, const double *part, int64_t part_len,
                            int nslab, double *Lnew, int64_t lnew_len, int64_t ld, double *z2, int64_t z2_len,
                            long long *info);

int gogp_test_remove_gather(int device, const double *src, int64_t src_len, int64_t ld0, const int *map, int64_t map_len,
                            int64_t n1, double *dst, int64_t dst_len, int64_t npad1);

int gogp_test_remove_w(int device, const double *src, int64_t src_len, int64_t ld0, const int *map, int64_t map_len,
                       const int *rem, int64_t rem_len, int mc, int mw, int64_t r0, int64_t n1, int64_t npad1, double *W,
                       int64_t w_len);

int gogp_test_remove_block(int device, double *L, int64_t l_len, int64_t ld, int snap_b0, int snap_nb, double *snap,
                           int64_t snap_len, double *W, int64_t w_len, int mw, int64_t kb0, int64_t kb1, int64_t n1);

int gogp_test_bwd_panel(int device, int64_t rows16, const double *A, int64_t a_len, int64_t a_off, int64_t lda,
                        const double *B, int64_t b_len, int64_t b_off, int64_t ldb, double *C, int64_t c_len, int64_t c_off,
                        int64_t ldc, int64_t ncols, int64_t K, int tri, int sub);

int gogp_test_pcov_slabs(int64_t npad, int64_t m, int ncu, int *cols_per_slab);

int gogp_test_pcov(int device, const gogp_test_kparams *kparams, int ev, const double *Z, int64_t z_len, int64_t m,
                   const double *Vt, int64_t vt_len, int64_t ld, int64_t npad, int ncu, double *part, int64_t part_len,
                   double diag_add, double *out, int64_t out_len, int64_t mo, int64_t ldo);

int gogp_test_multi_weight(int device, const double *At, int64_t at_len, int64_t ld, int T, const double *Kinv,
                           int64_t kinv_len, int64_t ldk, int64_t n, int64_t npad, double *G, int64_t g_len);

int gogp_bench_gemm(int device, int mode, int mt, int nt, int64_t K, int reps,
                    double *ms_per_launch, double *tflops);

int gogp_test_diag256(int device, const double *A, double *Lout, double *Dinv,
                      unsigned long long *stamps, double *elapsed_us);

int gogp_test_valu_cost(int device, double *out8);

int gogp_test_panel128(int device, const double *A, double *Lout, int64_t rows_below, int reps,
                       unsigned long long *stamps, double *elapsed_us);

int gogp_test_panel128_slabs(int device, const double *A, double *Lout, int64_t rows_below, int slabs, int reps,
                             double *elapsed_us);

int gogp_test_dist_init_replay(void *h, int rank, int nranks, int prow, int pcol);

#ifdef __cplusplus
}
#endif
#endif
```

Measured before the change: 13.94.

## Add streaming 64-block diag256 factor/inverse kernel for large eager fp64 chains

Adds a new diag256 kernel that factors and inverts the 256x256 diagonal block by streaming 64x64 sub-blocks through a small LDS footprint with buffer loads and MFMA, instead of holding the whole block resident. It is selected by default for eager fp64 non-split chains with npad > 8192, except for the first superpanel and the last few panels. The intent is to shorten the serial diagonal step on the Cholesky critical path. The cost is extra global round-trips, which could make this one-workgroup step slower. The existing LDS helpers are templated on leading dimension and size, and a benchmarking test hook is added.

```diff
diff --git a/gogp_amd/_lib.py b/gogp_amd/_lib.py
--- a/gogp_amd/_lib.py
+++ b/gogp_amd/_lib.py
@@ -150,6 +150,9 @@
      [ctypes.c_int, ctypes.c_int, ctypes.c_void_p, _i64, _i64, _i64, _i64, _i64, _dp, _i64, ctypes.c_int]),
     ("gogp_test_diag256_product", ctypes.c_int,
      [ctypes.c_int, ctypes.c_int, _dp, _i64, _dp, _i64, _dp, _i64, _i64, ctypes.POINTER(ctypes.c_longlong)]),
+    ("gogp_test_diag256_cand", ctypes.c_int,
+     [ctypes.c_int, ctypes.c_int, ctypes.c_int, _dp, _i64, _dp, _i64, _dp, _i64, _i64,
+      ctypes.POINTER(ctypes.c_longlong), ctypes.c_int, _dp]),
     ("gogp_test_trsm_small_workspace", _i64, [_i64]),
     ("gogp_test_trsm_small", ctypes.c_int,
      [ctypes.c_int, ctypes.c_int, _i64, ctypes.c_void_p, _i64, _i64, ctypes.c_void_p, ctypes.c_void_p, _i64, _i64,
diff --git a/gogp_amd/csrc/api.hip b/gogp_amd/csrc/api.hip
--- a/gogp_amd/csrc/api.hip
+++ b/gogp_amd/csrc/api.hip
@@ -528,11 +528,14 @@
 }
 
 static void diag_block(gogp_handle *h, hipStream_t sp, const double *A, int64_t ld, double *L, int64_t ldl,
-                       double *Dp, int64_t c0) {
-  launch_diag256(sp, A, ld, L, ldl, Dp, c0, h->n, h->info);
+                       double *Dp, int64_t c0, bool resident) {
+  if (resident)
+    launch_diag256_resident(sp, A, ld, L, ldl, Dp, c0, h->n, h->info);
+  else
+    launch_diag256(sp, A, ld, L, ldl, Dp, c0, h->n, h->info);
 }
 static void diag_block(gogp_handle *h, hipStream_t sp, const float *A, int64_t ld, float *L, int64_t ldl,
-                       float *Dp, int64_t c0) {
+                       float *Dp, int64_t c0, bool ) {
   double *A64 = h->dscr, *L64 = h->dscr + PANEL * PANEL, *D64 = h->dscr + 2 * PANEL * PANEL;
   if (h->d64_active)
     A64 = h->D64 + (size_t)(c0 / PANEL) * PANEL * PANEL;
@@ -772,6 +775,15 @@
   if (h->chain_split >= 0) return h->chain_split;
   return (h->npad <= 8192 || !eager) ? 2 : 0;
 }
+constexpr int DIAG_RESIDENT_TAIL = 8;
+static inline bool diag_resident_of(const gogp_handle *h, bool eager, int split) {
+  if (h->dist || h->prec != 64 || split != 0) return false;
+  if (h->diag_resident >= 0) return h->diag_resident != 0;
+  return eager && h->npad > 8192;
+}
+static inline bool diag_resident_at(const gogp_handle *h, bool resident, int p, int npanel, int first_width) {
+  return resident && (h->diag_resident == 1 || (p >= first_width && p < npanel - DIAG_RESIDENT_TAIL));
+}
 static void fused_panel(gogp_handle *h, hipStream_t sp, double *A, double *L, int64_t ld, int64_t c0, int64_t npad,
                         GemmProfile *pf) {
   const int64_t c1 = c0 + TILE, c2 = c0 + PANEL;
@@ -832,6 +844,7 @@
   bool mixed = !fp32 && mixed_gradient(h);
   bool fuse_kinv = eager && (h->kinv_fused < 0 ? (npad <= 10240 || mixed) : h->kinv_fused != 0);
   int split = fp32 ? 0 : chain_split_of(h, eager);
+  bool resident = !fp32 && diag_resident_of(h, eager, split);
 
   void d64_init(hipStream_t q, int first, int nblk) const {
     if constexpr (fp32)
@@ -879,7 +892,8 @@
       }
       if (!split) {
         T *Dp = Dinv + (size_t)p * PANEL * PANEL;
-        diag_block(h, sp, A + c0 * ld + c0, ld, L + c0 * ld + c0, ld, Dp, c0);
+        diag_block(h, sp, A + c0 * ld + c0, ld, L + c0 * ld + c0, ld, Dp, c0,
+                   diag_resident_at(h, resident, p, npanel, superpanel_width(h, npanel, 0)));
         const int mt2 = (int)((npad - c2) / TILE);
         if (mt2 > 0) {
           GemmGrid gtri = chain_grid(h);
@@ -3132,6 +3146,11 @@
     h->chain_slabs = (int)value;
     return GOGP_OK;
   }
+  if (strcmp(name, "diag_resident") == 0) {
+    if (value < -1 || value > 1) return fail(h, GOGP_EARG, "diag_resident must be -1, 0 or 1");
+    h->diag_resident = (int)value;
+    return GOGP_OK;
+  }
   if (strcmp(name, "chain_split") == 0) {
     if (value < -1 || value > 2 || value == 1) return fail(h, GOGP_EARG, "chain_split must be -1, 0 or 2");
     h->chain_split = (int)value;
diff --git a/gogp_amd/csrc/common.h b/gogp_amd/csrc/common.h
--- a/gogp_amd/csrc/common.h
+++ b/gogp_amd/csrc/common.h
@@ -157,6 +157,8 @@
                         const double *y, const double *alpha, int64_t n, double *scalars);
 void launch_diag256(hipStream_t s, const double *A, int64_t ld, double *Lout, int64_t ldl,
                     double *Dinv, int64_t row0, int64_t nvalid, long long *info);
+void launch_diag256_resident(hipStream_t s, const double *A, int64_t ld, double *Lout, int64_t ldl,
+                             double *Dinv, int64_t row0, int64_t nvalid, long long *info);
 void launch_diag256_ld512(hipStream_t s, const double *A, int64_t ld, double *Lout, int64_t ldl,
                           double *Dinv, int64_t row0, int64_t nvalid, long long *info);
 void launch_diag256_inv_only(hipStream_t s, const double *L, int64_t ld, double *Dinv);
diff --git a/gogp_amd/csrc/diag256.hip b/gogp_amd/csrc/diag256.hip
--- a/gogp_amd/csrc/diag256.hip
+++ b/gogp_amd/csrc/diag256.hip
@@ -32,13 +32,14 @@
   return __builtin_amdgcn_mfma_f64_16x16x4f64(a, b, c, 0, 0, 0);
 }
 
+template <int LD = SLD, int N = 128>
 __device__ __forceinline__ void panel16(double *S, int kb, int lane, int row0, bool report,
                                         long grow0, long nvalid, long long *info,
                                         double (&keep)[16], double &keep_rinv) {
   const int r = lane & 15;
   const int prow = row0 + lane;
-  const double *srcd = S + (kb * 16 + r) * SLD + kb * 16;
-  double *srcp = S + (prow < 128 ? prow : 127) * SLD + kb * 16;
+  const double *srcd = S + (kb * 16 + r) * LD + kb * 16;
+  double *srcp = S + (prow < N ? prow : N - 1) * LD + kb * 16;
   double ap[16];
 #pragma unroll
   for (int c = 0; c < 16; c += 2) {
@@ -55,7 +56,7 @@
 #pragma unroll
   for (int c = 0; c < 16; ++c) asm volatile("" : "+v"(ap[c]));
   asm volatile("" : "+v"(mine));
-  if (row0 < 128) {
+  if (row0 < N) {
 #pragma unroll
     for (int c = 0; c < 16; c += 2) *reinterpret_cast<f64x2 *>(srcp + c) = (f64x2){ap[c], ap[c + 1]};
   }
@@ -64,32 +65,33 @@
     *info = (long long)(grow0 + bad + 1);
 }
 
+template <int LD = SLD>
 __device__ __forceinline__ void panel16_store_diag(double *S, int kb, double *rinv, int lane,
                                                    const double (&keep)[16], double keep_rinv) {
   if (lane < 16) {
-    double *dst = S + (kb * 16 + lane) * SLD + kb * 16;
+    double *dst = S + (kb * 16 + lane) * LD + kb * 16;
 #pragma unroll
     for (int c = 0; c < 16; ++c) dst[c] = (c <= lane) ? keep[c] : 0.0;
     rinv[lane] = keep_rinv;
   }
 }
 
-template <bool HAVE_RINV>
+template <bool HAVE_RINV, int LD = SLD>
 __device__ __forceinline__ void inv16(const double *S, int kb, double *Xb, const double *rinv,
                                       int lane) {
   const int r = lane & 15;
-  const double *Lb = S + (kb * 16) * SLD + kb * 16;
+  const double *Lb = S + (kb * 16) * LD + kb * 16;
   double x[16];
 #pragma unroll
   for (int rr = 0; rr < 16; ++rr) {
     double s = (rr == r) ? 1.0 : 0.0;
 #pragma unroll
-    for (int q = 0; q < rr; ++q) s -= Lb[rr * SLD + q] * x[q];
+    for (int q = 0; q < rr; ++q) s -= Lb[rr * LD + q] * x[q];
     double ri;
     if (HAVE_RINV) {
       ri = rinv[rr];
     } else {
-      const double d = Lb[rr * SLD + rr];
+      const double d = Lb[rr * LD + rr];
       ri = __builtin_amdgcn_rcp(d);
       ri = fma(ri, fma(-d, ri, 1.0), ri);
       ri = fma(ri, fma(-d, ri, 1.0), ri);
@@ -102,16 +104,17 @@
   }
 }
 
+template <int LD = SLD>
 __device__ __forceinline__ void tile_update16(double *S, int i, int c, int kb, int fr, int fk) {
   f64x4 acc = {0.0, 0.0, 0.0, 0.0};
 #pragma unroll
   for (int k4 = 0; k4 < 4; ++k4) {
-    const double av = S[(i * 16 + fr) * SLD + kb * 16 + k4 * 4 + fk];
-    const double bv = S[(c * 16 + fr) * SLD + kb * 16 + k4 * 4 + fk];
+    const double av = S[(i * 16 + fr) * LD + kb * 16 + k4 * 4 + fk];
+    const double bv = S[(c * 16 + fr) * LD + kb * 16 + k4 * 4 + fk];
     acc = mfma(av, bv, acc);
   }
 #pragma unroll
-  for (int v = 0; v < 4; ++v) S[(i * 16 + fk + 4 * v) * SLD + c * 16 + fr] -= acc[v];
+  for (int v = 0; v < 4; ++v) S[(i * 16 + fk + 4 * v) * LD + c * 16 + fr] -= acc[v];
 }
 
 #ifdef GOGP_POTRF_NOINLINE
@@ -154,59 +157,60 @@
   __syncthreads();
 }
 
-template <int BS>
-__device__ __forceinline__ void inv_phase(const double *S, f64x4 (&acc)[2], int w, int fr, int fk,
+template <int BS, int LD = SLD, int N = 128, int NWV = NW, int U = 2>
+__device__ __forceinline__ void inv_phase(const double *S, f64x4 (&acc)[U], int w, int fr, int fk,
                                           int aoff, int boff) {
-  constexpr int TB = BS / 16, NTPP = TB * TB, NTL = 4 * TB, KS = BS / 4;
-  double av[2][KS], bv[2][KS];
-#pragma unroll
-  for (int u = 0; u < 2; ++u) {
-    const int tile = w + u * NW;
+  constexpr int TB = BS / 16, NTPP = TB * TB, NTL = N / (2 * BS) * NTPP, KS = BS / 4;
+  static_assert(NTL <= U * NWV, "every tile of the level needs a wave");
+  double av[U][KS], bv[U][KS];
+#pragma unroll
+  for (int u = 0; u < U; ++u) {
+    const int tile = w + u * NWV;
     acc[u] = (f64x4){0.0, 0.0, 0.0, 0.0};
     if (tile < NTL) {
       const int p = tile / NTPP, tl = tile - p * NTPP;
       const int ti = tl / TB, tj = tl - ti * TB, o = p * 2 * BS;
 #pragma unroll
       for (int ks = 0; ks < KS; ++ks) {
-        av[u][ks] = S[(o + BS + ti * 16 + fr) * SLD + o + aoff + ks * 4 + fk];
-        bv[u][ks] = S[(o + boff + ks * 4 + fk) * SLD + o + tj * 16 + fr];
+        av[u][ks] = S[(o + BS + ti * 16 + fr) * LD + o + aoff + ks * 4 + fk];
+        bv[u][ks] = S[(o + boff + ks * 4 + fk) * LD + o + tj * 16 + fr];
       }
     }
   }
 #pragma unroll
   for (int ks = 0; ks < KS; ++ks)
 #pragma unroll
-    for (int u = 0; u < 2; ++u)
-      if (w + u * NW < NTL) acc[u] = mfma(av[u][ks], bv[u][ks], acc[u]);
-}
-
-template <int BS>
-__device__ __forceinline__ void inv_store(double *S, const f64x4 (&acc)[2], int w, int fr, int fk,
+    for (int u = 0; u < U; ++u)
+      if (w + u * NWV < NTL) acc[u] = mfma(av[u][ks], bv[u][ks], acc[u]);
+}
+
+template <int BS, int LD = SLD, int N = 128, int NWV = NW, int U = 2>
+__device__ __forceinline__ void inv_store(double *S, const f64x4 (&acc)[U], int w, int fr, int fk,
                                           double sign) {
-  constexpr int TB = BS / 16, NTPP = TB * TB, NTL = 4 * TB;
-#pragma unroll
-  for (int u = 0; u < 2; ++u) {
-    const int tile = w + u * NW;
+  constexpr int TB = BS / 16, NTPP = TB * TB, NTL = N / (2 * BS) * NTPP;
+#pragma unroll
+  for (int u = 0; u < U; ++u) {
+    const int tile = w + u * NWV;
     if (tile < NTL) {
       const int p = tile / NTPP, tl = tile - p * NTPP;
       const int ti = tl / TB, tj = tl - ti * TB, o = p * 2 * BS;
 #pragma unroll
       for (int v = 0; v < 4; ++v)
-        S[(o + BS + ti * 16 + fk + 4 * v) * SLD + o + tj * 16 + fr] = sign * acc[u][v];
-    }
-  }
-}
-
-template <int BS>
+        S[(o + BS + ti * 16 + fk + 4 * v) * LD + o + tj * 16 + fr] = sign * acc[u][v];
+    }
+  }
+}
+
+template <int BS, int LD = SLD, int N = 128, int NWV = NW, int U = 2>
 __device__ __forceinline__ void inv_level(double *S, int w, int fr, int fk) {
-  f64x4 acc[2];
-  inv_phase<BS>(S, acc, w, fr, fk, 0, 0);
-  __syncthreads();
-  inv_store<BS>(S, acc, w, fr, fk, 1.0);
-  __syncthreads();
-  inv_phase<BS>(S, acc, w, fr, fk, BS, BS);
-  __syncthreads();
-  inv_store<BS>(S, acc, w, fr, fk, -1.0);
+  f64x4 acc[U];
+  inv_phase<BS, LD, N, NWV, U>(S, acc, w, fr, fk, 0, 0);
+  __syncthreads();
+  inv_store<BS, LD, N, NWV, U>(S, acc, w, fr, fk, 1.0);
+  __syncthreads();
+  inv_phase<BS, LD, N, NWV, U>(S, acc, w, fr, fk, BS, BS);
+  __syncthreads();
+  inv_store<BS, LD, N, NWV, U>(S, acc, w, fr, fk, -1.0);
   __syncthreads();
 }
 
@@ -502,6 +506,292 @@
   diag256_body<false, false, 256>(S, G, rinv_s, L + b * 256 * (ld + 1), ld, nullptr, 0L, Dinv + b * 65536L, 0L, 0L, nullptr,
                                   nullptr);
 }
+
+
+#ifndef GOGP_BUILD_TESTHOOKS
+namespace {
+constexpr int RB = 64;
+constexpr int RLD = 66;
+constexpr int RNT = 256;
+constexpr int RNW = RNT / 64;
+
+typedef unsigned u32x4 __attribute__((ext_vector_type(4)));
+typedef unsigned u32x2 __attribute__((ext_vector_type(2)));
+__device__ __forceinline__ auto blk_rsrc(const double *g, long ld) {
+  return __builtin_amdgcn_make_buffer_rsrc(const_cast<double *>(g), 0, (int)(RB * ld * 8), 0x00020000);
+}
+__device__ __forceinline__ unsigned blk_off(long ld, int tid) {
+  return ((unsigned)(tid >> 5) * (unsigned)ld + (tid & 31) * 2) * 8u;
+}
+__device__ __forceinline__ void blk_load(f64x2 (&v)[8], const double *g, long ld, unsigned bo) {
+  const auto rs = blk_rsrc(g, ld);
+#pragma unroll
+  for (int t = 0; t < 8; ++t)
+    v[t] = __builtin_bit_cast(f64x2, __builtin_amdgcn_raw_buffer_load_b128(rs, bo, t * 64 * (int)ld, 0));
+}
+__device__ __forceinline__ void blk_to_lds(double *B, const f64x2 (&v)[8], int tid) {
+#pragma unroll
+  for (int t = 0; t < 8; ++t) {
+    const int idx = tid + RNT * t, i = idx >> 5, cc = (idx & 31) * 2;
+    *reinterpret_cast<f64x2 *>(B + i * RLD + cc) = v[t];
+  }
+}
+__device__ __forceinline__ void blk_lds_to_global(double *g, long ld, unsigned bo, const double *B, int tid) {
+  const auto rs = blk_rsrc(g, ld);
+#pragma unroll
+  for (int t = 0; t < 8; ++t) {
+    const int idx = tid + RNT * t, i = idx >> 5, cc = (idx & 31) * 2;
+    __builtin_amdgcn_raw_buffer_store_b128(__builtin_bit_cast(u32x4, *reinterpret_cast<const f64x2 *>(B + i * RLD + cc)), rs,
+                                           bo, t * 64 * (int)ld, 0);
+  }
+}
+__device__ __forceinline__ void blk_zero_global(double *g, long ld, unsigned bo) {
+  const auto rs = blk_rsrc(g, ld);
+#pragma unroll
+  for (int t = 0; t < 8; ++t) __builtin_amdgcn_raw_buffer_store_b128((u32x4){0u, 0u, 0u, 0u}, rs, bo, t * 64 * (int)ld, 0);
+}
+__device__ __forceinline__ void acc_zero(f64x4 (&c)[2][2]) {
+#pragma unroll
+  for (int m = 0; m < 2; ++m)
+#pragma unroll
+    for (int n = 0; n < 2; ++n) c[m][n] = (f64x4){0.0, 0.0, 0.0, 0.0};
+}
+__device__ __forceinline__ void acc_load_neg(f64x4 (&c)[2][2], const double *g, long ld, unsigned ao) {
+  const auto rs = blk_rsrc(g, ld);
+#pragma unroll
+  for (int m = 0; m < 2; ++m)
+#pragma unroll
+    for (int n = 0; n < 2; ++n)
+#pragma unroll
+      for (int v = 0; v < 4; ++v)
+        c[m][n][v] = -__builtin_bit_cast(
+            double, __builtin_amdgcn_raw_buffer_load_b64(rs, ao, ((16 * m + 4 * v) * (int)ld + 16 * n) * 8, 0));
+}
+__device__ __forceinline__ void acc_store(double *g, long ld, unsigned ao, const f64x4 (&c)[2][2], double sign) {
+  const auto rs = blk_rsrc(g, ld);
+#pragma unroll
+  for (int m = 0; m < 2; ++m)
+#pragma unroll
+    for (int n = 0; n < 2; ++n)
+#pragma unroll
+      for (int v = 0; v < 4; ++v)
+        __builtin_amdgcn_raw_buffer_store_b64(__builtin_bit_cast(u32x2, sign * c[m][n][v]), rs, ao,
+                                              ((16 * m + 4 * v) * (int)ld + 16 * n) * 8, 0);
+}
+
+template <bool QT>
+__device__ __forceinline__ void mma64(f64x4 (&c)[2][2], const double *P, const double *Q, int wr, int wc, int fr, int fk,
+                                      int k40, int k41) {
+  const double *ap = P + (wr * 32 + fr) * RLD + fk;
+  const double *bp = QT ? Q + (wc * 32 + fr) * RLD + fk : Q + fk * RLD + wc * 32 + fr;
+#pragma unroll 4
+  for (int k4 = k40; k4 < k41; ++k4) {
+    double a[2], b[2];
+#pragma unroll
+    for (int m = 0; m < 2; ++m) a[m] = ap[m * 16 * RLD + k4 * 4];
+#pragma unroll
+    for (int n = 0; n < 2; ++n) b[n] = QT ? bp[n * 16 * RLD + k4 * 4] : bp[k4 * 4 * RLD + n * 16];
+#pragma unroll
+    for (int m = 0; m < 2; ++m)
+#pragma unroll
+      for (int n = 0; n < 2; ++n) c[m][n] = mfma(a[m], b[n], c[m][n]);
+  }
+}
+
+template <bool QT, bool TAIL>
+__device__ __forceinline__ void accumulate(f64x4 (&c)[2][2], double *P, double *Q, const double *pg, long pstep, long pld,
+                                           unsigned pbo, const double *qg, long qstep, long qld, unsigned qbo, int nk,
+                                           int k40, bool skip, const double *tail, long tld, unsigned tbo, f64x2 (&tv)[8],
+                                           int tid, int wr, int wc, int fr, int fk) {
+  f64x2 pv[8], qv[8];
+  if (nk > 0) {
+    blk_load(pv, pg, pld, pbo);
+    blk_load(qv, qg, qld, qbo);
+  } else if (TAIL) {
+    blk_load(tv, tail, tld, tbo);
+  }
+#pragma unroll 1
+  for (int k = 0; k < nk; ++k) {
+    blk_to_lds(P, pv, tid);
+    blk_to_lds(Q, qv, tid);
+    __syncthreads();
+    if (k + 1 < nk) {
+      blk_load(pv, pg + (k + 1) * pstep, pld, pbo);
+      blk_load(qv, qg + (k + 1) * qstep, qld, qbo);
+    } else if (TAIL) {
+      blk_load(tv, tail, tld, tbo);
+    }
+    if (!skip) mma64<QT>(c, P, Q, wr, wc, fr, fk, k == 0 ? k40 : 0, RB / 4);
+    __syncthreads();
+  }
+}
+
+__device__ __forceinline__ void sync_global_writes() {
+  __builtin_amdgcn_s_waitcnt(0x0F70);
+  __syncthreads();
+}
+
+__device__ __forceinline__ void potrf64_lds(double *S, double *XD, double *rinv, int tid, long grow0, long nvalid,
+                                            long long *info) {
+  asm volatile("" : "+v"(tid));
+  const int lane = tid & 63, w = tid >> 6;
+  const int fr = lane & 15, fk = lane >> 4;
+  double keep[16], keep_rinv = 0.0;
+  if (w == 0) panel16<RLD, RB>(S, 0, lane, 16, true, grow0, nvalid, info, keep, keep_rinv);
+  __syncthreads();
+  for (int kb = 0; kb < 3; ++kb) {
+    if (w == 0) panel16_store_diag<RLD>(S, kb, rinv + kb * 16, lane, keep, keep_rinv);
+    if (kb + 1 + w < 4) tile_update16<RLD>(S, kb + 1 + w, kb + 1, kb, fr, fk);
+    __syncthreads();
+    if (w == 0) {
+      panel16<RLD, RB>(S, kb + 1, lane, (kb + 2) * 16, true, grow0 + (kb + 1) * 16, nvalid, info, keep, keep_rinv);
+    } else {
+      const int m = 2 - kb, nt3 = m * (m + 1) / 2;
+      for (int t = w - 1; t < nt3; t += 3) {
+        int ii = 0;
+        while ((ii + 1) * (ii + 2) / 2 <= t) ++ii;
+        const int cc = t - ii * (ii + 1) / 2;
+        tile_update16<RLD>(S, kb + 2 + ii, kb + 2 + cc, kb, fr, fk);
+      }
+    }
+    __syncthreads();
+  }
+  if (w == 0) panel16_store_diag<RLD>(S, 3, rinv + 3 * 16, lane, keep, keep_rinv);
+  __syncthreads();
+  inv16<true, RLD>(S, w, XD + w * 16 * XLD, rinv + w * 16, lane);
+  __syncthreads();
+}
+
+__device__ __forceinline__ void invert64_lds(double *S, const double *XD, int tid) {
+  asm volatile("" : "+v"(tid));
+  const int lane = tid & 63, w = tid >> 6;
+  const int fr = lane & 15, fk = lane >> 4;
+  for (int idx = tid; idx < 4 * 256; idx += RNT) {
+    const int kb = idx >> 8, e = idx & 255, rr = e >> 4, c = e & 15;
+    S[(kb * 16 + rr) * RLD + kb * 16 + c] = XD[kb * 16 * XLD + rr * XLD + c];
+  }
+  __syncthreads();
+  inv_level<16, RLD, RB, RNW, 1>(S, w, fr, fk);
+  inv_level<32, RLD, RB, RNW, 1>(S, w, fr, fk);
+}
+struct RLane {
+  int tid, wr, wc, fr, fk, r0, c0;
+  unsigned bol, bod, aoa, aol, aod;
+};
+__device__ __forceinline__ RLane rlane(long ld, long ldl) {
+  RLane t;
+  t.tid = threadIdx.x;
+  asm volatile("" : "+v"(t.tid));
+  const int lane = t.tid & 63, w = t.tid >> 6;
+  t.fr = lane & 15, t.fk = lane >> 4;
+  t.wr = w >> 1, t.wc = w & 1;
+  t.r0 = t.wr * 32 + t.fk, t.c0 = t.wc * 32 + t.fr;
+  t.bol = blk_off(ldl, t.tid), t.bod = blk_off(256, t.tid);
+  t.aoa = ((unsigned)t.r0 * (unsigned)ld + t.c0) * 8u, t.aol = ((unsigned)t.r0 * (unsigned)ldl + t.c0) * 8u;
+  t.aod = (t.r0 * 256u + t.c0) * 8u;
+  return t;
+}
+}
+
+__global__ __launch_bounds__(RNT, 2) void diag256_resident_kernel(const double *A, long ld, double *Lout, long ldl,
+                                                                  double *Dinv, long row0, long nvalid, long long *info,
+                                                                  long bstride) {
+  A = gogp::cand(A, bstride);
+  Lout = gogp::cand(Lout, bstride);
+  Dinv = gogp::cand(Dinv, bstride);
+  if (info) info = gogp::cand(info, bstride);
+  __builtin_amdgcn_s_setprio(3);
+  __shared__ __attribute__((aligned(16))) double P[RB * RLD];
+  __shared__ __attribute__((aligned(16))) double Q[RB * RLD];
+  __shared__ __attribute__((aligned(16))) double XD[4 * 16 * XLD];
+  __shared__ double rinv_s[RB];
+  constexpr long LDD = 256;
+  f64x4 c[2][2];
+  f64x2 tv[8];
+
+#pragma unroll 1
+  for (int j = 0; j < 4; ++j) {
+    {
+      const RLane t = rlane(ld, ldl);
+      acc_load_neg(c, A + (long)j * RB * (ld + 1), ld, t.aoa);
+      accumulate<true, false>(c, P, Q, Lout + (long)j * RB * ldl, RB, ldl, t.bol, Lout + (long)j * RB * ldl, RB, ldl, t.bol,
+                              j, 0, t.wr < t.wc, nullptr, 0, 0, tv, t.tid, t.wr, t.wc, t.fr, t.fk);
+#pragma unroll
+      for (int m = 0; m < 2; ++m)
+#pragma unroll
+        for (int n = 0; n < 2; ++n)
+#pragma unroll
+          for (int v = 0; v < 4; ++v) {
+            const int rr = t.r0 + 16 * m + 4 * v, cc = t.c0 + 16 * n;
+            Q[rr * RLD + cc] = (cc <= rr) ? -c[m][n][v] : 0.0;
+          }
+      __syncthreads();
+    }
+    potrf64_lds(Q, XD, rinv_s, threadIdx.x, row0 + j * RB, nvalid, info);
+    {
+      const RLane t = rlane(ld, ldl);
+      blk_lds_to_global(Lout + (long)j * RB * (ldl + 1), ldl, t.bol, Q, t.tid);
+#pragma unroll 1
+      for (int jj = j + 1; jj < 4; ++jj) {
+        blk_zero_global(Lout + (long)j * RB * ldl + jj * RB, ldl, t.bol);
+        blk_zero_global(Dinv + (long)j * RB * LDD + jj * RB, LDD, t.bod);
+      }
+      sync_global_writes();
+    }
+    invert64_lds(Q, XD, threadIdx.x);
+    const RLane t = rlane(ld, ldl);
+    blk_lds_to_global(Dinv + (long)j * RB * (LDD + 1), LDD, t.bod, Q, t.tid);
+    sync_global_writes();
+#pragma unroll 1
+    for (int i = j + 1; i < 4; ++i) {
+      acc_load_neg(c, A + (long)i * RB * ld + j * RB, ld, t.aoa);
+      accumulate<true, true>(c, P, Q, Lout + (long)i * RB * ldl, RB, ldl, t.bol, Lout + (long)j * RB * ldl, RB, ldl, t.bol, j,
+                             0, false, Dinv + (long)j * RB * (LDD + 1), LDD, t.bod, tv, t.tid, t.wr, t.wc, t.fr, t.fk);
+#pragma unroll
+      for (int m = 0; m < 2; ++m)
+#pragma unroll
+        for (int n = 0; n < 2; ++n)
+#pragma unroll
+          for (int v = 0; v < 4; ++v) P[(t.r0 + 16 * m + 4 * v) * RLD + t.c0 + 16 * n] = -c[m][n][v];
+      blk_to_lds(Q, tv, t.tid);
+      __syncthreads();
+      acc_zero(c);
+      mma64<true>(c, P, Q, t.wr, t.wc, t.fr, t.fk, 0, (t.wc + 1) * 8);
+      acc_store(Lout + (long)i * RB * ldl + j * RB, ldl, t.aol, c, 1.0);
+      sync_global_writes();
+    }
+  }
+#pragma unroll 1
+  for (int j = 0; j < 3; ++j) {
+    const RLane t = rlane(ld, ldl);
+#pragma unroll 1
+    for (int i = j + 1; i < 4; ++i) {
+      acc_zero(c);
+      accumulate<false, true>(c, P, Q, Lout + (long)i * RB * ldl + j * RB, RB, ldl, t.bol, Dinv + (long)j * RB * (LDD + 1),
+                              RB * LDD, LDD, t.bod, i - j, t.wc * 8, false, Dinv + (long)i * RB * (LDD + 1), LDD, t.bod, tv,
+                              t.tid, t.wr, t.wc, t.fr, t.fk);
+#pragma unroll
+      for (int m = 0; m < 2; ++m)
+#pragma unroll
+        for (int n = 0; n < 2; ++n)
+#pragma unroll
+          for (int v = 0; v < 4; ++v) Q[(t.r0 + 16 * m + 4 * v) * RLD + t.c0 + 16 * n] = c[m][n][v];
+      blk_to_lds(P, tv, t.tid);
+      __syncthreads();
+      acc_zero(c);
+      mma64<false>(c, P, Q, t.wr, t.wc, t.fr, t.fk, 0, (t.wr + 1) * 8);
+      acc_store(Dinv + (long)i * RB * LDD + j * RB, LDD, t.aod, c, -1.0);
+      sync_global_writes();
+    }
+  }
+}
+
+void launch_diag256_resident(hipStream_t s, const double *A, int64_t ld, double *Lout, int64_t ldl, double *Dinv,
+                             int64_t row0, int64_t nvalid, long long *info) {
+  GOGP_KLAUNCH(diag256_resident_kernel, dim3(1, 1, (unsigned)gogp::tl_batch.k), dim3(RNT), 0, s, A, (long)ld, Lout,
+               (long)ldl, Dinv, (long)row0, (long)nvalid, info, gogp::tl_batch.stride);
+}
+#endif
 
 #define GOGP_EV 0
 #define GOGP_EVN(name) name
diff --git a/gogp_amd/csrc/handle.h b/gogp_amd/csrc/handle.h
--- a/gogp_amd/csrc/handle.h
+++ b/gogp_amd/csrc/handle.h
@@ -144,6 +144,7 @@
   int chain_prio = -1;
   int tiny = 1;
   int chain_slabs = 0;
+  int diag_resident = -1;
   int chain_split = -1;
   int ktri = 1;
   double *TX = nullptr, *Tmt = nullptr;
diff --git a/gogp_amd/csrc/testhooks.hip b/gogp_amd/csrc/testhooks.hip
--- a/gogp_amd/csrc/testhooks.hip
+++ b/gogp_amd/csrc/testhooks.hip
@@ -350,7 +350,8 @@
 
 extern "C" int gogp_test_diag256_product(int device, int variant, const double *A, int64_t ld, double *L, int64_t ldl,
                                          double *Dinv, int64_t row0, int64_t nvalid, long long *info) {
-  if (!A || !L || !Dinv || !info || variant < 0 || variant > 3) return GOGP_EARG;
+  const bool resident = variant == GOGP_TEST_DIAG256_RESIDENT;
+  if (!A || !L || !Dinv || !info || variant < 0 || (variant > 3 && !resident)) return GOGP_EARG;
   if (ld < PANEL || ldl < PANEL || ld % 2 || ldl % 2 || row0 < 0 || nvalid < 0) return GOGP_EARG;
   const int64_t ldd = (variant & 1) ? 2 * PANEL : PANEL;
   if (!device_ok(device)) return GOGP_EHIP;
@@ -367,6 +368,7 @@
   if (e == hipSuccess) e = hipMemcpy(dinfo, info, 8, hipMemcpyHostToDevice);
   if (e == hipSuccess) {
     switch (variant) {
+      case GOGP_TEST_DIAG256_RESIDENT: launch_diag256_resident(0, dA, ld, dL, ldl, dD, row0, nvalid, dinfo); break;
       case 0: launch_diag256(0, dA, ld, dL, ldl, dD, row0, nvalid, dinfo); break;
       case 1: launch_diag256_ld512(0, dA, ld, dL, ldl, dD, row0, nvalid, dinfo); break;
       case 2: launch_diag256_inv_only(0, dA, ld, dD); break;
@@ -379,6 +381,59 @@
   if (e == hipSuccess) e = hipMemcpy(Dinv, dD, nd, hipMemcpyDeviceToHost);
   if (e == hipSuccess) e = hipMemcpy(info, dinfo, 8, hipMemcpyDeviceToHost);
   (void)hipFree(dA); (void)hipFree(dL); (void)hipFree(dD); (void)hipFree(dinfo);
+  return e == hipSuccess ? GOGP_OK : GOGP_EHIP;
+}
+
+extern "C" int gogp_test_diag256_cand(int device, int variant, int k, const double *A, int64_t ld, double *L, int64_t ldl,
+                                      double *Dinv, int64_t row0, int64_t nvalid, long long *info, int reps,
+                                      double *us_per_launch) {
+  if (!A || !L || !Dinv || !info || (variant != 0 && variant != GOGP_TEST_DIAG256_RESIDENT) || k < 1 || k > 64)
+    return GOGP_EARG;
+  if (ld < PANEL || ldl < PANEL || ld % 2 || ldl % 2 || row0 < 0 || nvalid < 0 || reps < 0 || reps > 10000) return GOGP_EARG;
+  if (!device_ok(device)) return GOGP_EHIP;
+  const size_t na = (size_t)PANEL * ld, nl = (size_t)PANEL * ldl, nd = (size_t)PANEL * PANEL, slot = na + nl + nd + 2;
+  double *arena = nullptr;
+  hipError_t e = hipMalloc(&arena, (size_t)k * slot * 8);
+  for (int c = 0; c < k && e == hipSuccess; ++c) {
+    double *s0 = arena + c * slot;
+    e = hipMemcpy(s0, A + c * na, na * 8, hipMemcpyHostToDevice);
+    if (e == hipSuccess) e = hipMemcpy(s0 + na, L + c * nl, nl * 8, hipMemcpyHostToDevice);
+    if (e == hipSuccess) e = hipMemcpy(s0 + na + nl, Dinv + c * nd, nd * 8, hipMemcpyHostToDevice);
+    if (e == hipSuccess) e = hipMemcpy(s0 + na + nl + nd, info + c, 8, hipMemcpyHostToDevice);
+  }
+  hipEvent_t e0 = nullptr, e1 = nullptr;
+  if (e == hipSuccess) e = hipEventCreate(&e0);
+  if (e == hipSuccess) e = hipEventCreate(&e1);
+  if (e == hipSuccess) {
+    tl_batch.k = k;
+    tl_batch.stride = (long)(slot * 8);
+    for (int r = 0; r <= reps; ++r) {
+      if (r == 1) (void)hipEventRecord(e0, 0);
+      if (variant == 0)
+        launch_diag256(0, arena, ld, arena + na, ldl, arena + na + nl, row0, nvalid,
+                       reinterpret_cast<long long *>(arena + na + nl + nd));
+      else
+        launch_diag256_resident(0, arena, ld, arena + na, ldl, arena + na + nl, row0, nvalid,
+                                reinterpret_cast<long long *>(arena + na + nl + nd));
+    }
+    if (reps > 0) (void)hipEventRecord(e1, 0);
+    tl_batch.k = 1;
+    tl_batch.stride = 0;
+    e = hipGetLastError();
+    if (e == hipSuccess) e = hipDeviceSynchronize();
+    float ms = 0.f;
+    if (e == hipSuccess && reps > 0) e = hipEventElapsedTime(&ms, e0, e1);
+    if (us_per_launch) *us_per_launch = reps > 0 ? ms * 1e3 / reps : 0.0;
+  }
+  for (int c = 0; c < k && e == hipSuccess; ++c) {
+    const double *s0 = arena + c * slot;
+    e = hipMemcpy(L + c * nl, s0 + na, nl * 8, hipMemcpyDeviceToHost);
+    if (e == hipSuccess) e = hipMemcpy(Dinv + c * nd, s0 + na + nl, nd * 8, hipMemcpyDeviceToHost);
+    if (e == hipSuccess) e = hipMemcpy(info + c, s0 + na + nl + nd, 8, hipMemcpyDeviceToHost);
+  }
+  if (e0) (void)hipEventDestroy(e0);
+  if (e1) (void)hipEventDestroy(e1);
+  (void)hipFree(arena);
   return e == hipSuccess ? GOGP_OK : GOGP_EHIP;
 }
 
diff --git a/gogp_amd/gp.py b/gogp_amd/gp.py
--- a/gogp_amd/gp.py
+++ b/gogp_amd/gp.py
@@ -732,6 +732,25 @@
     return out
 
 
+DIAG256_RESIDENT = 16
+
+
+def diag256_cand(A: np.ndarray, variant: int = 0, row0: int = 0, nvalid: int = 256, ldl: int = 256, reps: int = 0,
+                 device: int = -1):
+    A = _arr(A)
+    if A.ndim != 3 or A.shape[1] != 256 or A.shape[2] < 256 or ldl < 256:
+        raise ValueError("A: k x 256 rows of at least 256")
+    k = A.shape[0]
+    L, Dinv = np.zeros((k, 256, ldl)), np.zeros((k, 256, 256))
+    info = (ctypes.c_longlong * k)()
+    us = ctypes.c_double(0.0)
+    rc = _lib.hooks().gogp_test_diag256_cand(device, variant, k, _dp(A), A.shape[2], _dp(L), ldl, _dp(Dinv), row0, nvalid,
+                                             info, reps, ctypes.byref(us))
+    if rc != _lib.GOGP_OK:
+        raise GogpError(rc, "test_diag256_cand")
+    return L, Dinv, np.array(list(info), dtype=np.int64), us.value
+
+
 def diag256_product(A: np.ndarray, variant: int = 0, row0: int = 0, nvalid: int = 256, L=None, Dinv=None,
                     device: int = -1):
     A = _arr(A)
diff --git a/include/gogp_testhooks.h b/include/gogp_testhooks.h
--- a/include/gogp_testhooks.h
+++ b/include/gogp_testhooks.h
@@ -41,8 +41,11 @@
 int gogp_test_diag_syrk(int device, int bs, const float *L, int64_t l_len, int64_t l_off, int64_t ld, int64_t K,
                         int64_t row_stride, double *D64, int64_t d_len, int nblocks);
 
+#define GOGP_TEST_DIAG256_RESIDENT 16
 int gogp_test_diag256_product(int device, int variant, const double *A, int64_t ld, double *L, int64_t ldl,
                               double *Dinv, int64_t row0, int64_t nvalid, long long *info);
+int gogp_test_diag256_cand(int device, int variant, int k, const double *A, int64_t ld, double *L, int64_t ldl,
+                           double *Dinv, int64_t row0, int64_t nvalid, long long *info, int reps, double *us_per_launch);
 
 
 int64_t gogp_test_trsm_small_workspace(int64_t npad);
```

After: 14.08, median of 6. Within noise of the previous version (+1.0%).
